# Crowsinc/LiveVisionKit

Hardware: AMD Instinct MI355X
Metric: stabilized frames/sec (one 4K YUV420 stream per GPU, steady state) (higher is better)
Workload: dtype f32

## Files before the change

### include/lvk_hip.h

```cpp
#ifndef LVK_HIP_H
#define LVK_HIP_H

#include <stdint.h>
#include <stddef.h>

#ifdef __cplusplus
extern "C" {
#endif

#define LVK_HIP_OK              0
#define LVK_HIP_ERR_ARG        -1
#define LVK_HIP_ERR_RUNTIME    -2
#define LVK_HIP_ERR_NO_DEVICE  -3

typedef struct lvk_hip_ctx lvk_hip_ctx;


int  lvk_hip_ctx_create(int device, lvk_hip_ctx** out);
int  lvk_hip_ctx_create_on_stream(int device, void* hip_stream, lvk_hip_ctx** out);
void lvk_hip_ctx_destroy(lvk_hip_ctx* ctx);
int  lvk_hip_sync(lvk_hip_ctx* ctx);
void* lvk_hip_stream(lvk_hip_ctx* ctx);
const char* lvk_hip_last_error(lvk_hip_ctx* ctx);
const char* lvk_hip_version(void);
// ... 247 lines not shown
#define LVK_SCHED_PUSH_FREE_RUNNING   0
#define LVK_SCHED_PUSH_SYNCHRONISED   1
#define LVK_SCHED_INGEST_ON_TRACKER   2
#define LVK_SCHED_INGEST_ON_BULK      3
#define LVK_SCHED_INGEST_INLINE       4
#define LVK_SCHED_REMAP_PERSISTENT    5
#define LVK_SCHED_REMAP_FULL          6
#define LVK_SCHED_WAIT_SIGNAL_WORD    7
#define LVK_SCHED_WAIT_EVENT          8
#define LVK_SCHED_WAIT_WORD_TIMEOUT   9
#define LVK_SCHED_COUNT              10
int  lvk_hip_stab_schedule_counters(lvk_hip_stab* stab, long long out[LVK_SCHED_COUNT], int reset);

int  lvk_hip_stab_get_stats(const lvk_hip_stab* stab, lvk_stab_stats* out);
int  lvk_hip_stab_detector_frames(const lvk_hip_stab* stab, long long* on_device, long long* on_host);
int  lvk_hip_stab_get_meshes(const lvk_hip_stab* stab, float* motion, float* correction, int cap_floats);
int  lvk_hip_stab_get_features(const lvk_hip_stab* stab, float* xy_resp_age, int cap);


#define LVK_STAGE_DOWNSCALE 0
#define LVK_STAGE_PYRAMID   1
#define LVK_STAGE_FAST      2
#define LVK_STAGE_PYRLK     3
#define LVK_STAGE_MOTION    4
#define LVK_STAGE_REMAP     5
#define LVK_STAGE_INGEST    6
#define LVK_STAGE_EGRESS    7
#define LVK_STAGE_COUNT     8
int  lvk_hip_stab_set_profiling(lvk_hip_stab* stab, int enable);
int  lvk_hip_stab_get_profile(lvk_hip_stab* stab, double total_ms[LVK_STAGE_COUNT], long long launches[LVK_STAGE_COUNT]);

int lvk_hip_native_rcp(lvk_hip_ctx* ctx, const float* d_in, float* d_out, size_t n);

typedef struct lvk_hip_mesh_solver lvk_hip_mesh_solver;
int  lvk_hip_mesh_solver_create(lvk_hip_ctx* ctx, int cols, int rows, float gen_region_w, float gen_region_h,
                                float temporal_smoothing, float local_smoothing, int max_points, lvk_hip_mesh_solver** out);
void lvk_hip_mesh_solver_destroy(lvk_hip_mesh_solver* solver);
int  lvk_hip_mesh_solver_reset(lvk_hip_mesh_solver* solver);
int  lvk_hip_mesh_solver_solve(lvk_hip_mesh_solver* solver, const float* tracked, const float* matched, int n, float region_w, float region_h,
                               float temporal_now, float threshold, uint8_t* inliers, float* offsets);

int lvk_hip_luma_area_resize(lvk_hip_ctx* ctx, const void* d_src, int src_step, int pix_stride, int channel,
                             int srows, int scols, void* d_dst, int dst_step, int drows, int dcols);

int lvk_hip_pyr_down(lvk_hip_ctx* ctx, const void* d_src, int src_step, int rows, int cols, void* d_dst, int dst_step);
int lvk_hip_scharr(lvk_hip_ctx* ctx, const void* d_src, int src_step, int rows, int cols, void* d_dst);

int lvk_hip_build_pyramid(lvk_hip_ctx* ctx, const void* d_img, int step, int rows, int cols, int max_level, int win_w, int win_h,
                          uint8_t* levels, int16_t* derivs, int* level_rows, int* level_cols);

int lvk_hip_fast_detect(lvk_hip_ctx* ctx, const void* d_img, int step, int rows, int cols,
                        const int* regions, int nregions, uint32_t* out, int cap, int* counts);

int lvk_hip_pyrlk(lvk_hip_ctx* ctx, const void* d_prev, int prev_step, const void* d_next, int next_step, int rows, int cols,
                  const float* prev_pts, int n, float* next_pts, uint8_t* status,
                  int win_w, int win_h, int max_level, int max_count, double epsilon, double min_eig_threshold);

int lvk_hip_estimate_global_motion(lvk_hip_ctx* ctx, const float* pts1, const float* pts2, int n, double threshold,
                                   double region_w, double region_h, int full_homography, double H[9], uint8_t* mask);

int lvk_hip_fast_filter(lvk_hip_ctx* ctx, const float* prev, const float* matched, const uint8_t* status, int n, float* out_prev, float* out_matched);

#define LVK_TRACK_CHAIN_GUARD 64
#define LVK_TRACK_CHAIN_FILL  0xA5
typedef struct lvk_track_chain_desc
{
    const float* prev; const float* matched; const uint8_t* status; const float* und;
    const void* d_prev_img; int prev_step; const void* d_next_img; int next_step; int rows, cols;
    int win_w, win_h, max_level, max_count; double epsilon, min_eig;
    const lvk_camera_params* lens; int lens_rows, lens_cols; double lens_sx, lens_sy;
    int n_bound, count_on_device, n_word;
    int full, model_on_device, full_word;
    int separate_compact, host_signal;
    double threshold; int region_w, region_h;
} lvk_track_chain_desc;
typedef struct lvk_track_chain_result
{
    double H[9]; int rc, signalled, count_dev, count_host;
    uint8_t* mask; float* pairs_dev; float* mirror_matched; uint8_t* mirror_status;
    float* next_pts; uint8_t* flow_status; float* flow_und;
} lvk_track_chain_result;
int lvk_hip_track_chain(lvk_hip_ctx* ctx, const lvk_track_chain_desc* desc, lvk_track_chain_result* result);

int lvk_hip_deblock_get_grid(lvk_hip_deblock* deb, uint8_t* mean, uint8_t* grid, float* keep_block, int capacity, int extent_xy[2]);

int lvk_hip_cas_const(float sharpness, float* peak);

int lvk_hip_cvt_code_target(int code, int src_format, int dcn);

int lvk_hip_fsr_easu_const(int rw, int rh, int W, int H, int ow, int oh, float con[16]);

int lvk_hip_fsr_easu_path(int rw, int rh, int out_rows, int out_cols);

enum
{
    LVK_AREA_PATH_FAST_DW_8x8_C3_BGR = 0, LVK_AREA_PATH_FAST_DW_8x8_C3_RGB = 1, LVK_AREA_PATH_FAST_DW_4x4_C3_BGR = 2, LVK_AREA_PATH_FAST_DW_4x4_C3_RGB = 3,
    LVK_AREA_PATH_FAST_DW_8x8_C3 = 4, LVK_AREA_PATH_FAST_DW_4x4_C3 = 5, LVK_AREA_PATH_FAST_DW_8x8_C1 = 6, LVK_AREA_PATH_FAST_DW_4x4_C1 = 7,
    LVK_AREA_PATH_FAST = 8, LVK_AREA_PATH_TILE_4 = 9, LVK_AREA_PATH_TILE_8 = 10, LVK_AREA_PATH_TAPS_4 = 11, LVK_AREA_PATH_TAPS_8 = 12,
    LVK_AREA_PATH_GENERAL = 13, LVK_AREA_PATH_ENLARGE = 14, LVK_AREA_PATH_COUNT = 15
};
int lvk_hip_area_resize_path(lvk_hip_ctx* ctx, const void* d_src, int src_step, int pix_stride, int channel,
                             int srows, int scols, int drows, int dcols);

#ifdef __cplusplus
}
#endif

#include "lvk_hip_deblock_px.h"
#endif
```

### livevisionkit_amd/_native.py

```python
import ctypes
import os

_HERE = os.path.dirname(os.path.abspath(__file__))
LIB_PATH = os.environ.get("LVK_HIP_LIB") or os.path.join(_HERE, "liblvk_hip.so")

_c = ctypes
_P = _c.c_void_p
_SIG = {
    "lvk_hip_ctx_create": (_c.c_int, [_c.c_int, _c.POINTER(_P)]),
    "lvk_hip_ctx_create_on_stream": (_c.c_int, [_c.c_int, _P, _c.POINTER(_P)]),
    "lvk_hip_ctx_destroy": (None, [_P]),
    "lvk_hip_sync": (_c.c_int, [_P]),
    "lvk_hip_stream": (_P, [_P]),
    "lvk_hip_last_error": (_c.c_char_p, [_P]),
    "lvk_hip_version": (_c.c_char_p, []),
    "lvk_hip_abi_version": (_c.c_int, []),
    "lvk_hip_device_count": (_c.c_int, []),
    "lvk_hip_device_usable": (_c.c_int, [_c.c_int]),
    "lvk_hip_malloc": (_c.c_int, [_P, _c.c_size_t, _c.POINTER(_P)]),
    "lvk_hip_free": (_c.c_int, [_P, _P]),
    "lvk_hip_trim": (_c.c_int, [_P]),
    "lvk_hip_ctx_wait": (_c.c_int, [_P, _P]),
    "lvk_hip_upload": (_c.c_int, [_P, _P, _P, _c.c_size_t]),
    "lvk_hip_download": (_c.c_int, [_P, _P, _P, _c.c_size_t]),
    "lvk_hip_remap_homography": (_c.c_int, [_P, _P, _c.c_int, _c.c_int, _c.c_int, _P, _c.c_int, _c.c_int, _c.c_int,
                                            _c.c_int, _c.c_int, _c.POINTER(_c.c_float), _c.POINTER(_c.c_uint8), _c.c_int]),
    "lvk_hip_remap_mesh": (_c.c_int, [_P, _P, _c.c_int, _c.c_int, _c.c_int, _P, _c.c_int,
                                      _c.POINTER(_c.c_float), _c.c_int, _c.c_int, _c.POINTER(_c.c_uint8), _c.c_int]),
    "lvk_hip_remap_map": (_c.c_int, [_P, _P, _c.c_int, _c.c_int, _c.c_int, _P, _c.c_int, _P, _c.c_int, _c.POINTER(_c.c_uint8), _c.c_int]),
    "lvk_hip_remap_homography_gray": (_c.c_int, [_P, _P, _c.c_int, _c.c_int, _c.c_int, _P, _c.c_int, _c.c_int, _c.c_int,
                                                 _c.c_int, _c.c_int, _c.POINTER(_c.c_float), _c.c_uint8]),
    "lvk_hip_remap_mesh_gray": (_c.c_int, [_P, _P, _c.c_int, _c.c_int, _c.c_int, _P, _c.c_int, _c.POINTER(_c.c_float), _c.c_int, _c.c_int, _c.c_uint8]),
    "lvk_hip_remap_map_gray": (_c.c_int, [_P, _P, _c.c_int, _c.c_int, _c.c_int, _P, _c.c_int, _P, _c.c_int, _c.c_uint8]),
    "lvk_hip_warpmesh_apply_gray": (_c.c_int, [_P, _P, _c.c_int, _c.c_int, _c.c_int, _P, _c.c_int, _c.POINTER(_c.c_float), _c.c_int, _c.c_int, _c.c_uint8]),
    "lvk_hip_warpmesh_apply_lens_gray": (_c.c_int, [_P, _P, _c.c_int, _c.c_int, _c.c_int, _P, _c.c_int, _c.POINTER(_c.c_float), _c.c_int, _c.c_int, _c.c_uint8, _P]),
    "lvk_hip_stab_push_gray": (_c.c_int, [_P, _P, _c.c_int, _c.c_int, _c.c_int, _c.c_uint64, _P, _c.c_int, _c.c_int,
                                          _c.POINTER(_c.c_int), _c.POINTER(_c.c_uint64), _c.POINTER(_P), _P]),
    "lvk_hip_stab_push_gray_host": (_c.c_int, [_P, _P, _c.c_int, _c.c_int, _c.c_int, _c.c_uint64, _P, _c.c_int, _c.c_int,
                                               _c.POINTER(_c.c_int), _c.POINTER(_c.c_uint64), _P]),
    "lvk_hip_set_remap_precision": (_c.c_int, [_P, _c.c_int]),
    "lvk_hip_get_remap_precision": (_c.c_int, [_P]),
    "lvk_hip_stab_set_remap_precision": (_c.c_int, [_P, _c.c_int]),
    "lvk_hip_stab_get_remap_precision": (_c.c_int, [_P]),
    "lvk_hip_remap_homography_c4": (_c.c_int, [_P, _P, _c.c_int, _c.c_int, _c.c_int, _P, _c.c_int, _c.c_int, _c.c_int,
                                               _c.c_int, _c.c_int, _c.POINTER(_c.c_float), _c.POINTER(_c.c_uint8)]),
    "lvk_hip_remap_mesh_c4": (_c.c_int, [_P, _P, _c.c_int, _c.c_int, _c.c_int, _P, _c.c_int, _c.POINTER(_c.c_float), _c.c_int, _c.c_int, _c.POINTER(_c.c_uint8)]),
    "lvk_hip_remap_map_c4": (_c.c_int, [_P, _P, _c.c_int, _c.c_int, _c.c_int, _P, _c.c_int, _P, _c.c_int, _c.POINTER(_c.c_uint8)]),
    "lvk_hip_warpmesh_apply_c4": (_c.c_int, [_P, _P, _c.c_int, _c.c_int, _c.c_int, _P, _c.c_int, _c.POINTER(_c.c_float), _c.c_int, _c.c_int, _c.POINTER(_c.c_uint8)]),
    "lvk_hip_warpmesh_apply_lens_c4": (_c.c_int, [_P, _P, _c.c_int, _c.c_int, _c.c_int, _P, _c.c_int, _c.POINTER(_c.c_float), _c.c_int, _c.c_int, _c.POINTER(_c.c_uint8), _P]),
    "lvk_hip_stab_set_background_alpha": (_c.c_int, [_P, _c.c_int]),
    "lvk_hip_stab_push_c4": (_c.c_int, [_P, _P, _c.c_int, _c.c_int, _c.c_int, _c.c_uint64, _c.c_int, _P, _c.c_int, _c.c_int,
                                        _c.POINTER(_c.c_int), _c.POINTER(_c.c_uint64), _c.POINTER(_P), _P]),
    "lvk_hip_stab_push_c4_host": (_c.c_int, [_P, _P, _c.c_int, _c.c_int, _c.c_int, _c.c_uint64, _c.c_int, _P, _c.c_int, _c.c_int,
                                             _c.POINTER(_c.c_int), _c.POINTER(_c.c_uint64), _P]),
    "lvk_hip_upscale": (_c.c_int, [_P, _P, _c.c_int, _c.c_int, _c.c_int, _P, _c.c_int, _c.c_int, _c.c_int, _c.c_int]),
    "lvk_hip_sharpen": (_c.c_int, [_P, _P, _c.c_int, _c.c_int, _c.c_int, _P, _c.c_int, _c.c_float]),
    "lvk_hip_upscale_gray": (_c.c_int, [_P, _P, _c.c_int, _c.c_int, _c.c_int, _P, _c.c_int, _c.c_int, _c.c_int]),
    "lvk_hip_upscale_c4": (_c.c_int, [_P, _P, _c.c_int, _c.c_int, _c.c_int, _P, _c.c_int, _c.c_int, _c.c_int]),
    "lvk_hip_sharpen_gray": (_c.c_int, [_P, _P, _c.c_int, _c.c_int, _c.c_int, _P, _c.c_int, _c.c_float]),
    "lvk_hip_sharpen_c4": (_c.c_int, [_P, _P, _c.c_int, _c.c_int, _c.c_int, _P, _c.c_int, _c.c_float]),
    "lvk_hip_native_rcp": (_c.c_int, [_P, _P, _P, _c.c_size_t]),
    "lvk_hip_mesh_solver_create": (_c.c_int, [_P, _c.c_int, _c.c_int, _c.c_float, _c.c_float, _c.c_float, _c.c_float, _c.c_int, _c.POINTER(_P)]),
    "lvk_hip_mesh_solver_destroy": (None, [_P]),
    "lvk_hip_mesh_solver_reset": (_c.c_int, [_P]),
    "lvk_hip_mesh_solver_solve": (_c.c_int, [_P, _c.POINTER(_c.c_float), _c.POINTER(_c.c_float), _c.c_int, _c.c_float, _c.c_float, _c.c_float, _c.c_float,
                                             _c.POINTER(_c.c_uint8), _c.POINTER(_c.c_float)]),
    "lvk_hip_lens_map_create": (_c.c_int, [_P, _P, _c.c_int, _c.c_int, _c.POINTER(_P), _c.POINTER(_c.c_int)]),
    "lvk_hip_lens_map_destroy": (_c.c_int, [_P, _P]),
    "lvk_hip_warpmesh_apply_lens": (_c.c_int, [_P, _P, _c.c_int, _c.c_int, _c.c_int, _P, _c.c_int, _c.POINTER(_c.c_float), _c.c_int, _c.c_int, _c.POINTER(_c.c_uint8), _c.c_int, _P]),
    "lvk_hip_lens_undistort_points": (_c.c_int, [_P, _P, _c.c_int, _c.c_int, _c.c_double, _c.c_double, _c.POINTER(_c.c_float), _c.c_int, _c.POINTER(_c.c_float)]),
    "lvk_hip_stab_set_lens": (_c.c_int, [_P, _P]),
    "lvk_hip_stab_output_stream": (_P, [_P]),
    "lvk_hip_fast_filter": (_c.c_int, [_P, _c.POINTER(_c.c_float), _c.POINTER(_c.c_float), _c.POINTER(_c.c_uint8), _c.c_int, _c.POINTER(_c.c_float), _c.POINTER(_c.c_float)]),
    "lvk_hip_stab_draw_trackers": (_c.c_int, [_P]),
    "lvk_hip_stab_draw_motion_mesh": (_c.c_int, [_P]),
    "lvk_hip_draw_grid": (_c.c_int, [_P, _P, _c.c_int, _c.c_int, _c.c_int, _c.c_int, _c.c_int, _c.POINTER(_c.c_uint8), _c.c_int]),
    "lvk_hip_draw_crosses": (_c.c_int, [_P, _P, _c.c_int, _c.c_int, _c.c_int, _c.POINTER(_c.c_float), _c.c_int, _c.c_float, _c.c_float,
                                        _c.POINTER(_c.c_uint8), _c.c_int, _c.c_int]),
    "lvk_hip_draw_points": (_c.c_int, [_P, _P, _c.c_int, _c.c_int, _c.c_int, _c.POINTER(_c.c_float), _c.c_int, _c.c_float, _c.c_float,
                                       _c.POINTER(_c.c_uint8), _c.c_int]),
    "lvk_hip_draw_rect": (_c.c_int, [_P, _P, _c.c_int, _c.c_int, _c.c_int, _c.POINTER(_c.c_int), _c.POINTER(_c.c_uint8), _c.c_int]),
    "lvk_hip_draw_text": (_c.c_int, [_P, _P, _c.c_int, _c.c_int, _c.c_int, _c.c_char_p, _c.c_int, _c.c_int, _c.POINTER(_c.c_uint8), _c.c_int, _c.c_int]),
    "lvk_hip_text_size": (_c.c_int, [_c.c_char_p, _c.c_int, _c.c_int, _c.POINTER(_c.c_int), _c.POINTER(_c.c_int)]),
    "lvk_hip_warpmesh_apply_yuv420": (_c.c_int, [_P, _P, _c.c_int, _c.c_int, _c.c_int, _P, _c.c_int, _P, _c.c_int, _P, _c.c_int, _c.c_int,
                                                 _c.POINTER(_c.c_float), _c.c_int, _c.c_int, _c.POINTER(_c.c_uint8)]),
    "lvk_hip_warpmesh_apply": (_c.c_int, [_P, _P, _c.c_int, _c.c_int, _c.c_int, _P, _c.c_int,
                                          _c.POINTER(_c.c_float), _c.c_int, _c.c_int, _c.POINTER(_c.c_uint8), _c.c_int]),
    "lvk_hip_luma_area_resize": (_c.c_int, [_P, _P, _c.c_int, _c.c_int, _c.c_int, _c.c_int, _c.c_int, _P, _c.c_int, _c.c_int, _c.c_int]),
    "lvk_hip_pyr_down": (_c.c_int, [_P, _P, _c.c_int, _c.c_int, _c.c_int, _P, _c.c_int]),
    "lvk_hip_scharr": (_c.c_int, [_P, _P, _c.c_int, _c.c_int, _c.c_int, _P]),
    "lvk_hip_build_pyramid": (_c.c_int, [_P, _P, _c.c_int, _c.c_int, _c.c_int, _c.c_int, _c.c_int, _c.c_int,
                                         _c.POINTER(_c.c_uint8), _c.POINTER(_c.c_int16), _c.POINTER(_c.c_int), _c.POINTER(_c.c_int)]),
    "lvk_hip_fast_detect": (_c.c_int, [_P, _P, _c.c_int, _c.c_int, _c.c_int, _c.POINTER(_c.c_int), _c.c_int,
                                       _c.POINTER(_c.c_uint32), _c.c_int, _c.POINTER(_c.c_int)]),
    "lvk_hip_pyrlk": (_c.c_int, [_P, _P, _c.c_int, _P, _c.c_int, _c.c_int, _c.c_int, _c.POINTER(_c.c_float), _c.c_int,
                                 _c.POINTER(_c.c_float), _c.POINTER(_c.c_uint8), _c.c_int, _c.c_int, _c.c_int, _c.c_int,
                                 _c.c_double, _c.c_double]),
    "lvk_hip_ingest_yuv420": (_c.c_int, [_P, _P, _c.c_int, _P, _c.c_int, _P, _c.c_int, _c.c_int, _c.c_int, _c.c_int, _P, _c.c_int]),
    "lvk_hip_egress_yuv420": (_c.c_int, [_P, _P, _c.c_int, _c.c_int, _c.c_int, _P, _c.c_int, _P, _c.c_int, _P, _c.c_int, _c.c_int]),
    "lvk_hip_ingest_obs": (_c.c_int, [_P, _c.c_int, _P * 3, _c.c_int * 3, _c.c_int, _c.c_int, _P, _c.c_int]),
    "lvk_hip_egress_obs": (_c.c_int, [_P, _c.c_int, _P, _c.c_int, _c.c_int, _c.c_int, _P * 3, _c.c_int * 3]),
    "lvk_hip_obs_frame_format": (_c.c_int, [_c.c_int]),
    "lvk_hip_estimate_global_motion": (_c.c_int, [_P, _c.POINTER(_c.c_float), _c.POINTER(_c.c_float), _c.c_int, _c.c_double,
                                                  _c.c_double, _c.c_double, _c.c_int, _c.POINTER(_c.c_double), _c.POINTER(_c.c_uint8)]),
    "lvk_hip_track_chain": (_c.c_int, [_P, _P, _P]),
    "lvk_stab_default_settings": (None, [_P]),
    "lvk_hip_stab_create": (_c.c_int, [_P, _P, _c.POINTER(_P)]),
    "lvk_hip_stab_destroy": (None, [_P]),
    "lvk_hip_stab_configure": (_c.c_int, [_P, _P]),
    "lvk_hip_stab_restart": (_c.c_int, [_P]),
    "lvk_hip_stab_reset_context": (_c.c_int, [_P]),
    "lvk_hip_stab_ready": (_c.c_int, [_P]),
    "lvk_hip_stab_frame_delay": (_c.c_int, [_P]),
    "lvk_hip_stab_stable_region": (_c.c_int, [_P, _c.c_int, _c.c_int, _c.POINTER(_c.c_int)]),
    "lvk_hip_stab_next_output": (_c.c_int, [_P, _c.c_int, _c.c_int, _c.c_int, _P]),
    "lvk_hip_stab_push": (_c.c_int, [_P, _P, _c.c_int, _c.c_int, _c.c_int, _c.c_uint64, _c.c_int, _P, _c.c_int, _c.c_int,
                                     _c.POINTER(_c.c_int), _c.POINTER(_c.c_uint64), _c.POINTER(_P), _P]),
    "lvk_hip_stab_push_yuv420": (_c.c_int, [_P, _P, _c.c_int, _P, _c.c_int, _P, _c.c_int, _c.c_int, _c.c_int, _c.c_int, _c.c_uint64,
                                            _P, _c.c_int, _P, _c.c_int, _P, _c.c_int, _c.c_int, _c.POINTER(_c.c_int), _c.POINTER(_c.c_uint64), _P]),
    "lvk_hip_stab_push_obs": (_c.c_int, [_P, _c.c_int, _P * 3, _c.c_int * 3, _c.c_int, _c.c_int, _c.c_uint64, _P * 3, _c.c_int * 3, _c.c_int,
                                         _c.POINTER(_c.c_int), _c.POINTER(_c.c_uint64), _P]),
    "lvk_hip_stab_push_yuv420_host": (_c.c_int, [_P, _P, _c.c_int, _P, _c.c_int, _P, _c.c_int, _c.c_int, _c.c_int, _c.c_int, _c.c_uint64,
                                            _P, _c.c_int, _P, _c.c_int, _P, _c.c_int, _c.c_int, _c.POINTER(_c.c_int), _c.POINTER(_c.c_uint64), _P]),
    "lvk_hip_stab_push_obs_host": (_c.c_int, [_P, _c.c_int, _P * 3, _c.c_int * 3, _c.c_int, _c.c_int, _c.c_uint64, _P * 3, _c.c_int * 3, _c.c_int,
                                              _c.POINTER(_c.c_int), _c.POINTER(_c.c_uint64), _P]),
    "lvk_hip_stab_prefetch_yuv420_host": (_c.c_int, [_P, _P, _c.c_int, _P, _c.c_int, _P, _c.c_int, _c.c_int, _c.c_int, _c.c_int]),
    "lvk_hip_stab_prefetch_cancel": (_c.c_int, [_P]),
    "lvk_hip_stab_prefetch": (_c.c_int, [_P, _P, _c.c_int, _c.c_int, _c.c_int, _c.c_int]),
    "lvk_hip_stab_prefetch_yuv420": (_c.c_int, [_P, _P, _c.c_int, _P, _c.c_int, _P, _c.c_int, _c.c_int, _c.c_int, _c.c_int]),
    "lvk_hip_stab_lookahead_frames": (_c.c_longlong, [_P]),
    "lvk_hip_stab_schedule_counters": (_c.c_int, [_P, _c.POINTER(_c.c_longlong), _c.c_int]),
    "lvk_hip_stab_detector_frames": (_c.c_int, [_P, _c.POINTER(_c.c_longlong), _c.POINTER(_c.c_longlong)]),
    "lvk_hip_host_malloc": (_c.c_int, [_P, _c.c_size_t, _c.POINTER(_P)]),
    "lvk_hip_host_free": (_c.c_int, [_P, _P]),
    "lvk_hip_stab_get_stats": (_c.c_int, [_P, _P]),
    "lvk_hip_stab_get_meshes": (_c.c_int, [_P, _c.POINTER(_c.c_float), _c.POINTER(_c.c_float), _c.c_int]),
    "lvk_hip_stab_get_features": (_c.c_int, [_P, _c.POINTER(_c.c_float), _c.c_int]),
    "lvk_hip_stab_set_overlap": (_c.c_int, [_P, _c.c_int]),
    "lvk_hip_stab_set_bulk_context": (_c.c_int, [_P, _P]),
    "lvk_hip_stab_set_profiling": (_c.c_int, [_P, _c.c_int]),
    "lvk_hip_stab_get_profile": (_c.c_int, [_P, _c.POINTER(_c.c_double), _c.POINTER(_c.c_longlong)]),
    "lvk_hip_deblock_default_settings": (None, [_P]),
    "lvk_hip_deblock_create": (_c.c_int, [_P, _P, _c.POINTER(_P)]),
    "lvk_hip_deblock_configure": (_c.c_int, [_P, _P]),
    "lvk_hip_deblock_destroy": (None, [_P]),
    "lvk_hip_deblock_apply": (_c.c_int, [_P, _P, _c.c_int, _c.c_int, _c.c_int, _c.c_int, _c.POINTER(_c.c_int)]),
    "lvk_hip_deblock_draw_influence": (_c.c_int, [_P, _P, _c.c_int, _c.c_int, _c.c_int, _c.c_int]),
    "lvk_hip_deblock_filter_region": (_c.c_int, [_P, _c.POINTER(_c.c_int)]),
    "lvk_hip_deblock_get_grid": (_c.c_int, [_P, _c.POINTER(_c.c_uint8), _c.POINTER(_c.c_uint8), _c.POINTER(_c.c_float), _c.c_int, _c.POINTER(_c.c_int)]),
    "lvk_hip_cas": (_c.c_int, [_P, _P, _c.c_int, _c.c_int, _c.c_int, _c.c_int, _P, _c.c_int, _c.c_float]),
    "lvk_hip_cas_const": (_c.c_int, [_c.c_float, _c.POINTER(_c.c_float)]),
    "lvk_hip_reformat": (_c.c_int, [_P, _P, _c.c_int, _c.c_int, _c.c_int, _c.c_int, _P, _c.c_int, _c.c_int]),
    "lvk_hip_cvt_code_target": (_c.c_int, [_c.c_int, _c.c_int, _c.c_int]),
    "lvk_hip_fsr_easu": (_c.c_int, [_P, _P, _c.c_int, _c.c_int, _c.c_int, _c.c_int, _c.POINTER(_c.c_int), _P, _c.c_int, _c.c_int, _c.c_int]),
    "lvk_hip_fsr_geometry": (_c.c_int, [_c.c_int, _c.c_int, _c.c_int, _c.c_int, _c.c_float, _c.c_int, _c.POINTER(_c.c_int), _c.POINTER(_c.c_int),
                                        _c.POINTER(_c.c_int), _c.POINTER(_c.c_int)]),
    "lvk_hip_fsr_easu_const": (_c.c_int, [_c.c_int, _c.c_int, _c.c_int, _c.c_int, _c.c_int, _c.c_int, _c.POINTER(_c.c_float)]),
    "lvk_hip_fsr_easu_path": (_c.c_int, [_c.c_int, _c.c_int, _c.c_int, _c.c_int]),
    "lvk_hip_area_resize_path": (_c.c_int, [_P, _P, _c.c_int, _c.c_int, _c.c_int, _c.c_int, _c.c_int, _c.c_int, _c.c_int]),
}

_SIG_DEBLOCK_PX = {
    "lvk_hip_deblock_apply_gray": (_c.c_int, [_P, _P, _c.c_int, _c.c_int, _c.c_int, _c.POINTER(_c.c_int)]),
    "lvk_hip_deblock_apply_c4": (_c.c_int, [_P, _P, _c.c_int, _c.c_int, _c.c_int, _c.c_int, _c.POINTER(_c.c_int)]),
}

_lib = None

# ... 26 lines not shown
```

### livevisionkit_amd/context.py

```python
import ctypes

import numpy as np

from . import _native


class LvkHipError(RuntimeError):
    pass


def _f32(a):
    a = np.ascontiguousarray(a, dtype=np.float32)
    return a, a.ctypes.data_as(ctypes.POINTER(ctypes.c_float))


def _u8x3(bg):
    a = np.ascontiguousarray(bg, dtype=np.uint8).reshape(3)
    return a, a.ctypes.data_as(ctypes.POINTER(ctypes.c_uint8))


def _u8x4(bg):
    a = np.ascontiguousarray(bg, dtype=np.uint8).reshape(4)
    return a, a.ctypes.data_as(ctypes.POINTER(ctypes.c_uint8))

# ... 408 lines not shown
        p = np.ascontiguousarray(points, np.float32).reshape(-1, 2)
        ca, cp = _u8x3(colour)
        self._check(self.lib.lvk_hip_draw_crosses(self.handle, frame.data_ptr(), frame.stride(0), frame.shape[0], frame.shape[1],
                                                  p.ctypes.data_as(ctypes.POINTER(ctypes.c_float)), len(p), float(scaling[0]), float(scaling[1]), cp,
                                                  int(cross_size), int(thickness)))
        return frame

    def fast_filter(self, prev, matched, status):
        a = np.ascontiguousarray(prev, np.float32).reshape(-1, 2); b = np.ascontiguousarray(matched, np.float32).reshape(-1, 2)
        st = np.ascontiguousarray(status, np.uint8).reshape(-1)
        oa = np.zeros_like(a); ob = np.zeros_like(b)
        fp = ctypes.POINTER(ctypes.c_float)
        m = self.lib.lvk_hip_fast_filter(self.handle, a.ctypes.data_as(fp), b.ctypes.data_as(fp), st.ctypes.data_as(ctypes.POINTER(ctypes.c_uint8)), len(a),
                                         oa.ctypes.data_as(fp), ob.ctypes.data_as(fp))
        if m < 0:
            self._check(m)
        return oa[:m], ob[:m]

    def track_chain(self, prev, matched=None, status=None, und=None, images=None, win=(11, 11), max_level=3, max_count=5, epsilon=0.01, min_eig=1e-4,
                    lens=None, threshold=3.0, region=(480, 270), full=True, full_word=None, n_word=None, separate_compact=False, host_signal=False):
        fp, bp = ctypes.POINTER(ctypes.c_float), ctypes.POINTER(ctypes.c_uint8)
        prev = np.ascontiguousarray(prev, np.float32).reshape(-1, 2)
        nb, G = len(prev), TRACK_CHAIN_GUARD
        d, r = TrackChainDesc(), TrackChainResult()
        keep = [prev]
        d.prev = prev.ctypes.data_as(fp)
        if images is None:
            matched = np.ascontiguousarray(matched, np.float32).reshape(nb, 2); status = np.ascontiguousarray(status, np.uint8).reshape(nb)
            keep += [matched, status]
            d.matched = matched.ctypes.data_as(fp); d.status = status.ctypes.data_as(bp)
            if und is not None:
                und = np.ascontiguousarray(und, np.float32).reshape(-1, 2)
                n_eff = nb if n_word is None else min(max(int(n_word), 0), nb)
                if len(und) != 2 * n_eff:
                    raise ValueError("und holds 2 x the effective count of positions (previous | matched)")
                keep.append(und)
                d.und = und.ctypes.data_as(fp)
        else:
            a, b = images
            keep += [a, b]
            d.d_prev_img = a.data_ptr(); d.prev_step = a.stride(0); d.d_next_img = b.data_ptr(); d.next_step = b.stride(0)
            d.rows, d.cols = a.shape[0], a.shape[1]
            d.win_w, d.win_h, d.max_level, d.max_count, d.epsilon, d.min_eig = win[0], win[1], max_level, max_count, float(epsilon), float(min_eig)
            if lens is not None:
                params, lrows, lcols, sx, sy = lens
                arr = (ctypes.c_double * 9)(*[float(v) for v in params])
                keep.append(arr)
                d.lens = ctypes.cast(arr, ctypes.c_void_p); d.lens_rows, d.lens_cols, d.lens_sx, d.lens_sy = int(lrows), int(lcols), float(sx), float(sy)
        d.n_bound = nb
        d.count_on_device, d.n_word = (0, 0) if n_word is None else (1, int(n_word))
        d.full = 1 if full else 0
        d.model_on_device, d.full_word = (0, 0) if full_word is None else (1, int(full_word))
        d.separate_compact = 1 if separate_compact else 0; d.host_signal = 1 if host_signal else 0
        d.threshold = float(threshold); d.region_w, d.region_h = int(region[0]), int(region[1])
        mask = np.zeros(nb, np.uint8); pairs = np.zeros((2, nb, 2), np.float32); mm = np.zeros((nb, 2), np.float32); ms = np.zeros(nb, np.uint8)
        r.mask = mask.ctypes.data_as(bp); r.pairs_dev = pairs.ctypes.data_as(fp); r.mirror_matched = mm.ctypes.data_as(fp); r.mirror_status = ms.ctypes.data_as(bp)
        out = {}
        if images is not None:
            nxt = np.zeros((nb + 2 * G, 2), np.float32); fst = np.zeros(nb + 2 * G, np.uint8); fund = np.zeros((2 * nb + 2 * G, 2), np.float32)
            r.next_pts = nxt.ctypes.data_as(fp); r.flow_status = fst.ctypes.data_as(bp); r.flow_und = fund.ctypes.data_as(fp)
            out.update(next_pts=nxt, flow_status=fst, flow_und=fund)
        self._check(self.lib.lvk_hip_track_chain(self.handle, ctypes.byref(d), ctypes.byref(r)))
        del keep
        out.update(H=np.array(r.H, np.float64).reshape(3, 3), rc=r.rc, signalled=r.signalled, count_dev=r.count_dev, count_host=r.count_host, mask=mask,
                   pairs_dev=pairs, mirror_matched=mm, mirror_status=ms)
        return out

    def warpmesh_apply_yuv420(self, src, mesh, bg=(255, 0, 255), nv12=False):
        import torch
        rows, cols = src.shape[0], src.shape[1]
        y = torch.empty((rows, cols), dtype=torch.uint8, device=src.device)
        if nv12:
            u = torch.empty((rows // 2, cols // 2, 2), dtype=torch.uint8, device=src.device); v = u
        else:
            u = torch.empty((rows // 2, cols // 2), dtype=torch.uint8, device=src.device); v = torch.empty_like(u)
        m = np.ascontiguousarray(mesh, dtype=np.float32)
        ma, mp = _f32(m)
        bga, bgp = _u8x3(bg)
        self._check(self.lib.lvk_hip_warpmesh_apply_yuv420(self.handle, src.data_ptr(), src.stride(0), rows, cols, y.data_ptr(), y.stride(0),
                                                           u.data_ptr(), u.stride(0), v.data_ptr(), v.stride(0), 1 if nv12 else 0,
                                                           mp, m.shape[0], m.shape[1], bgp))
        return (y, u) if nv12 else (y, u, v)


class MeshSolver:

    def __init__(self, ctx, cols, rows, gen_region, temporal, local, max_points):
        self.ctx, self.cols, self.rows = ctx, cols, rows
        h = ctypes.c_void_p()
        ctx._check(ctx.lib.lvk_hip_mesh_solver_create(ctx.handle, cols, rows, float(gen_region[0]), float(gen_region[1]), float(temporal), float(local),
                                                      int(max_points), ctypes.byref(h)))
        self.handle = h

    def solve(self, tracked, matched, region=(480, 270), temporal=1.0, threshold=10.0):
        t = np.ascontiguousarray(tracked, np.float32).reshape(-1, 2); m = np.ascontiguousarray(matched, np.float32).reshape(-1, 2)
        inl = np.zeros(len(t), np.uint8); off = np.zeros((self.rows, self.cols, 2), np.float32)
        fp = ctypes.POINTER(ctypes.c_float)
        rc = self.ctx.lib.lvk_hip_mesh_solver_solve(self.handle, t.ctypes.data_as(fp), m.ctypes.data_as(fp), len(t), float(region[0]), float(region[1]),
                                                    float(temporal), float(threshold), inl.ctypes.data_as(ctypes.POINTER(ctypes.c_uint8)), off.ctypes.data_as(fp))
        if rc < 0:
            self.ctx._check(rc)
        return rc, inl, off

    def reset(self):
        self.ctx._check(self.ctx.lib.lvk_hip_mesh_solver_reset(self.handle))

    def close(self):
        if getattr(self, "handle", None):
            if getattr(self.ctx, "handle", None):
                self.ctx.lib.lvk_hip_mesh_solver_destroy(self.handle)
            self.handle = None
```

### livevisionkit_amd/csrc/lvk_hip_internal.hpp

```cpp
#pragma once

#include <hip/hip_runtime.h>
#include <cstdint>
#include <cstdio>
#include <string>
#include <vector>
#include <functional>
#include <map>
#include <set>
#include <mutex>
#include <utility>

#include "lvk_hip.h"

struct LinTabEntry { int s0, s1; float a0, a1; };
struct Lin8Entry { int s0, s1, a0, a1; };
struct AreaTabEntry { int si; float alpha; };
struct FastRegion { int x, y, w, h, threshold, active; };
constexpr int LVK_FAST_INLINE_REGIONS = 8;

constexpr int LVK_MAX_PYR_LEVELS = 8;
struct PyrLevel { const uint8_t* img; const short2* deriv; int rows, cols, step; };
struct PyrArgs { PyrLevel lv[LVK_MAX_PYR_LEVELS]; int nlevels; };

// ... 154 lines not shown
int lvk_launch_fast(lvk_hip_ctx* ctx, const void* d_img, int step, int rows, int cols,
                    const FastRegion* d_regions, int nregions, int max_rw, int max_rh,
                    void* d_masks, void* d_scores, uint32_t* d_out, int cap, int* d_counts, const FastRegion* host_regions = nullptr);

struct FastInsertDesc
{
    const uint16_t* col_of; const uint32_t* row_base; const uint8_t* bucket;
    uint32_t* cell_first; void* cell_best ; int* region_count;
    const uint32_t* occ;
    const int* occ_bucket;
    int capacity; bool small_grid; int n_held, min_samples; float uniformity, homography_threshold;
    float2* pts; uint32_t* new_kp; int* result; int* d_n; int* d_full; int* counts;
};
int lvk_launch_fast_insert(lvk_hip_ctx* ctx, const void* d_img, int step, int rows, int cols, const FastRegion* host_regions, int nregions,
                           int max_rw, int max_rh, void* d_masks, void* d_scores, const FastInsertDesc& d);
bool lvk_fast_insert_fits(int cells, int nregions, int max_rw, int max_rh, int cols, int rows);
int lvk_fast_cells_reset(lvk_hip_ctx* ctx, uint32_t* d_first, void* d_best, int cells, int* d_region_count );

struct LensModel;
int lvk_pyramid_geometry(int rows, int cols, int max_level, int win_w, int win_h, int* lrows, int* lcols);
int lvk_launch_pyrlk(lvk_hip_ctx* ctx, const PyrArgs& prev, const PyrArgs& next, const float2* d_prev_pts, int n,
                     float2* d_next_pts, uint8_t* d_status, int win_w, int win_h, int max_count, double epsilon, double min_eig,
                     float2* d_prev_copy = nullptr,
                     const LensModel* lens = nullptr, double lens_sx = 0.0, double lens_sy = 0.0, float2* d_und = nullptr,
                     const int* d_n = nullptr);

struct DevicePyramid
{
    uint8_t* img_base = nullptr;
    uint8_t* deriv_base = nullptr;
    PyrArgs args{};
    int allocate(lvk_hip_ctx* ctx, int rows, int cols, int max_level, int win_w, int win_h);
    int build(lvk_hip_ctx* ctx, bool derivs = false);
    void release();
};

struct LvkHostSignal { unsigned* flag; unsigned seq; };

size_t lvk_ransac_workspace_bytes(int n);
int lvk_launch_ransac(lvk_hip_ctx* ctx, const float2* d_p1, const float2* d_p2, int n, double threshold, double region_w, double region_h,
                      bool full_homography, void* d_ws, double* d_H, int* d_ninl, uint8_t* d_mask, const int* d_n = nullptr,
                      const int* d_full = nullptr,
                      LvkHostSignal done = LvkHostSignal{nullptr, 0});
int lvk_launch_match_compact(lvk_hip_ctx* ctx, const float2* d_prev, const float2* d_matched, const uint8_t* d_status, int n,
                             float2* d_p1, float2* d_p2, int* d_count, int* h_count, float2* h_matched, uint8_t* h_status,
                             const float2* d_und = nullptr, float region_w = 0.0f, float region_h = 0.0f,
                             const int* d_n_raw = nullptr);
constexpr int LVK_COMPACT_RANSAC_MAX = 2048;
int lvk_launch_compact_ransac(lvk_hip_ctx* ctx, const float2* d_prev, const float2* d_matched, const uint8_t* d_status, int n,
                              float2* d_p1, float2* d_p2, int* d_count, int* h_count, float2* h_matched, uint8_t* h_status,
                              const float2* d_und, float region_wf, float region_hf,
                              double threshold, double region_w, double region_h, bool full_homography, void* d_ws, double* d_H, int* d_ninl, uint8_t* d_mask,
                              const int* d_n_raw = nullptr, const int* d_full = nullptr, LvkHostSignal done = LvkHostSignal{nullptr, 0});

struct LvkTrackChain
{
    const PyrArgs* prev_pyr = nullptr; const PyrArgs* next_pyr = nullptr;
    const float2* h_pts = nullptr;
    int win_w = 0, win_h = 0, max_count = 0; double epsilon = 0.0, min_eig = 0.0;
    const LensModel* lens = nullptr; double lens_sx = 0.0, lens_sy = 0.0;
    int n = 0; const int* d_n = nullptr;
    bool full = false; const int* d_full = nullptr;
    float2* d_pts = nullptr; float2* d_matched = nullptr; uint8_t* d_status = nullptr;
    float2* d_und = nullptr;
    float2* d_p1 = nullptr; float2* d_p2 = nullptr; int* d_count = nullptr;
    int* h_count = nullptr; float2* h_matched = nullptr; uint8_t* h_status = nullptr;
    int region_w = 0, region_h = 0; double threshold = 0.0;
    bool separate_compact = false;
    bool estimate = true;
    void* d_ws = nullptr; double* h_H = nullptr; int* h_ninl = nullptr; uint8_t* h_mask = nullptr;
    LvkHostSignal done{nullptr, 0};
    void (*stage_boundary)(void* user) = nullptr; void* user = nullptr;
};
int lvk_launch_track_chain(lvk_hip_ctx* ctx, const LvkTrackChain& c);

struct LensArgs;
struct RemapLaunch
{
    hipStream_t stream = nullptr;
    int precision = LVK_REMAP_EXACT;
    const LensArgs* lens = nullptr;
    bool co_scheduled = false;
    int co_blocks_per_cu = 0;
};
int lvk_launch_remap_homography(lvk_hip_ctx* ctx, const void* d_src, int src_step, int src_rows, int src_cols,
                                void* d_dst, int dst_step, int dst_rows, int dst_cols, int off_x, int off_y,
                                const float H[9], const uint8_t bg[3], int yuv, const RemapLaunch& o);
int lvk_launch_remap_mesh(lvk_hip_ctx* ctx, const void* d_src, int src_step, int src_rows, int src_cols,
                          void* d_dst, int dst_step, const float* mesh, int mesh_rows, int mesh_cols, const uint8_t bg[3], int yuv, const RemapLaunch& o);

int lvk_launch_ingest_yuv420(lvk_hip_ctx* ctx, hipStream_t stream, const void* d_y, int y_step, const void* d_u, int u_step,
                             const void* d_v, int v_step, int nv12, int rows, int cols, void* d_dst, int dst_step);
int lvk_launch_egress_yuv420(lvk_hip_ctx* ctx, hipStream_t stream, const void* d_src, int src_step, int rows, int cols,
                             void* d_y, int y_step, void* d_u, int u_step, void* d_v, int v_step, int nv12);
int lvk_ingest_obs_check(lvk_hip_ctx* ctx, int video_format, const void* const d_planes[3], const int steps[3], int rows, int cols);
int lvk_launch_ingest_obs(lvk_hip_ctx* ctx, hipStream_t stream, int video_format, const void* const d_planes[3], const int steps[3],
                          int rows, int cols, void* d_dst, int dst_step);
int lvk_launch_egress_obs(lvk_hip_ctx* ctx, hipStream_t stream, int video_format, const void* d_src, int src_step, int rows, int cols,
                          void* const d_planes[3], const int steps[3]);


int lvk_launch_remap_map(lvk_hip_ctx* ctx, const void* d_src, int src_step, int rows, int cols,
                         void* d_dst, int dst_step, const void* d_map, int map_step, const uint8_t bg[3], int yuv, const RemapLaunch& o);

struct LensModel { double d[17]; float f[17]; int view[4]; };
struct LensModelD { double d[17]; };
__device__ __forceinline__ float2 lvk_lens_undistort_point(const LensModelD& M, double sx, double sy, float2 p)
{
    const double nfx = M.d[0], nfy = M.d[1], ncx = M.d[2], ncy = M.d[3], fx = M.d[4], fy = M.d[5], cx = M.d[6], cy = M.d[7];
    const double k1 = M.d[8], k2 = M.d[9], p1 = M.d[10], p2 = M.d[11], k3 = M.d[12];
    const double kxc = M.d[13], vxc = M.d[14], kyc = M.d[15], vyc = M.d[16];
    const double s = (double)p.x * sx, t = (double)p.y * sy;
    double u = s, v = t;
    for (int pass = 0; pass < 2; pass++)
    {
        const double s1 = s - (u * kxc + vxc), t1 = t - (v * kyc + vyc);
        const double x0 = (s1 - cx) / fx, y0 = (t1 - cy) / fy;
        double x = x0, y = y0;
        for (int j = 0; j < 5; j++)
        {
            const double r2 = x * x + y * y;
            const double icdist = 1.0 / (1 + ((k3 * r2 + k2) * r2 + k1) * r2);
            if (icdist < 0) { x = x0; y = y0; break; }
            const double dX = 2 * p1 * x * y + p2 * (r2 + 2 * x * x);
            const double dY = p1 * (r2 + 2 * y * y) + 2 * p2 * x * y;
            x = (x0 - dX) * icdist;
            y = (y0 - dY) * icdist;
        }
        u = x * nfx + ncx; v = y * nfy + ncy;
    }
    return make_float2((float)(u / sx), (float)(v / sy));
}
struct LensArgs { float f[17]; };
int lvk_lens_model_build(const lvk_camera_params& params, int rows, int cols, LensModel& out);
int lvk_launch_lens_undistort(lvk_hip_ctx* ctx, hipStream_t stream, const LensModel& model, double sx, double sy,
                              const float2* a, int na, const float2* b, int nb, float2* out);
int lvk_launch_warpmesh_apply_lens(lvk_hip_ctx* ctx, const void* d_src, int src_step, int rows, int cols,
                                   void* d_dst, int dst_step, const float* mesh, int mesh_rows, int mesh_cols, const uint8_t bg[3], int yuv, const RemapLaunch& o);

int lvk_launch_remap_homography_gray(lvk_hip_ctx* ctx, const void* d_src, int src_step, int src_rows, int src_cols,
                                     void* d_dst, int dst_step, int dst_rows, int dst_cols, int off_x, int off_y, const float H[9], uint8_t bg, const RemapLaunch& o);
int lvk_launch_remap_mesh_gray(lvk_hip_ctx* ctx, const void* d_src, int src_step, int rows, int cols, void* d_dst, int dst_step,
                               const float* mesh, int mesh_rows, int mesh_cols, uint8_t bg, const RemapLaunch& o);
int lvk_launch_remap_map_gray(lvk_hip_ctx* ctx, const void* d_src, int src_step, int rows, int cols,
                              void* d_dst, int dst_step, const void* d_map, int map_step, uint8_t bg, const RemapLaunch& o);
int lvk_launch_warpmesh_apply_lens_gray(lvk_hip_ctx* ctx, const void* d_src, int src_step, int rows, int cols, void* d_dst, int dst_step,
                                        const float* mesh, int mesh_rows, int mesh_cols, uint8_t bg, const RemapLaunch& o);

int lvk_launch_remap_homography_c4(lvk_hip_ctx* ctx, const void* d_src, int src_step, int src_rows, int src_cols,
                                   void* d_dst, int dst_step, int dst_rows, int dst_cols, int off_x, int off_y, const float H[9], const uint8_t bg[4], const RemapLaunch& o);
int lvk_launch_remap_mesh_c4(lvk_hip_ctx* ctx, const void* d_src, int src_step, int rows, int cols, void* d_dst, int dst_step,
                             const float* mesh, int mesh_rows, int mesh_cols, const uint8_t bg[4], const RemapLaunch& o);
int lvk_launch_remap_map_c4(lvk_hip_ctx* ctx, const void* d_src, int src_step, int rows, int cols,
                            void* d_dst, int dst_step, const void* d_map, int map_step, const uint8_t bg[4], const RemapLaunch& o);
int lvk_launch_warpmesh_apply_lens_c4(lvk_hip_ctx* ctx, const void* d_src, int src_step, int rows, int cols, void* d_dst, int dst_step,
                                      const float* mesh, int mesh_rows, int mesh_cols, const uint8_t bg[4], const RemapLaunch& o);

int lvk_launch_draw_grid(lvk_hip_ctx* ctx, hipStream_t stream, void* d_dst, int dst_step, int rows, int cols, int grid_w, int grid_h,
                         const uint8_t colour[3], int thickness);
int lvk_launch_draw_crosses(lvk_hip_ctx* ctx, hipStream_t stream, void* d_dst, int dst_step, int rows, int cols, const float* pts, int n,
                            float scale_x, float scale_y, const uint8_t colour[3], int cross_size, int thickness);

int lvk_launch_upscale(lvk_hip_ctx* ctx, hipStream_t stream, const void* d_src, int src_step, int src_rows, int src_cols,
                       void* d_dst, int dst_step, int dst_rows, int dst_cols, int yuv);
int lvk_launch_sharpen(lvk_hip_ctx* ctx, hipStream_t stream, const void* d_src, int src_step, int rows, int cols,
                       void* d_dst, int dst_step, float sharpness);

struct lvk_mesh_solver_dev;
int lvk_mesh_solver_create(lvk_hip_ctx* ctx, int cols, int rows, float gen_w, float gen_h, float temporal, float local, lvk_mesh_solver_dev** out);
void lvk_mesh_solver_free(lvk_mesh_solver_dev* s);
int lvk_mesh_solver_reset(lvk_mesh_solver_dev* s, hipStream_t stream);
int lvk_mesh_solver_cols(const lvk_mesh_solver_dev* s);
int lvk_mesh_solver_rows(const lvk_mesh_solver_dev* s);
int lvk_launch_mesh_solve(lvk_mesh_solver_dev* s, hipStream_t stream, void* d_scratch , const float2* d_p1, const float2* d_p2, const int* d_count, int n_pts,
                          int min_samples, float region_w, float region_h, float temporal_now, float threshold,
                          float* h_offsets, uint8_t* h_mask, int* h_status);

int lvk_launch_warpmesh_apply_420(lvk_hip_ctx* ctx, const void* d_src, int src_step, int rows, int cols,
                                  void* o_y, int oy_step, void* o_u, int ou_step, void* o_v, int ov_step, int nv12,
                                  const float* mesh, int mesh_rows, int mesh_cols, const uint8_t bg[3], const RemapLaunch& o);
bool lvk_remap_obs_fusable(int video_format);
int lvk_launch_warpmesh_apply_obs(lvk_hip_ctx* ctx, int video_format, const void* d_src, int src_step, int rows, int cols,
                                  void* const planes[3], const int steps[3], const float* mesh, int mesh_rows, int mesh_cols, const uint8_t bg[3], const RemapLaunch& o);
```

### livevisionkit_amd/csrc/remap.hip

```cpp
#include "remap_core.hpp"
#ifndef LVK_CO_LDS_PAD
#define LVK_CO_LDS_PAD 0
#endif

namespace {


LVK_REMAP_KERNEL_CO(bool YUV, k_remap_homography,
                    (const uint8_t* __restrict__ src, int src_step, int src_rows, int src_cols,
                     uint8_t* __restrict__ dst, int dst_step, int dst_rows, int dst_cols,
                     int off_x, int off_y, HomographyArgs H, uint32_t bg),
{
    remap_homography<YUV, W, false>(src, src_step, src_rows, src_cols, PackedSink{dst, dst_step}, dst_rows, dst_cols, off_x, off_y, H, LensArgs{}, bg);
})

LVK_REMAP_KERNEL_CO(bool YUV, k_remap_homography_lens,
                    (const uint8_t* __restrict__ src, int src_step, int src_rows, int src_cols,
                     uint8_t* __restrict__ dst, int dst_step, int dst_rows, int dst_cols,
                     int off_x, int off_y, HomographyArgs H, LensArgs L, uint32_t bg),
{
    remap_homography<YUV, W, true>(src, src_step, src_rows, src_cols, PackedSink{dst, dst_step}, dst_rows, dst_cols, off_x, off_y, H, L, bg);
})

LVK_REMAP_KERNEL_CO(bool YUV, k_remap_mesh,
                    (const uint8_t* __restrict__ src, int src_step, int src_rows, int src_cols,
                     uint8_t* __restrict__ dst, int dst_step,
                     const float* __restrict__ mesh, int mesh_cols, int mesh_floats,
                     const LinTabEntry* __restrict__ xtab, const LinTabEntry* __restrict__ ytab, uint32_t bg),
{
    LVK_WITH_MESH_COORD(false, LensArgs{}, src_rows, src_cols, (remap_strip<YUV, W>(src, src_step, src_rows, src_cols, PackedSink{dst, dst_step}, src_rows, src_cols, coord, bg)))
})

LVK_REMAP_KERNEL_CO(bool YUV, k_remap_mesh_lens,
                    (const uint8_t* __restrict__ src, int src_step, int src_rows, int src_cols,
                     uint8_t* __restrict__ dst, int dst_step,
                     const float* __restrict__ mesh, int mesh_cols, int mesh_floats,
                     const LinTabEntry* __restrict__ xtab, const LinTabEntry* __restrict__ ytab, LensArgs L, uint32_t bg),
{
    LVK_WITH_MESH_COORD(true, L, src_rows, src_cols, (remap_strip<YUV, W>(src, src_step, src_rows, src_cols, PackedSink{dst, dst_step}, src_rows, src_cols, coord, bg)))
})

LVK_REMAP_KERNEL(bool YUV, , k_remap_map,
                 (const uint8_t* __restrict__ src, int src_step, int src_rows, int src_cols,
                  uint8_t* __restrict__ dst, int dst_step, const uint8_t* __restrict__ map, int map_step, uint32_t bg),
{
    const MapCoord coord{map, map_step};
    remap_strip<YUV, W>(src, src_step, src_rows, src_cols, PackedSink{dst, dst_step}, src_rows, src_cols, coord, bg);
})

template <bool YUV>
__global__ __launch_bounds__(256) LVK_REMAP_ATTR
void k_easu_scale(const uint8_t* __restrict__ src, int src_step, int src_rows, int src_cols,
                  uint8_t* __restrict__ dst, int dst_step, int dst_rows, int dst_cols, float rsx, float rsy)
{
    const ScaleCoord coord{rsx, rsy};
    remap_strip<YUV>(src, src_step, src_rows, src_cols, PackedSink{dst, dst_step}, dst_rows, dst_cols, coord, 0u);
}

struct Planes420 { uint8_t* y; int y_step; uint8_t* u; int u_step; uint8_t* v; int v_step; };
template <bool NV12> __device__ __forceinline__ Sink420<NV12> sink420(const Planes420& o) { return Sink420<NV12>{o.y, o.y_step, o.u, o.u_step, o.v, o.v_step}; }

LVK_REMAP_KERNEL(bool NV12, LVK_CO_SCHEDULED, k_remap_homography_420,
                 (const uint8_t* __restrict__ src, int src_step, int rows, int cols, Planes420 o, HomographyArgs H, uint32_t bg),
{
    LVK_TL(0);
    remap_homography<true, W, false>(src, src_step, rows, cols, sink420<NV12>(o), rows, cols, 0, 0, H, LensArgs{}, bg);
})

LVK_REMAP_KERNEL(bool NV12, LVK_CO_SCHEDULED, k_remap_homography_lens_420,
                 (const uint8_t* __restrict__ src, int src_step, int rows, int cols, Planes420 o, HomographyArgs H, LensArgs L, uint32_t bg),
{
    remap_homography<true, W, true>(src, src_step, rows, cols, sink420<NV12>(o), rows, cols, 0, 0, H, L, bg);
})

LVK_REMAP_KERNEL(bool NV12, LVK_CO_SCHEDULED, k_remap_mesh_420,
                 (const uint8_t* __restrict__ src, int src_step, int rows, int cols, Planes420 o,
                  const float* __restrict__ mesh, int mesh_cols, int mesh_floats, const LinTabEntry* __restrict__ xtab, const LinTabEntry* __restrict__ ytab, uint32_t bg),
{
    const Sink420<NV12> sink = sink420<NV12>(o);
    LVK_WITH_MESH_COORD(false, LensArgs{}, rows, cols, (remap_strip<true, W>(src, src_step, rows, cols, sink, rows, cols, coord, bg)))
})

LVK_REMAP_KERNEL(bool NV12, LVK_CO_SCHEDULED, k_remap_mesh_lens_420,
                 (const uint8_t* __restrict__ src, int src_step, int rows, int cols, Planes420 o,
                  const float* __restrict__ mesh, int mesh_cols, int mesh_floats, const LinTabEntry* __restrict__ xtab, const LinTabEntry* __restrict__ ytab,
                  LensArgs L, uint32_t bg),
{
    const Sink420<NV12> sink = sink420<NV12>(o);
    LVK_WITH_MESH_COORD(true, L, rows, cols, (remap_strip<true, W>(src, src_step, rows, cols, sink, rows, cols, coord, bg)))
})

}

int lvk_launch_remap_homography(lvk_hip_ctx* ctx, const void* d_src, int src_step, int src_rows, int src_cols,
                                void* d_dst, int dst_step, int dst_rows, int dst_cols,
                                int off_x, int off_y, const float H[9], const uint8_t bg[3], int yuv, const RemapLaunch& o)
{
    LVK_HIP_REQUIRE(ctx, remap_precision_known(o.precision));
    LVK_HIP_REQUIRE(ctx, H != nullptr && bg != nullptr);
    LVK_HIP_REQUIRE(ctx, remap_plane_ok(d_src, src_step, src_rows, src_cols, 3) && remap_plane_ok(d_dst, dst_step, dst_rows, dst_cols, 3));
    HomographyArgs args;
    std::memcpy(args.h, H, sizeof(args.h));
    if (o.lens)
        launch_remap(ctx, LVK_REMAP_FORMS_CO(k_remap_homography_lens, false, true), yuv != 0, dst_rows, dst_cols, o, 0, (const uint8_t*)d_src, src_step, src_rows, src_cols,
                     (uint8_t*)d_dst, dst_step, dst_rows, dst_cols, off_x, off_y, args, *o.lens, pack_bg(bg));
    else
        launch_remap(ctx, LVK_REMAP_FORMS_CO(k_remap_homography, false, true), yuv != 0, dst_rows, dst_cols, o, 0, (const uint8_t*)d_src, src_step, src_rows, src_cols,
                     (uint8_t*)d_dst, dst_step, dst_rows, dst_cols, off_x, off_y, args, pack_bg(bg));
    LVK_HIP_CHECK(ctx, hipGetLastError());
    return LVK_HIP_OK;
}

int lvk_launch_remap_mesh(lvk_hip_ctx* ctx, const void* d_src, int src_step, int src_rows, int src_cols,
                          void* d_dst, int dst_step,
                          const float* mesh, int mesh_rows, int mesh_cols, const uint8_t bg[3], int yuv, const RemapLaunch& o)
{
    LVK_HIP_REQUIRE(ctx, remap_precision_known(o.precision));
    LVK_HIP_REQUIRE(ctx, bg != nullptr && remap_mesh_ok(mesh, mesh_rows, mesh_cols));
    LVK_HIP_REQUIRE(ctx, remap_plane_ok(d_src, src_step, src_rows, src_cols, 3) && remap_plane_ok(d_dst, dst_step, src_rows, src_cols, 3));
    return with_staged_mesh(ctx, o.stream, mesh, mesh_rows, mesh_cols, src_rows, src_cols, [&](const StagedMesh& m) {
        if (o.lens)
            launch_remap(ctx, LVK_REMAP_FORMS_CO(k_remap_mesh_lens, false, true), yuv != 0, src_rows, src_cols, o, 0, (const uint8_t*)d_src, src_step, src_rows, src_cols,
                         (uint8_t*)d_dst, dst_step, m.d_mesh, m.mesh_cols, m.mesh_floats, m.xtab, m.ytab, *o.lens, pack_bg(bg));
        else
            launch_remap(ctx, LVK_REMAP_FORMS_CO(k_remap_mesh, false, true), yuv != 0, src_rows, src_cols, o, 0, (const uint8_t*)d_src, src_step, src_rows, src_cols,
                         (uint8_t*)d_dst, dst_step, m.d_mesh, m.mesh_cols, m.mesh_floats, m.xtab, m.ytab, pack_bg(bg));
    });
}

int lvk_launch_remap_map(lvk_hip_ctx* ctx, const void* d_src, int src_step, int rows, int cols,
                         void* d_dst, int dst_step, const void* d_map, int map_step, const uint8_t bg[3], int yuv, const RemapLaunch& o)
{
    LVK_HIP_REQUIRE(ctx, remap_precision_known(o.precision));
    LVK_HIP_REQUIRE(ctx, bg != nullptr);
    LVK_HIP_REQUIRE(ctx, remap_plane_ok(d_src, src_step, rows, cols, 3) && remap_plane_ok(d_dst, dst_step, rows, cols, 3) && remap_map_ok(d_map, map_step, rows, cols));
    launch_remap(ctx, LVK_REMAP_FORMS(k_remap_map, false, true), yuv != 0, rows, cols, RemapLaunch{o.stream, o.precision}, 0, (const uint8_t*)d_src, src_step, rows, cols, (uint8_t*)d_dst, dst_step,
                 (const uint8_t*)d_map, map_step, pack_bg(bg));
    LVK_HIP_CHECK(ctx, hipGetLastError());
    return LVK_HIP_OK;
}

int lvk_launch_upscale(lvk_hip_ctx* ctx, hipStream_t stream, const void* d_src, int src_step, int src_rows, int src_cols,
                       void* d_dst, int dst_step, int dst_rows, int dst_cols, int yuv)
{
    LVK_HIP_REQUIRE(ctx, d_src != d_dst);
    LVK_HIP_REQUIRE(ctx, dst_cols >= src_cols && dst_rows >= src_rows);
    LVK_HIP_REQUIRE(ctx, remap_plane_ok(d_src, src_step, src_rows, src_cols, 3) && remap_plane_ok(d_dst, dst_step, dst_rows, dst_cols, 3));
    if (dst_cols == src_cols && dst_rows == src_rows)
    {
        LVK_HIP_CHECK(ctx, hipMemcpy2DAsync(d_dst, (size_t)dst_step, d_src, (size_t)src_step, 3 * (size_t)src_cols, (size_t)src_rows,
                                            hipMemcpyDeviceToDevice, stream));
        return LVK_HIP_OK;
    }
    const float rsx = (float)src_cols / (float)dst_cols, rsy = (float)src_rows / (float)dst_rows;
    const dim3 block(256), grid = remap_grid(dst_rows, dst_cols);
    if (yuv) hipLaunchKernelGGL(k_easu_scale<true>, grid, block, 0, stream, (const uint8_t*)d_src, src_step, src_rows, src_cols, (uint8_t*)d_dst, dst_step, dst_rows, dst_cols, rsx, rsy);
    else hipLaunchKernelGGL(k_easu_scale<false>, grid, block, 0, stream, (const uint8_t*)d_src, src_step, src_rows, src_cols, (uint8_t*)d_dst, dst_step, dst_rows, dst_cols, rsx, rsy);
    LVK_HIP_CHECK(ctx, hipGetLastError());
    return LVK_HIP_OK;
}

int lvk_launch_warpmesh_apply_lens(lvk_hip_ctx* ctx, const void* d_src, int src_step, int rows, int cols,
                                   void* d_dst, int dst_step,
                                   const float* mesh, int mesh_rows, int mesh_cols, const uint8_t bg[3], int yuv, const RemapLaunch& o)
{
    return route_warpmesh(ctx, mesh, mesh_rows, mesh_cols, rows, cols,
                          [&](const float H[9]) { return lvk_launch_remap_homography(ctx, d_src, src_step, rows, cols, d_dst, dst_step, rows, cols, 0, 0, H, bg, yuv, o); },
                          [&] { return lvk_launch_remap_mesh(ctx, d_src, src_step, rows, cols, d_dst, dst_step, mesh, mesh_rows, mesh_cols, bg, yuv, o); });
}

int lvk_launch_warpmesh_apply_420(lvk_hip_ctx* ctx, const void* d_src, int src_step, int rows, int cols,
                                  void* o_y, int oy_step, void* o_u, int ou_step, void* o_v, int ov_step, int nv12,
                                  const float* mesh, int mesh_rows, int mesh_cols, const uint8_t bg[3], const RemapLaunch& o)
{
    LVK_HIP_REQUIRE(ctx, remap_precision_known(o.precision));
    LVK_HIP_REQUIRE(ctx, bg != nullptr && remap_mesh_ok(mesh, mesh_rows, mesh_cols));
    LVK_HIP_REQUIRE(ctx, (rows & 1) == 0 && (cols & 1) == 0 && remap_plane_ok(d_src, src_step, rows, cols, 3) && remap_plane_ok(o_y, oy_step, rows, cols, 1));
    LVK_HIP_REQUIRE(ctx, remap_plane_ok(o_u, ou_step, rows / 2, cols / 2, nv12 ? 2 : 1) && (nv12 || remap_plane_ok(o_v, ov_step, rows / 2, cols / 2, 1)));
    const Planes420 planes{(uint8_t*)o_y, oy_step, (uint8_t*)o_u, ou_step, (uint8_t*)(nv12 ? o_u : o_v), nv12 ? ou_step : ov_step};
    const size_t lds_pad = o.co_scheduled ? (size_t)LVK_CO_LDS_PAD : 0;
    if (mesh_rows == 2 && mesh_cols == 2)
    {
        HomographyArgs H;
        lvkh::mesh2x2_to_homography(mesh, rows, cols, H.h);
        if (o.lens) launch_remap(ctx, LVK_REMAP_FORMS(k_remap_homography_lens_420, false, true), nv12 != 0, rows, cols, o, lds_pad, (const uint8_t*)d_src, src_step, rows, cols, planes, H, *o.lens, pack_bg(bg));
        else launch_remap(ctx, LVK_REMAP_FORMS(k_remap_homography_420, false, true), nv12 != 0, rows, cols, o, lds_pad, (const uint8_t*)d_src, src_step, rows, cols, planes, H, pack_bg(bg));
        LVK_HIP_CHECK(ctx, hipGetLastError());
        return LVK_HIP_OK;
    }
    return with_staged_mesh(ctx, o.stream, mesh, mesh_rows, mesh_cols, rows, cols, [&](const StagedMesh& m) {
        if (o.lens) launch_remap(ctx, LVK_REMAP_FORMS(k_remap_mesh_lens_420, false, true), nv12 != 0, rows, cols, o, lds_pad, (const uint8_t*)d_src, src_step, rows, cols, planes,
                                 m.d_mesh, m.mesh_cols, m.mesh_floats, m.xtab, m.ytab, *o.lens, pack_bg(bg));
        else launch_remap(ctx, LVK_REMAP_FORMS(k_remap_mesh_420, false, true), nv12 != 0, rows, cols, o, lds_pad, (const uint8_t*)d_src, src_step, rows, cols, planes,
                          m.d_mesh, m.mesh_cols, m.mesh_floats, m.xtab, m.ytab, pack_bg(bg));
    });
}

extern "C" {

int lvk_hip_remap_homography(lvk_hip_ctx* ctx,
                             const void* d_src, int src_step, int src_rows, int src_cols,
                             void* d_dst, int dst_step, int dst_rows, int dst_cols,
                             int off_x, int off_y, const float H[9], const uint8_t bg[3], int yuv)
{
    LVK_HIP_ENTRY(ctx);
    return lvk_launch_remap_homography(ctx, d_src, src_step, src_rows, src_cols, d_dst, dst_step, dst_rows, dst_cols, off_x, off_y, H, bg, yuv, RemapLaunch{ctx->stream, ctx->remap_precision});
}

int lvk_hip_remap_mesh(lvk_hip_ctx* ctx,
                       const void* d_src, int src_step, int src_rows, int src_cols,
                       void* d_dst, int dst_step,
                       const float* mesh, int mesh_rows, int mesh_cols, const uint8_t bg[3], int yuv)
{
    LVK_HIP_ENTRY(ctx);
    return lvk_launch_remap_mesh(ctx, d_src, src_step, src_rows, src_cols, d_dst, dst_step, mesh, mesh_rows, mesh_cols, bg, yuv, RemapLaunch{ctx->stream, ctx->remap_precision});
}

int lvk_hip_remap_map(lvk_hip_ctx* ctx, const void* d_src, int src_step, int rows, int cols, void* d_dst, int dst_step,
                      const void* d_map, int map_step, const uint8_t bg[3], int yuv)
{
    LVK_HIP_ENTRY(ctx);
    return lvk_launch_remap_map(ctx, d_src, src_step, rows, cols, d_dst, dst_step, d_map, map_step, bg, yuv, RemapLaunch{ctx->stream, ctx->remap_precision});
}

int lvk_hip_warpmesh_apply_lens(lvk_hip_ctx* ctx, const void* d_src, int src_step, int rows, int cols, void* d_dst, int dst_step,
                                const float* mesh, int mesh_rows, int mesh_cols, const uint8_t bg[3], int yuv, const lvk_camera_params* lens)
{
    LVK_HIP_ENTRY(ctx);
    LVK_HIP_REQUIRE(ctx, lens != nullptr && rows > 1 && cols > 1);
    LensArgs a;
    const int rc = lens_args_of(ctx, lens, rows, cols, a);
    if (rc != LVK_HIP_OK) return rc;
    return lvk_launch_warpmesh_apply_lens(ctx, d_src, src_step, rows, cols, d_dst, dst_step, mesh, mesh_rows, mesh_cols, bg, yuv, RemapLaunch{ctx->stream, ctx->remap_precision, &a});
}

int lvk_hip_warpmesh_apply_yuv420(lvk_hip_ctx* ctx, const void* d_src, int src_step, int rows, int cols,
                                  void* o_y, int oy_step, void* o_u, int ou_step, void* o_v, int ov_step, int nv12,
                                  const float* mesh, int mesh_rows, int mesh_cols, const uint8_t bg[3])
{
    LVK_HIP_ENTRY(ctx);
    return lvk_launch_warpmesh_apply_420(ctx, d_src, src_step, rows, cols, o_y, oy_step, o_u, ou_step, o_v, ov_step, nv12, mesh, mesh_rows, mesh_cols, bg, RemapLaunch{ctx->stream, ctx->remap_precision});
}

int lvk_hip_upscale(lvk_hip_ctx* ctx, const void* d_src, int src_step, int src_rows, int src_cols,
                    void* d_dst, int dst_step, int dst_rows, int dst_cols, int yuv)
{
    LVK_HIP_ENTRY(ctx);
    return lvk_launch_upscale(ctx, ctx->stream, d_src, src_step, src_rows, src_cols, d_dst, dst_step, dst_rows, dst_cols, yuv);
}

int lvk_hip_warpmesh_apply(lvk_hip_ctx* ctx,
                           const void* d_src, int src_step, int rows, int cols,
                           void* d_dst, int dst_step,
                           const float* mesh, int mesh_rows, int mesh_cols, const uint8_t bg[3], int yuv)
{
    LVK_HIP_ENTRY(ctx);
    return lvk_launch_warpmesh_apply_lens(ctx, d_src, src_step, rows, cols, d_dst, dst_step, mesh, mesh_rows, mesh_cols, bg, yuv, RemapLaunch{ctx->stream, ctx->remap_precision});
}

}

LVK_TL_EXPORT(remap)
```

### livevisionkit_amd/csrc/remap_core.hpp

```cpp
#pragma once
#include "lvk_hip_internal.hpp"
#include "host_logic.hpp"

#include <climits>
#include <cstdlib>
#include <cstring>
#include <cmath>
#include <type_traits>

namespace {

struct HomographyArgs { float h[9]; };

__device__ __forceinline__ float fma_(float a, float b, float c) { return __builtin_fmaf(a, b, c); }
__device__ __forceinline__ float min_(float a, float b) { return __builtin_fminf(a, b); }
__device__ __forceinline__ float max_(float a, float b) { return __builtin_fmaxf(a, b); }
__device__ __forceinline__ float abs_(float a) { return __builtin_fabsf(a); }
__device__ __forceinline__ float rcp_lo(float a) { return __uint_as_float(0x7ef07ebbu - __float_as_uint(a)); }
__device__ __forceinline__ float rsq_lo(float a) { return __uint_as_float(0x5f347d74u - (__float_as_uint(a) >> 1)); }
__device__ __forceinline__ float sat_(float x) { return __builtin_amdgcn_fmed3f(x, 0.0f, 1.0f); }
__device__ __forceinline__ float clamp3_(float x, float lo, float hi) { return __builtin_amdgcn_fmed3f(x, lo, hi); }
__device__ __forceinline__ float rcp_native(float x) { return __builtin_amdgcn_rcpf(x); }
__device__ __forceinline__ float rcp_cl(float x)
{
// ... 284 lines not shown
struct LensCoord
{
    Inner inner; LensArgs L; int rows, cols;
    __device__ __forceinline__ void operator()(int px, int py, float& subx, float& suby) const
    {
        float u, v;
        inner(px, py, u, v);
        const int ux = (int)u, vy = (int)v;
        if (ux < 0 || ux >= cols || vy < 0 || vy >= rows) { subx = -16.0f; suby = -16.0f; return; }
        const float* f = L.f;
        const float x = (u - f[2]) * f[0], y = (v - f[3]) * f[1];
        const float r2 = __builtin_fmaf(x, x, y * y);
        const float kr = __builtin_fmaf(__builtin_fmaf(__builtin_fmaf(f[12], r2, f[9]), r2, f[8]), r2, 1.0f);
        const float xy2 = (x + x) * y;
        const float xd = __builtin_fmaf(x, kr, __builtin_fmaf(f[10], xy2, f[11] * __builtin_fmaf(x + x, x, r2)));
        const float yd = __builtin_fmaf(y, kr, __builtin_fmaf(f[10], __builtin_fmaf(y + y, y, r2), f[11] * xy2));
        subx = __builtin_fmaf(f[4], xd, f[6]) + __builtin_fmaf(u, f[13], f[14]);
        suby = __builtin_fmaf(f[5], yd, f[7]) + __builtin_fmaf(v, f[15], f[16]);
    }
};

template <bool LENS, class Coord>
__device__ __forceinline__ auto lens_coord(const Coord& coord, const LensArgs& L, int rows, int cols)
{
    if constexpr (LENS) return LensCoord<Coord>{coord, L, rows, cols};
    else return coord;
}

template <bool LENS, class F>
__device__ __forceinline__ void with_homography_coord(const HomographyArgs& H, int off_x, int off_y, const LensArgs& L, int rows, int cols, const F& f)
{
    f(lens_coord<LENS>(HomographyCoord{H, off_x, off_y}, L, rows, cols));
}

#define LVK_WITH_MESH_COORD(LENS, L, ROWS, COLS, RUN)                                                                                                        \
    if (mesh_to_lds(mesh, mesh_floats)) { const auto coord = lens_coord<LENS>(MeshCoordT<true>{mesh, mesh_cols, xtab, ytab, (float)(COLS), (float)(ROWS)}, L, ROWS, COLS); RUN; }  \
    else { const auto coord = lens_coord<LENS>(MeshCoordT<false>{mesh, mesh_cols, xtab, ytab, (float)(COLS), (float)(ROWS)}, L, ROWS, COLS); RUN; }

constexpr int PXT = 4, STRIP_W = 64 * PXT, STRIP_H = 4;
#ifndef LVK_CO_WAVES
#define LVK_CO_WAVES 4
#endif
#define LVK_CO_SCHEDULED
#ifdef LVK_REMAP_WAVES
#define LVK_REMAP_ATTR __attribute__((amdgpu_waves_per_eu(LVK_REMAP_WAVES, LVK_REMAP_WAVES)))
#else
#define LVK_REMAP_ATTR
#endif
constexpr int NUM_XCD = 8;

#define LVK_STREAM_STORE(ptr, v) __builtin_nontemporal_store((uint32_t)(v), (ptr))
__device__ __forceinline__ void store_pixels(uint8_t* __restrict__ drow, int x0, int npx, const uint32_t px[PXT], bool aligned)
{
    if (npx == PXT && aligned)
    {
        uint32_t* d = reinterpret_cast<uint32_t*>(drow + 3 * x0);
        LVK_STREAM_STORE(d + 0, px[0] | (px[1] << 24));
        LVK_STREAM_STORE(d + 1, (px[1] >> 8) | (px[2] << 16));
        LVK_STREAM_STORE(d + 2, (px[2] >> 16) | (px[3] << 8));
    }
    else
        for (int p = 0; p < npx; p++)
        {
            uint8_t* d = drow + 3 * (x0 + p);
            d[0] = (uint8_t)px[p]; d[1] = (uint8_t)(px[p] >> 8); d[2] = (uint8_t)(px[p] >> 16);
        }
}

struct PackedSink
{
    uint8_t* __restrict__ dst; int dst_step;
    __device__ __forceinline__ void store(int x0, int y, int npx, const uint32_t px[PXT], bool active, int ) const
    {
        if (!active) return;
        uint8_t* drow = dst + __umul24((uint32_t)y, (uint32_t)dst_step);
        store_pixels(drow, x0, npx, px, ((reinterpret_cast<uintptr_t>(drow) & 3u) == 0));
    }
};

template <bool NV12>
struct Sink420
{
    uint8_t* __restrict__ yp; int y_step; uint8_t* __restrict__ up; int u_step; uint8_t* __restrict__ vp; int v_step;
    __device__ __forceinline__ void store(int x0, int y, int npx, const uint32_t px[PXT], bool active, int parity) const
    {
        __shared__ uint2 s_uv2[2][256];
        uint2* s_uv = s_uv2[parity & 1];
        const int t = (int)threadIdx.x;
        const uint32_t u01 = ((px[0] >> 8) & 0xffu) + ((px[1] >> 8) & 0xffu), u23 = ((px[2] >> 8) & 0xffu) + ((px[3] >> 8) & 0xffu);
        const uint32_t v01 = ((px[0] >> 16) & 0xffu) + ((px[1] >> 16) & 0xffu), v23 = ((px[2] >> 16) & 0xffu) + ((px[3] >> 16) & 0xffu);
        s_uv[t] = make_uint2(u01 | (u23 << 16), v01 | (v23 << 16));
        if (active)
        {
            uint8_t* yr = yp + (__umul24((uint32_t)y, (uint32_t)y_step) + (uint32_t)x0);
            const uint32_t yy = (px[0] & 0xffu) | ((px[1] & 0xffu) << 8) | ((px[2] & 0xffu) << 16) | ((px[3] & 0xffu) << 24);
            if (npx == PXT && ((reinterpret_cast<uintptr_t>(yr) & 3u) == 0)) LVK_STREAM_STORE(reinterpret_cast<uint32_t*>(yr), yy);
            else for (int p = 0; p < npx; p++) yr[p] = (uint8_t)(yy >> (8 * p));
        }
        __syncthreads();
        if (active && ((t >> 6) & 1) == 0)
        {
            const uint2 a = s_uv[t], b = s_uv[t + 64];
            const uint32_t u0 = ((a.x & 0xffffu) + (b.x & 0xffffu) + 2u) >> 2, u1 = ((a.x >> 16) + (b.x >> 16) + 2u) >> 2;
            const uint32_t v0 = ((a.y & 0xffffu) + (b.y & 0xffffu) + 2u) >> 2, v1 = ((a.y >> 16) + (b.y >> 16) + 2u) >> 2;
            const int cx = x0 >> 1, cy = y >> 1, nc = npx >> 1;
            if (NV12)
            {
                uint8_t* d = up + (__umul24((uint32_t)cy, (uint32_t)u_step) + 2u * (uint32_t)cx);
                d[0] = (uint8_t)u0; d[1] = (uint8_t)v0;
                if (nc > 1) { d[2] = (uint8_t)u1; d[3] = (uint8_t)v1; }
            }
            else
            {
                uint8_t* du = up + (__umul24((uint32_t)cy, (uint32_t)u_step) + (uint32_t)cx); uint8_t* dv = vp + (__umul24((uint32_t)cy, (uint32_t)v_step) + (uint32_t)cx);
                du[0] = (uint8_t)u0; dv[0] = (uint8_t)v0;
                if (nc > 1) { du[1] = (uint8_t)u1; dv[1] = (uint8_t)v1; }
            }
        }
    }
};

template <bool YUV, class W = EasuExact, class Coord, class Sink>
__device__ __forceinline__ void remap_one_strip(const uint8_t* __restrict__ src, int src_step, int src_rows, int src_cols,
                                                const Sink& sink, int dst_rows, int dst_cols, const Coord& coord, uint32_t bg,
                                                int strip, int nstrips, int strips_x, int parity)
{
    const int sy_ = strip / strips_x, sx_ = strip - sy_ * strips_x;
    const int x0 = sx_ * STRIP_W + (int)(threadIdx.x & 63) * PXT;
    const int y = sy_ * STRIP_H + (int)(threadIdx.x >> 6);
    const bool active = strip < nstrips && x0 < dst_cols && y < dst_rows;
    const int npx = active ? min(PXT, dst_cols - x0) : 0;
    const TapBases tb = tap_bases(src, src_step);
    uint32_t px[PXT];
#pragma unroll
    for (int p = 0; p < PXT; p++)
    {
        px[p] = 0;
        if (p < npx)
        {
            float subx, suby;
            coord(x0 + p, y, subx, suby);
            const int sx = (int)subx;
            const int sy = (int)suby;
            const float ppx = __builtin_amdgcn_fractf(subx);
            const float ppy = __builtin_amdgcn_fractf(suby);
            if (sx < 1 || sy < 1 || sx >= src_cols - 4 || sy >= src_rows - 4)
            {
                if (sx >= 0 && sx < src_cols && sy >= 0 && sy < src_rows)
                {
                    const uint8_t* s = src + (__umul24((uint32_t)sy, (uint32_t)src_step) + 3u * (uint32_t)sx);
                    px[p] = (uint32_t)s[0] | ((uint32_t)s[1] << 8) | ((uint32_t)s[2] << 16);
                }
                else px[p] = bg;
            }
            else px[p] = easu_gather<YUV, W>(tb, src_step, sx, sy, ppx, ppy);
        }
    }
    sink.store(x0, y, npx, px, active, parity);
}

template <class F>
__device__ __forceinline__ void walk_strips(int dst_rows, int span_cols, const F& one_strip)
{
    const int strips_x = (span_cols + STRIP_W - 1) / STRIP_W, strips_y = (dst_rows + STRIP_H - 1) / STRIP_H;
    const int nstrips = strips_x * strips_y;
    const int band = (nstrips + NUM_XCD - 1) / NUM_XCD;
    const int xcd = (int)(blockIdx.x % NUM_XCD);
    const int kstride = (int)(gridDim.x / NUM_XCD);
    int parity = 0;
    for (int k = (int)(blockIdx.x / NUM_XCD); k < band; k += kstride, parity ^= 1)
    {
        const int strip = xcd * band + k;
        if (strip >= nstrips) break;
        one_strip(strip, nstrips, strips_x, parity);
    }
}

template <bool YUV, class W = EasuExact, class Coord, class Sink>
__device__ __forceinline__ void remap_strip(const uint8_t* __restrict__ src, int src_step, int src_rows, int src_cols,
                                            const Sink& sink, int dst_rows, int dst_cols,
                                            const Coord& coord, uint32_t bg)
{
    walk_strips(dst_rows, dst_cols, [&](int strip, int nstrips, int strips_x, int parity) __attribute__((always_inline)) {
        remap_one_strip<YUV, W>(src, src_step, src_rows, src_cols, sink, dst_rows, dst_cols, coord, bg, strip, nstrips, strips_x, parity);
    });
}

template <bool YUV, class W, bool LENS, class Sink>
__device__ __forceinline__ void remap_homography(const uint8_t* __restrict__ src, int src_step, int src_rows, int src_cols, const Sink& sink, int dst_rows, int dst_cols,
                                                 int off_x, int off_y, const HomographyArgs& H, const LensArgs& L, uint32_t bg)
{
    with_homography_coord<LENS>(H, off_x, off_y, L, src_rows, src_cols, [&](const auto& coord) __attribute__((always_inline)) {
        remap_strip<YUV, W>(src, src_step, src_rows, src_cols, sink, dst_rows, dst_cols, coord, bg);
    });
}

#define LVK_REMAP_KERNEL(TPARAM, ATTR, NAME, PARAMS, ...)                                                                          \
    template <TPARAM> __global__ __launch_bounds__(256) LVK_REMAP_ATTR ATTR void NAME PARAMS { using W = EasuExact; __VA_ARGS__ }  \
    template <TPARAM> __global__ __launch_bounds__(256) LVK_REMAP_ATTR ATTR void NAME##_r1 PARAMS { using W = EasuRegrouped; __VA_ARGS__ }
#define LVK_REMAP_KERNEL_CO(TPARAM, NAME, PARAMS, ...)                 \
    LVK_REMAP_KERNEL(TPARAM, , NAME, PARAMS, __VA_ARGS__)              \
    LVK_REMAP_KERNEL(TPARAM, LVK_CO_SCHEDULED, NAME##_co, PARAMS, __VA_ARGS__)
template <class K> struct RemapForms { K k[2][2][2]; };
#define LVK_REMAP_FORMS_(K, KCO, F0, F1) \
    RemapForms<decltype(&K<F0>)>{ { { { K<F0>, K<F1> }, { K##_r1<F0>, K##_r1<F1> } }, { { KCO<F0>, KCO<F1> }, { KCO##_r1<F0>, KCO##_r1<F1> } } } }
#define LVK_REMAP_FORMS(K, F0, F1) LVK_REMAP_FORMS_(K, K, F0, F1)
#define LVK_REMAP_FORMS_CO(K, F0, F1) LVK_REMAP_FORMS_(K, K##_co, F0, F1)

inline dim3 remap_grid(int dst_rows, int dst_cols)
{
    const int nstrips = ((dst_cols + STRIP_W - 1) / STRIP_W) * ((dst_rows + STRIP_H - 1) / STRIP_H);
    return dim3((unsigned)(((nstrips + NUM_XCD - 1) / NUM_XCD) * NUM_XCD));
}

inline dim3 lvk_co_grid(const lvk_hip_ctx* ctx, int blocks_per_cu, int dst_rows, int dst_cols)
{
    const int n = ctx->cu_count > 0 ? ctx->cu_count : 256;
    const unsigned full = remap_grid(dst_rows, dst_cols).x;
    const int per_cu = blocks_per_cu != 0 ? blocks_per_cu : LVK_CO_WAVES;
    const unsigned persistent = (unsigned)std::max(NUM_XCD, ((per_cu > 0 ? n * per_cu : n / -per_cu) / NUM_XCD) * NUM_XCD);
    return dim3(full < persistent ? full : persistent);
}

template <class K, class... Args>
inline void launch_remap(const lvk_hip_ctx* ctx, const RemapForms<K>& forms, bool flag, int dst_rows, int span_cols, const RemapLaunch& o, size_t lds_bytes,
                         const Args&... args)
{
    const dim3 grid = o.co_scheduled ? lvk_co_grid(ctx, o.co_blocks_per_cu, dst_rows, span_cols) : remap_grid(dst_rows, span_cols);
    hipLaunchKernelGGL(forms.k[o.co_scheduled ? 1 : 0][o.precision == LVK_REMAP_1LSB ? 1 : 0][flag ? 1 : 0], grid, dim3(256), lds_bytes, o.stream, args...);
}

inline bool remap_precision_known(int precision) { return precision == LVK_REMAP_EXACT || precision == LVK_REMAP_1LSB; }

inline bool fits_u32(int step, int rows) { return step > 0 && rows > 0 && step < (1 << 24) && rows < (1 << 24) && (uint64_t)step * (uint64_t)rows < (1ull << 32); }

inline bool remap_plane_ok(const void* p, int step, int rows, int cols, int bpp)
{
    return p != nullptr && cols > 0 && rows > 0 && step >= bpp * cols && fits_u32(step, rows);
}

inline bool remap_mesh_ok(const float* mesh, int mesh_rows, int mesh_cols) { return mesh != nullptr && mesh_rows >= 2 && mesh_cols >= 2; }

inline bool remap_map_ok(const void* d_map, int map_step, int rows, int cols)
{
    return remap_plane_ok(d_map, map_step, rows, cols, 8) && ((reinterpret_cast<uintptr_t>(d_map) | (uintptr_t)map_step) & 7u) == 0;
}

inline int lens_args_of(lvk_hip_ctx* ctx, const lvk_camera_params* lens, int rows, int cols, LensArgs& a)
{
    LensModel m;
    const int rc = lvk_lens_model_build(*lens, rows, cols, m);
    if (rc != LVK_HIP_OK) return ctx->fail(rc, "invalid camera profile");
    std::memcpy(a.f, m.f, sizeof(a.f));
    return LVK_HIP_OK;
}

template <class LaunchH, class LaunchM>
inline int route_warpmesh(lvk_hip_ctx* ctx, const float* mesh, int mesh_rows, int mesh_cols, int rows, int cols, const LaunchH& homography, const LaunchM& larger)
{
    LVK_HIP_REQUIRE(ctx, remap_mesh_ok(mesh, mesh_rows, mesh_cols));
    if (mesh_rows == 2 && mesh_cols == 2)
    {
        float H[9];
        lvkh::mesh2x2_to_homography(mesh, rows, cols, H);
        return homography(H);
    }
    return larger();
}

inline uint32_t pack_bg(const uint8_t bg[3]) { return (uint32_t)bg[0] | ((uint32_t)bg[1] << 8) | ((uint32_t)bg[2] << 16); }

struct StagedMesh { const float* d_mesh; int mesh_cols, mesh_floats; const LinTabEntry* xtab; const LinTabEntry* ytab; };

template <class Launch>
inline int with_staged_mesh(lvk_hip_ctx* ctx, hipStream_t stream, const float* mesh, int mesh_rows, int mesh_cols, int rows, int cols, const Launch& launch)
{
    const size_t mesh_bytes = (size_t)mesh_rows * mesh_cols * 2 * sizeof(float);
    LVK_HIP_REQUIRE(ctx, mesh_bytes <= lvk_hip_ctx::kStageBytes);
    StagedMesh m{nullptr, mesh_cols, mesh_rows * mesh_cols * 2, nullptr, nullptr};
    int rc;
    if ((rc = lvk_get_lintab(ctx, mesh_cols, cols, false, &m.xtab)) != LVK_HIP_OK) return rc;
    if ((rc = lvk_get_lintab(ctx, mesh_rows, rows, true, &m.ytab)) != LVK_HIP_OK) return rc;
    void* d_mesh = nullptr; int stage_slot = 0;
    if ((rc = lvk_stage_params(ctx, stream, mesh, mesh_bytes, &d_mesh, &stage_slot)) != LVK_HIP_OK) return rc;
    m.d_mesh = (const float*)d_mesh;
    static_assert(std::is_void_v<decltype(launch(m))>, "the launch cannot report a failure of its own: nothing returns between staging and lvk_stage_consumed");
    launch(m);
    const hipError_t le = hipGetLastError();
    rc = lvk_stage_consumed(ctx, stage_slot, stream);
    if (le != hipSuccess) return ctx->fail(LVK_HIP_ERR_RUNTIME, hipGetErrorString(le));
    return rc;
}

}
```

### livevisionkit_amd/csrc/remap_obs.hip

```cpp
#include "remap_core.hpp"

namespace {

__device__ __forceinline__ uint32_t half_even_u32(uint32_t s) { return (s + ((s >> 1) & 1u)) >> 1; }

template <int LAYOUT>
struct Sink422
{
    uint8_t* __restrict__ p0; int s0; uint8_t* __restrict__ p1; int s1; uint8_t* __restrict__ p2; int s2;
    __device__ __forceinline__ void store(int x0, int y, int npx, const uint32_t px[PXT], bool active, int ) const
    {
        if (!active) return;
        const uint32_t u0 = half_even_u32(((px[0] >> 8) & 0xffu) + ((px[1] >> 8) & 0xffu)), u1 = half_even_u32(((px[2] >> 8) & 0xffu) + ((px[3] >> 8) & 0xffu));
        const uint32_t v0 = half_even_u32(((px[0] >> 16) & 0xffu) + ((px[1] >> 16) & 0xffu)), v1 = half_even_u32(((px[2] >> 16) & 0xffu) + ((px[3] >> 16) & 0xffu));
        const uint32_t y0 = px[0] & 0xffu, y1 = px[1] & 0xffu, y2 = px[2] & 0xffu, y3 = px[3] & 0xffu;
        if (LAYOUT == 0)
        {
            uint8_t* yr = p0 + (__umul24((uint32_t)y, (uint32_t)s0) + (uint32_t)x0);
            uint8_t* ur = p1 + (__umul24((uint32_t)y, (uint32_t)s1) + (uint32_t)(x0 >> 1));
            uint8_t* vr = p2 + (__umul24((uint32_t)y, (uint32_t)s2) + (uint32_t)(x0 >> 1));
            const uint32_t yy = y0 | (y1 << 8) | (y2 << 16) | (y3 << 24);
            if (npx == PXT && ((reinterpret_cast<uintptr_t>(yr) & 3u) == 0)) LVK_STREAM_STORE(reinterpret_cast<uint32_t*>(yr), yy);
            else for (int p = 0; p < npx; p++) yr[p] = (uint8_t)(yy >> (8 * p));
            ur[0] = (uint8_t)u0; vr[0] = (uint8_t)v0;
// ... 4 lines not shown
            const uint32_t f0 = LAYOUT != 2 ? u0 : v0, g0 = LAYOUT != 2 ? v0 : u0, f1 = LAYOUT != 2 ? u1 : v1, g1 = LAYOUT != 2 ? v1 : u1;
            const uint32_t a = LAYOUT == 3 ? (f0 | (y0 << 8) | (g0 << 16) | (y1 << 24)) : (y0 | (f0 << 8) | (y1 << 16) | (g0 << 24));
            const uint32_t b = LAYOUT == 3 ? (f1 | (y2 << 8) | (g1 << 16) | (y3 << 24)) : (y2 | (f1 << 8) | (y3 << 16) | (g1 << 24));
            uint8_t* d = p0 + (__umul24((uint32_t)y, (uint32_t)s0) + 2u * (uint32_t)x0);
            if ((reinterpret_cast<uintptr_t>(d) & 3u) == 0)
            {
                LVK_STREAM_STORE(reinterpret_cast<uint32_t*>(d), a);
                if (npx > 2) LVK_STREAM_STORE(reinterpret_cast<uint32_t*>(d) + 1, b);
            }
            else
                for (int k = 0; k < 2 * npx; k++) d[k] = (uint8_t)((k < 4 ? a : b) >> (8 * (k & 3)));
        }
    }
};

template <int LAYOUT>
struct Sink444
{
    uint8_t* __restrict__ p0; int s0; uint8_t* __restrict__ p1; int s1; uint8_t* __restrict__ p2; int s2;
    __device__ __forceinline__ void store(int x0, int y, int npx, const uint32_t px[PXT], bool active, int ) const
    {
        if (!active) return;
        if (LAYOUT == 0)
        {
            uint8_t* r[3] = {p0 + (__umul24((uint32_t)y, (uint32_t)s0) + (uint32_t)x0), p1 + (__umul24((uint32_t)y, (uint32_t)s1) + (uint32_t)x0),
                             p2 + (__umul24((uint32_t)y, (uint32_t)s2) + (uint32_t)x0)};
#pragma unroll
            for (int ch = 0; ch < 3; ch++)
            {
                const uint32_t w = ((px[0] >> (8 * ch)) & 0xffu) | (((px[1] >> (8 * ch)) & 0xffu) << 8) | (((px[2] >> (8 * ch)) & 0xffu) << 16) | (((px[3] >> (8 * ch)) & 0xffu) << 24);
                if (npx == PXT && ((reinterpret_cast<uintptr_t>(r[ch]) & 3u) == 0)) LVK_STREAM_STORE(reinterpret_cast<uint32_t*>(r[ch]), w);
                else for (int p = 0; p < npx; p++) r[ch][p] = (uint8_t)(w >> (8 * p));
            }
        }
        else
        {
            uint8_t* d = p0 + (__umul24((uint32_t)y, (uint32_t)s0) + 4u * (uint32_t)x0);
            const bool al = (reinterpret_cast<uintptr_t>(d) & 3u) == 0;
            for (int p = 0; p < npx; p++)
            {
                const uint32_t w = 255u | (px[p] << 8);
                if (al) LVK_STREAM_STORE(reinterpret_cast<uint32_t*>(d) + p, w);
                else { d[4 * p] = 255; d[4 * p + 1] = (uint8_t)px[p]; d[4 * p + 2] = (uint8_t)(px[p] >> 8); d[4 * p + 3] = (uint8_t)(px[p] >> 16); }
            }
        }
    }
};

LVK_REMAP_KERNEL(class Sink, LVK_CO_SCHEDULED, k_remap_homography_planes,
                 (const uint8_t* __restrict__ src, int src_step, int rows, int cols, Sink sink, HomographyArgs H, uint32_t bg),
{
    remap_homography<true, W, false>(src, src_step, rows, cols, sink, rows, cols, 0, 0, H, LensArgs{}, bg);
})

LVK_REMAP_KERNEL(class Sink, LVK_CO_SCHEDULED, k_remap_homography_lens_planes,
                 (const uint8_t* __restrict__ src, int src_step, int rows, int cols, Sink sink, HomographyArgs H, LensArgs L, uint32_t bg),
{
    remap_homography<true, W, true>(src, src_step, rows, cols, sink, rows, cols, 0, 0, H, L, bg);
})

LVK_REMAP_KERNEL(class Sink, LVK_CO_SCHEDULED, k_remap_mesh_planes,
                 (const uint8_t* __restrict__ src, int src_step, int rows, int cols, Sink sink,
                  const float* __restrict__ mesh, int mesh_cols, int mesh_floats, const LinTabEntry* __restrict__ xtab, const LinTabEntry* __restrict__ ytab, uint32_t bg),
{
    LVK_WITH_MESH_COORD(false, LensArgs{}, rows, cols, (remap_strip<true, W>(src, src_step, rows, cols, sink, rows, cols, coord, bg)))
})

LVK_REMAP_KERNEL(class Sink, LVK_CO_SCHEDULED, k_remap_mesh_lens_planes,
                 (const uint8_t* __restrict__ src, int src_step, int rows, int cols, Sink sink,
                  const float* __restrict__ mesh, int mesh_cols, int mesh_floats, const LinTabEntry* __restrict__ xtab, const LinTabEntry* __restrict__ ytab,
                  LensArgs L, uint32_t bg),
{
    LVK_WITH_MESH_COORD(true, L, rows, cols, (remap_strip<true, W>(src, src_step, rows, cols, sink, rows, cols, coord, bg)))
})

template <class Sink>
int launch_planes(lvk_hip_ctx* ctx, const void* d_src, int src_step, int rows, int cols, const Sink& sink,
                  const float* mesh, int mesh_rows, int mesh_cols, const uint8_t bg[3], const RemapLaunch& o)
{
    if (mesh_rows == 2 && mesh_cols == 2)
    {
        HomographyArgs H;
        lvkh::mesh2x2_to_homography(mesh, rows, cols, H.h);
        if (o.lens) launch_remap(ctx, LVK_REMAP_FORMS(k_remap_homography_lens_planes, Sink, Sink), false, rows, cols, o, 0, (const uint8_t*)d_src, src_step, rows, cols, sink, H, *o.lens, pack_bg(bg));
        else launch_remap(ctx, LVK_REMAP_FORMS(k_remap_homography_planes, Sink, Sink), false, rows, cols, o, 0, (const uint8_t*)d_src, src_step, rows, cols, sink, H, pack_bg(bg));
        LVK_HIP_CHECK(ctx, hipGetLastError());
        return LVK_HIP_OK;
    }
    return with_staged_mesh(ctx, o.stream, mesh, mesh_rows, mesh_cols, rows, cols, [&](const StagedMesh& m) {
        if (o.lens) launch_remap(ctx, LVK_REMAP_FORMS(k_remap_mesh_lens_planes, Sink, Sink), false, rows, cols, o, 0, (const uint8_t*)d_src, src_step, rows, cols, sink,
                                 m.d_mesh, m.mesh_cols, m.mesh_floats, m.xtab, m.ytab, *o.lens, pack_bg(bg));
        else launch_remap(ctx, LVK_REMAP_FORMS(k_remap_mesh_planes, Sink, Sink), false, rows, cols, o, 0, (const uint8_t*)d_src, src_step, rows, cols, sink,
                          m.d_mesh, m.mesh_cols, m.mesh_floats, m.xtab, m.ytab, pack_bg(bg));
    });
}

}

bool lvk_remap_obs_fusable(int video_format)
{
    switch (video_format)
    {
    case LVK_VIDEO_FORMAT_I422: case LVK_VIDEO_FORMAT_I42A: case LVK_VIDEO_FORMAT_YUY2: case LVK_VIDEO_FORMAT_YVYU: case LVK_VIDEO_FORMAT_UYVY:
    case LVK_VIDEO_FORMAT_I444: case LVK_VIDEO_FORMAT_YUVA: case LVK_VIDEO_FORMAT_AYUV: return true;
    default: return false;
    }
}

int lvk_launch_warpmesh_apply_obs(lvk_hip_ctx* ctx, int video_format, const void* d_src, int src_step, int rows, int cols,
                                  void* const planes[3], const int steps[3], const float* mesh, int mesh_rows, int mesh_cols, const uint8_t bg[3], const RemapLaunch& o)
{
    LVK_HIP_REQUIRE(ctx, remap_precision_known(o.precision));
    LVK_HIP_REQUIRE(ctx, planes && steps && bg && remap_mesh_ok(mesh, mesh_rows, mesh_cols) && remap_plane_ok(d_src, src_step, rows, cols, 3));
    uint8_t* p0 = (uint8_t*)planes[0]; uint8_t* p1 = (uint8_t*)planes[1]; uint8_t* p2 = (uint8_t*)planes[2];
    auto plane_ok = [&](int i, int c, int bpp) { return remap_plane_ok(planes[i], steps[i], rows, c, bpp); };
    switch (video_format)
    {
    case LVK_VIDEO_FORMAT_I422: case LVK_VIDEO_FORMAT_I42A:
        LVK_HIP_REQUIRE(ctx, (cols & 1) == 0 && plane_ok(0, cols, 1) && plane_ok(1, cols / 2, 1) && plane_ok(2, cols / 2, 1));
        return launch_planes(ctx, d_src, src_step, rows, cols, Sink422<0>{p0, steps[0], p1, steps[1], p2, steps[2]}, mesh, mesh_rows, mesh_cols, bg, o);
    case LVK_VIDEO_FORMAT_YUY2:
        LVK_HIP_REQUIRE(ctx, (cols & 1) == 0 && plane_ok(0, cols, 2));
        return launch_planes(ctx, d_src, src_step, rows, cols, Sink422<1>{p0, steps[0], p0, 0, p0, 0}, mesh, mesh_rows, mesh_cols, bg, o);
    case LVK_VIDEO_FORMAT_YVYU:
        LVK_HIP_REQUIRE(ctx, (cols & 1) == 0 && plane_ok(0, cols, 2));
        return launch_planes(ctx, d_src, src_step, rows, cols, Sink422<2>{p0, steps[0], p0, 0, p0, 0}, mesh, mesh_rows, mesh_cols, bg, o);
    case LVK_VIDEO_FORMAT_UYVY:
        LVK_HIP_REQUIRE(ctx, (cols & 1) == 0 && plane_ok(0, cols, 2));
        return launch_planes(ctx, d_src, src_step, rows, cols, Sink422<3>{p0, steps[0], p0, 0, p0, 0}, mesh, mesh_rows, mesh_cols, bg, o);
    case LVK_VIDEO_FORMAT_I444: case LVK_VIDEO_FORMAT_YUVA:
        LVK_HIP_REQUIRE(ctx, plane_ok(0, cols, 1) && plane_ok(1, cols, 1) && plane_ok(2, cols, 1));
        return launch_planes(ctx, d_src, src_step, rows, cols, Sink444<0>{p0, steps[0], p1, steps[1], p2, steps[2]}, mesh, mesh_rows, mesh_cols, bg, o);
    case LVK_VIDEO_FORMAT_AYUV:
        LVK_HIP_REQUIRE(ctx, plane_ok(0, cols, 4));
        return launch_planes(ctx, d_src, src_step, rows, cols, Sink444<1>{p0, steps[0], p0, 0, p0, 0}, mesh, mesh_rows, mesh_cols, bg, o);
    }
    return ctx->fail(LVK_HIP_ERR_ARG, "lvk_launch_warpmesh_apply_obs: no fused sink for video format " + std::to_string(video_format));
}
```

### livevisionkit_amd/csrc/remap_px.hip

```cpp
#include "remap_core.hpp"

namespace {

typedef uint32_t u32x4 __attribute__((ext_vector_type(4)));

struct GrayPix
{
    static constexpr int BPP = 1;
    using Bg = uint8_t;
    static bool bg_ok(Bg) { return true; }
    static uint32_t pack_bg(Bg bg) { return bg; }
    static bool plane_ok(const void* p, int step, int rows, int cols) { return remap_plane_ok(p, step, rows, cols, 1); }

    static __device__ __forceinline__ TapBases bases(const uint8_t* __restrict__ src, int step)
    {
        return TapBases{src - 1, src + step - 1, src + 2 * (long)step - 1, src + 3 * (long)step - 1};
    }
    static __device__ __forceinline__ float4 make_tap(float byte_as_float)
    {
        const float v = byte_as_float * 0.00392156862f;
        return make_float4(v, 0.0f, 0.0f, v);
    }
#define LVK_GRAY_BYTE(w, k) make_tap((float)(((w) >> (8 * (k))) & 0xffu))
    static __device__ __forceinline__ uint32_t gather(const TapBases& gb, int step, int sx, int sy, float ppx, float ppy)
// ... 109 lines not shown
        if (x >= 0 && x < dst_cols)
        {
            float subx, suby;
            coord(x, y, subx, suby);
            const int sx = (int)subx;
            const int sy = (int)suby;
            const float ppx = __builtin_amdgcn_fractf(subx);
            const float ppy = __builtin_amdgcn_fractf(suby);
            if (sx < 1 || sy < 1 || sx >= src_cols - 4 || sy >= src_rows - 4)
            {
                if (sx >= 0 && sx < src_cols && sy >= 0 && sy < src_rows) px[p] = Pix::border(src, src_step, sx, sy);
                else px[p] = bg;
            }
            else px[p] = Pix::gather(tb, src_step, sx, sy, ppx, ppy);
        }
    }
    const auto g = Pix::group(drow, x0);
    if (x0 >= 0 && x0 + PXT <= dst_cols) Pix::store_group(g, px);
    else Pix::store_ragged(g, dst_cols, px);
}

template <class Pix, class Coord>
__device__ __forceinline__ void remap_strip_px(const uint8_t* __restrict__ src, int src_step, int src_rows, int src_cols,
                                               uint8_t* __restrict__ dst, int dst_step, int dst_rows, int dst_cols, const Coord& coord, uint32_t bg)
{
    walk_strips(dst_rows, px_span(dst_cols), [&](int strip, int , int strips_x, int ) __attribute__((always_inline)) {
        remap_one_strip_px<Pix>(src, src_step, src_rows, src_cols, dst, dst_step, dst_rows, dst_cols, coord, bg, strip, strips_x);
    });
}

template <class Pix, bool LENS, bool CO>
__global__ __launch_bounds__(256) LVK_REMAP_ATTR LVK_CO_SCHEDULED
void k_remap_homography_px(const uint8_t* __restrict__ src, int src_step, int src_rows, int src_cols,
                           uint8_t* __restrict__ dst, int dst_step, int dst_rows, int dst_cols,
                           int off_x, int off_y, HomographyArgs H, LensArgs L, uint32_t bg)
{
    with_homography_coord<LENS>(H, off_x, off_y, L, src_rows, src_cols, [&](const auto& coord) __attribute__((always_inline)) {
        remap_strip_px<Pix>(src, src_step, src_rows, src_cols, dst, dst_step, dst_rows, dst_cols, coord, bg);
    });
}

template <class Pix, bool LENS, bool CO>
__global__ __launch_bounds__(256) LVK_REMAP_ATTR LVK_CO_SCHEDULED
void k_remap_mesh_px(const uint8_t* __restrict__ src, int src_step, int rows, int cols, uint8_t* __restrict__ dst, int dst_step,
                     const float* __restrict__ mesh, int mesh_cols, int mesh_floats,
                     const LinTabEntry* __restrict__ xtab, const LinTabEntry* __restrict__ ytab, LensArgs L, uint32_t bg)
{
    LVK_WITH_MESH_COORD(LENS, L, rows, cols, remap_strip_px<Pix>(src, src_step, rows, cols, dst, dst_step, rows, cols, coord, bg))
}

template <class Pix>
__global__ __launch_bounds__(256) LVK_REMAP_ATTR
void k_remap_map_px(const uint8_t* __restrict__ src, int src_step, int rows, int cols, uint8_t* __restrict__ dst, int dst_step,
                    const uint8_t* __restrict__ map, int map_step, uint32_t bg)
{
    remap_strip_px<Pix>(src, src_step, rows, cols, dst, dst_step, rows, cols, MapCoord{map, map_step}, bg);
}

template <class Pix>
__global__ __launch_bounds__(256) LVK_REMAP_ATTR
void k_easu_scale_px(const uint8_t* __restrict__ src, int src_step, int src_rows, int src_cols,
                     uint8_t* __restrict__ dst, int dst_step, int dst_rows, int dst_cols, float rsx, float rsy)
{
    remap_strip_px<Pix>(src, src_step, src_rows, src_cols, dst, dst_step, dst_rows, dst_cols, ScaleCoord{rsx, rsy}, 0u);
}

#define LVK_PX_FORMS(K, PIX) RemapForms<decltype(&K<PIX, false, false>)>{ { { { K<PIX, false, false>, K<PIX, true, false> }, { K<PIX, false, false>, K<PIX, true, false> } }, \
                                                                            { { K<PIX, false, true>, K<PIX, true, true> }, { K<PIX, false, true>, K<PIX, true, true> } } } }

template <class Pix>
bool planes_ok(const void* src, int src_step, int src_rows, int src_cols, const void* dst, int dst_step, int dst_rows, int dst_cols)
{
    return Pix::plane_ok(src, src_step, src_rows, src_cols) && Pix::plane_ok(dst, dst_step, dst_rows, dst_cols) &&
           !lvk_pitched_overlap(src, src_step, src_rows, (long long)Pix::BPP * src_cols, dst, dst_step, dst_rows, (long long)Pix::BPP * dst_cols);
}

template <class Pix>
int launch_homography(lvk_hip_ctx* ctx, const void* d_src, int src_step, int src_rows, int src_cols,
                      void* d_dst, int dst_step, int dst_rows, int dst_cols, int off_x, int off_y, const float H[9], typename Pix::Bg bg, const RemapLaunch& o)
{
    LVK_HIP_REQUIRE(ctx, H != nullptr && Pix::bg_ok(bg) && planes_ok<Pix>(d_src, src_step, src_rows, src_cols, d_dst, dst_step, dst_rows, dst_cols));
    HomographyArgs args;
    std::memcpy(args.h, H, sizeof(args.h));
    launch_remap(ctx, LVK_PX_FORMS(k_remap_homography_px, Pix), o.lens != nullptr, dst_rows, px_span(dst_cols), o, 0, (const uint8_t*)d_src, src_step, src_rows, src_cols,
                 (uint8_t*)d_dst, dst_step, dst_rows, dst_cols, off_x, off_y, args, o.lens ? *o.lens : LensArgs{}, Pix::pack_bg(bg));
    LVK_HIP_CHECK(ctx, hipGetLastError());
    return LVK_HIP_OK;
}

template <class Pix>
int launch_mesh(lvk_hip_ctx* ctx, const void* d_src, int src_step, int rows, int cols, void* d_dst, int dst_step,
                const float* mesh, int mesh_rows, int mesh_cols, typename Pix::Bg bg, const RemapLaunch& o)
{
    LVK_HIP_REQUIRE(ctx, Pix::bg_ok(bg) && remap_mesh_ok(mesh, mesh_rows, mesh_cols) && planes_ok<Pix>(d_src, src_step, rows, cols, d_dst, dst_step, rows, cols));
    return with_staged_mesh(ctx, o.stream, mesh, mesh_rows, mesh_cols, rows, cols, [&](const StagedMesh& m) {
        launch_remap(ctx, LVK_PX_FORMS(k_remap_mesh_px, Pix), o.lens != nullptr, rows, px_span(cols), o, 0, (const uint8_t*)d_src, src_step, rows, cols, (uint8_t*)d_dst, dst_step,
                     m.d_mesh, m.mesh_cols, m.mesh_floats, m.xtab, m.ytab, o.lens ? *o.lens : LensArgs{}, Pix::pack_bg(bg));
    });
}

template <class Pix>
int launch_map(lvk_hip_ctx* ctx, const void* d_src, int src_step, int rows, int cols,
               void* d_dst, int dst_step, const void* d_map, int map_step, typename Pix::Bg bg, const RemapLaunch& o)
{
    LVK_HIP_REQUIRE(ctx, Pix::bg_ok(bg) && remap_map_ok(d_map, map_step, rows, cols) && planes_ok<Pix>(d_src, src_step, rows, cols, d_dst, dst_step, rows, cols));
    hipLaunchKernelGGL(k_remap_map_px<Pix>, remap_grid(rows, px_span(cols)), dim3(256), 0, o.stream, (const uint8_t*)d_src, src_step, rows, cols, (uint8_t*)d_dst, dst_step,
                       (const uint8_t*)d_map, map_step, Pix::pack_bg(bg));
    LVK_HIP_CHECK(ctx, hipGetLastError());
    return LVK_HIP_OK;
}

template <class Pix>
int launch_warpmesh_apply_lens(lvk_hip_ctx* ctx, const void* d_src, int src_step, int rows, int cols, void* d_dst, int dst_step,
                               const float* mesh, int mesh_rows, int mesh_cols, typename Pix::Bg bg, const RemapLaunch& o)
{
    return route_warpmesh(ctx, mesh, mesh_rows, mesh_cols, rows, cols,
                          [&](const float H[9]) { return launch_homography<Pix>(ctx, d_src, src_step, rows, cols, d_dst, dst_step, rows, cols, 0, 0, H, bg, o); },
                          [&] { return launch_mesh<Pix>(ctx, d_src, src_step, rows, cols, d_dst, dst_step, mesh, mesh_rows, mesh_cols, bg, o); });
}

template <class Pix>
int launch_upscale(lvk_hip_ctx* ctx, const void* d_src, int src_step, int src_rows, int src_cols, void* d_dst, int dst_step, int dst_rows, int dst_cols)
{
    LVK_HIP_REQUIRE(ctx, planes_ok<Pix>(d_src, src_step, src_rows, src_cols, d_dst, dst_step, dst_rows, dst_cols));
    LVK_HIP_REQUIRE(ctx, dst_cols >= src_cols && dst_rows >= src_rows);
    if (dst_cols == src_cols && dst_rows == src_rows)
    {
        LVK_HIP_CHECK(ctx, hipMemcpy2DAsync(d_dst, (size_t)dst_step, d_src, (size_t)src_step, Pix::BPP * (size_t)src_cols, (size_t)src_rows,
                                            hipMemcpyDeviceToDevice, ctx->stream));
        return LVK_HIP_OK;
    }
    const float rsx = (float)src_cols / (float)dst_cols, rsy = (float)src_rows / (float)dst_rows;
    hipLaunchKernelGGL(k_easu_scale_px<Pix>, remap_grid(dst_rows, px_span(dst_cols)), dim3(256), 0, ctx->stream, (const uint8_t*)d_src, src_step, src_rows, src_cols,
                       (uint8_t*)d_dst, dst_step, dst_rows, dst_cols, rsx, rsy);
    LVK_HIP_CHECK(ctx, hipGetLastError());
    return LVK_HIP_OK;
}

}

int lvk_launch_remap_homography_gray(lvk_hip_ctx* ctx, const void* d_src, int src_step, int src_rows, int src_cols,
                                     void* d_dst, int dst_step, int dst_rows, int dst_cols, int off_x, int off_y, const float H[9], uint8_t bg, const RemapLaunch& o)
{
    return launch_homography<GrayPix>(ctx, d_src, src_step, src_rows, src_cols, d_dst, dst_step, dst_rows, dst_cols, off_x, off_y, H, bg, o);
}

int lvk_launch_remap_mesh_gray(lvk_hip_ctx* ctx, const void* d_src, int src_step, int rows, int cols, void* d_dst, int dst_step,
                               const float* mesh, int mesh_rows, int mesh_cols, uint8_t bg, const RemapLaunch& o)
{
    return launch_mesh<GrayPix>(ctx, d_src, src_step, rows, cols, d_dst, dst_step, mesh, mesh_rows, mesh_cols, bg, o);
}

int lvk_launch_remap_map_gray(lvk_hip_ctx* ctx, const void* d_src, int src_step, int rows, int cols,
                              void* d_dst, int dst_step, const void* d_map, int map_step, uint8_t bg, const RemapLaunch& o)
{
    return launch_map<GrayPix>(ctx, d_src, src_step, rows, cols, d_dst, dst_step, d_map, map_step, bg, o);
}

int lvk_launch_warpmesh_apply_lens_gray(lvk_hip_ctx* ctx, const void* d_src, int src_step, int rows, int cols, void* d_dst, int dst_step,
                                        const float* mesh, int mesh_rows, int mesh_cols, uint8_t bg, const RemapLaunch& o)
{
    return launch_warpmesh_apply_lens<GrayPix>(ctx, d_src, src_step, rows, cols, d_dst, dst_step, mesh, mesh_rows, mesh_cols, bg, o);
}

int lvk_launch_remap_homography_c4(lvk_hip_ctx* ctx, const void* d_src, int src_step, int src_rows, int src_cols,
                                   void* d_dst, int dst_step, int dst_rows, int dst_cols, int off_x, int off_y, const float H[9], const uint8_t bg[4], const RemapLaunch& o)
{
    return launch_homography<C4Pix>(ctx, d_src, src_step, src_rows, src_cols, d_dst, dst_step, dst_rows, dst_cols, off_x, off_y, H, bg, o);
}

int lvk_launch_remap_mesh_c4(lvk_hip_ctx* ctx, const void* d_src, int src_step, int rows, int cols, void* d_dst, int dst_step,
                             const float* mesh, int mesh_rows, int mesh_cols, const uint8_t bg[4], const RemapLaunch& o)
{
    return launch_mesh<C4Pix>(ctx, d_src, src_step, rows, cols, d_dst, dst_step, mesh, mesh_rows, mesh_cols, bg, o);
}

int lvk_launch_remap_map_c4(lvk_hip_ctx* ctx, const void* d_src, int src_step, int rows, int cols,
                            void* d_dst, int dst_step, const void* d_map, int map_step, const uint8_t bg[4], const RemapLaunch& o)
{
// ... 104 lines not shown
```

### livevisionkit_amd/csrc/stab_configure.hip

```cpp
#include "stab_state.hpp"

using namespace lvkstab;

int lvk_hip_stab::prof_begin(int kind, hipStream_t stream)
{
    if (!stream) stream = ctx->stream;
    if (!profiling || !((prof_mask >> kind) & 1u) || (prof_tick % prof_every) != 0) return -1;
    if (ev_used >= 1024 && prof_collect() != LVK_HIP_OK) return -1;
    if (ev_used == ev_pool.size())
    {
        EvPair p{nullptr, nullptr, kind};
        if (hipEventCreate(&p.a) != hipSuccess || hipEventCreate(&p.b) != hipSuccess) return -1;
        ev_pool.push_back(p);
    }
    ev_pool[ev_used].kind = kind;
    (void)hipEventRecord(ev_pool[ev_used].a, stream);
    return (int)ev_used++;
}

void lvk_hip_stab::prof_end(int idx, hipStream_t stream) { if (idx >= 0) (void)hipEventRecord(ev_pool[(size_t)idx].b, stream ? stream : ctx->stream); }

int lvk_hip_stab::prof_collect()
{
    LVK_HIP_CHECK(ctx, hipStreamSynchronize(ctx->stream));
// ... 172 lines not shown
    if (configured && s.stabilize_output && !st.stabilize_output) reset_context();
    const bool res_changed = !configured || st.detection_width != s.detection_width || st.detection_height != s.detection_height;
    const bool layout_changed = res_changed || st.detection_regions_x != s.detection_regions_x || st.detection_regions_y != s.detection_regions_y
                                || st.max_feature_density != s.max_feature_density;
    mesh_gen = gen;
    if (regenerate || new_solver)
    {
        if (mesh_dev) { (void)hipStreamSynchronize(ctx->stream); lvk_mesh_solver_free(mesh_dev); }
        mesh_dev = new_solver;
    }
    if (new_offsets)
    {
        (void)hipStreamSynchronize(ctx->stream);
        if (h_offsets) (void)hipHostFree(h_offsets);
        h_offsets = new_offsets; h_offsets_floats = want_offsets;
    }
    tracker_s = st;
    smoother.configure(st);
    queue_capacity = (size_t)st.predictive_samples + 1;
    while (queue.size() > queue_capacity)
    {
        if (queue_kind == 1) orphaned.push_back(queue.front().d_ptr);
        queue.pop_front();
    }
    grid.configure(st);
    if (configured && res_changed && initialized) grid.reset();
    s = st;
    configured = true;
    if (layout_changed || !buffers_ok)
    {
        buffers_ok = false;
        int rc = alloc_tracker_buffers();
        if (rc != LVK_HIP_OK) return rc;
        if (res_changed || pyr_w != s.detection_width || pyr_h != s.detection_height)
        {
            if ((rc = alloc_pyramids()) != LVK_HIP_OK) return rc;
            prev_w = prev_h = cur_w = cur_h = 0;
        }
        buffers_ok = true;
    }
    return LVK_HIP_OK;
}

extern "C" {

void lvk_stab_default_settings(lvk_stab_settings* s)
{
    if (!s) return;
    s->detection_width = 256; s->detection_height = 256; s->detection_regions_x = 2; s->detection_regions_y = 2; s->force_detection = 0;
    s->max_feature_density = 0.20f; s->min_feature_density = 0.05f; s->accumulation_rate = 2.0f;
    s->track_local_motions = 1; s->temporal_smoothing = 1.0f; s->local_smoothing = 20.0f;
    s->min_motion_samples = 75; s->acceptance_threshold = 8.0f; s->uniformity_threshold = 0.20f;
    s->predictive_samples = 10; s->corrective_limit_x = 0.1f; s->corrective_limit_y = 0.1f; s->smoothing_steps = 20.0f; s->response_rate = 0.04f;
    s->motion_width = 2; s->motion_height = 2;
    s->background[0] = 255; s->background[1] = 0; s->background[2] = 255;
    s->crop_to_stable_region = 0; s->stabilize_output = 1; s->min_scene_quality = 0.8f; s->min_tracking_quality = 0.3f;
}

int lvk_hip_stab_create(lvk_hip_ctx* ctx, const lvk_stab_settings* settings, lvk_hip_stab** out)
{
    if (!ctx) return LVK_HIP_ERR_ARG;
    LVK_HIP_REQUIRE(ctx, settings && out);
    lvk_device_guard device_guard(ctx);
    *out = nullptr;
    auto* st = new lvk_hip_stab();
    st->ctx = ctx;
    const int rc = st->configure(*settings);
    if (rc != LVK_HIP_OK)
    {
        st->free_tracker_buffers(); lvk_mesh_solver_free(st->mesh_dev); st->pyr[0].release(); st->pyr[1].release();
        if (st->h_offsets) (void)hipHostFree(st->h_offsets);
        if (st->h_mesh_status) (void)hipHostFree(st->h_mesh_status);
        delete st; return rc;
    }
    *out = st;
    return LVK_HIP_OK;
}

static void rehome_stage_events(lvk_hip_ctx* ctx);

void lvk_hip_stab_destroy(lvk_hip_stab* st)
{
    if (!st) return;
    lvk_device_guard device_guard(st->ctx);
    (void)hipStreamSynchronize(st->ctx->stream);
    st->trace.dump();
    if (st->trace.on && st->host_trace_n)
        std::fprintf(stderr, "[lvk host trace] push_yuv420_host, us/frame: uploads enqueued %.1f, stream wait + sink choice %.1f, inner push %.1f, chroma wait %.1f, download enqueued %.1f\n",
                     st->host_trace_acc[0] / st->host_trace_n, st->host_trace_acc[1] / st->host_trace_n, st->host_trace_acc[2] / st->host_trace_n,
                     st->host_trace_acc[3] / st->host_trace_n, st->host_trace_acc[4] / st->host_trace_n);
    st->free_tracker_buffers();
    lvk_mesh_solver_free(st->mesh_dev);
    if (st->h_offsets) (void)hipHostFree(st->h_offsets);
    if (st->h_mesh_status) (void)hipHostFree(st->h_mesh_status);
    st->pyr[0].release(); st->pyr[1].release();
    st->free_pool();
    st->free_hostio();
    if (st->remap_stream) (void)hipStreamSynchronize(st->remap_stream);
    st->free_gray_host();
    if (st->remap_stream)
    {
        (void)hipStreamSynchronize(st->remap_stream);
        rehome_stage_events(st->ctx);
        auto& aux = st->ctx->aux_streams;
        { std::lock_guard<std::mutex> alock(st->ctx->aux_mutex); aux.erase(std::remove(aux.begin(), aux.end(), st->remap_stream), aux.end()); }
        if (st->remap_stream_owned) (void)hipStreamDestroy(st->remap_stream);
    }
    for (int i = 0; i < 2; i++) if (st->remap_done[i]) (void)hipEventDestroy(st->remap_done[i]);
    if (st->ingest_done) (void)hipEventDestroy(st->ingest_done);
    if (st->chain_done) (void)hipEventDestroy(st->chain_done);
    if (st->caller_ready) (void)hipEventDestroy(st->caller_ready);
    if (st->ahead_read_done) (void)hipEventDestroy(st->ahead_read_done);
    if (st->h_chain_flag) (void)hipHostFree(st->h_chain_flag);
    for (auto& p : st->ev_pool) { (void)hipEventDestroy(p.a); (void)hipEventDestroy(p.b); }
    delete st;
}

void* lvk_hip_stab_output_stream(lvk_hip_stab* st)
{
    if (!st) return nullptr;
    return (void*)((st->overlap && st->s.stabilize_output && st->remap_stream) ? st->remap_stream : st->ctx->stream);
}

static void rehome_stage_events(lvk_hip_ctx* ctx)
{
    for (int i = 0; i < lvk_hip_ctx::kStageSlots; i++) if (ctx->stage_done[i]) (void)hipEventRecord(ctx->stage_done[i], ctx->stream);
}

static int stab_detach_bulk_stream(lvk_hip_stab* st)
{
    lvk_hip_ctx* ctx = st->ctx;
    if (!st->remap_stream) return LVK_HIP_OK;
    (void)hipStreamSynchronize(st->remap_stream);
    rehome_stage_events(ctx);
    std::fill(st->slot_read_armed.begin(), st->slot_read_armed.end(), (char)0);
    for (int i = 0; i < 2; i++) if (st->remap_done[i]) (void)hipEventRecord(st->remap_done[i], ctx->stream);
    if (st->ingest_done) (void)hipEventRecord(st->ingest_done, ctx->stream);
    st->remap_wait = nullptr;
    auto& aux = ctx->aux_streams;
    { std::lock_guard<std::mutex> alock(ctx->aux_mutex); aux.erase(std::remove(aux.begin(), aux.end(), st->remap_stream), aux.end()); }
    if (st->remap_stream_owned) LVK_HIP_CHECK(ctx, hipStreamDestroy(st->remap_stream));
    st->remap_stream = nullptr; st->remap_stream_owned = false;
    return LVK_HIP_OK;
}

static int stab_set_overlap(lvk_hip_stab* st, bool enable, lvk_hip_ctx* bulk)
{
    lvk_hip_ctx* ctx = st->ctx;
    LVK_HIP_CHECK(ctx, hipStreamSynchronize(ctx->stream));
    if (st->remap_stream) LVK_HIP_CHECK(ctx, hipStreamSynchronize(st->remap_stream));
    if (st->pending_release) { if (st->queue_kind == 1) st->orphaned.push_back(st->pending_release); st->pending_release = nullptr; st->pending_slot = -1; }
    st->caller_wait_pending = false;
    if (enable)
    {
        hipStream_t want = bulk ? bulk->stream : nullptr;
        if (bulk) LVK_HIP_REQUIRE(ctx, bulk != ctx && bulk->device == ctx->device && bulk->stream != ctx->stream);
        if (st->remap_stream && (bulk ? st->remap_stream != want : !st->remap_stream_owned))
        { const int rc = stab_detach_bulk_stream(st); if (rc != LVK_HIP_OK) return rc; }
        if (!st->remap_stream)
        {
            if (bulk) { st->remap_stream = want; st->remap_stream_owned = false; }
            else
            {
                int prio_least = 0, prio_greatest = 0;
                LVK_HIP_CHECK(ctx, hipDeviceGetStreamPriorityRange(&prio_least, &prio_greatest));
                LVK_HIP_CHECK(ctx, hipStreamCreateWithPriority(&st->remap_stream, hipStreamNonBlocking, prio_least));
// ... 219 lines not shown
```

### livevisionkit_amd/csrc/stab_state.hpp

```cpp
#pragma once
#include "lvk_hip_internal.hpp"
#include "host_logic.hpp"

#include <chrono>
#include <cstdio>
#include <cstdlib>
#include <cstring>
#include <deque>
#include <functional>
#include <thread>

namespace lvkstab {

using lvkh::Feature;
using lvkh::WarpMeshF;

constexpr int LK_WIN = 11, LK_LEVELS = 3, LK_ITERS = 5;
constexpr double LK_EPS = 0.01, LK_MIN_EIG = 1e-4;
constexpr float HOMOGRAPHY_DISTRIBUTION_THRESHOLD = 0.6f;
constexpr float QA_UPDATE_RATE = 0.1f, QA_BLEND_STEP = 0.05f;

inline void lvk_cpu_relax()
{
#if defined(__x86_64__) || defined(__i386__)
    __builtin_ia32_pause();
#elif defined(__aarch64__)
    asm volatile("yield" ::: "memory");
#else
    std::this_thread::yield();
#endif
}

inline float step_toward(float current, float target, float amount)
{
    return current > target ? std::max(current - amount, target) : std::min(current + amount, target);
}

struct HostTrace
{
    enum { ENTER, DOWN_PYR_LAUNCH, FAST_SYNC, GRID, LK_LAUNCH, LK_SYNC, FILTER, RANSAC_LAUNCH, RANSAC_SYNC, POST, SMOOTH, REMAP_LAUNCH, EXIT, EMIT_WAITS, EMIT_KERNEL, EMIT_EVENT, EXIT_PRE, EXIT_WAIT, N };
    bool on = std::getenv("LVK_HIP_HOST_TRACE") != nullptr;
    double acc[N] = {0}; long cnt[N] = {0};
    std::chrono::steady_clock::time_point last;
    void begin() { if (on) last = std::chrono::steady_clock::now(); }
    void mark(int k)
    {
        if (!on) return;
        const auto now = std::chrono::steady_clock::now();
        acc[k] += std::chrono::duration<double, std::micro>(now - last).count(); cnt[k]++; last = now;
    }
    void dump() const
    {
        if (!on) return;
        static const char* names[N] = {"enter", "downscale+pyramid launch", "fast launch+sync", "grid (host)", "lk upload+launch", "lk sync", "filter (host)",
                                       "ransac upload+launch", "ransac sync", "post (host)", "qa+smoother (host)", "remap launch", "exit",
                                       "  emit: stream waits", "  emit: remap kernel launch", "  emit: slot event record", "  exit: up to the conversion wait", "  exit: conversion wait"};
        double total = 0; long frames = cnt[DOWN_PYR_LAUNCH] ? cnt[DOWN_PYR_LAUNCH] : 1;
        for (int i = 0; i < N; i++) total += acc[i];
        std::fprintf(stderr, "[lvk host trace] %ld frames, %.1f us/frame inside push\n", frames, total / frames);
        for (int i = 0; i < N; i++) if (cnt[i]) std::fprintf(stderr, "  %-28s %8.1f us/frame (%ld marks)\n", names[i], acc[i] / frames, cnt[i]);
    }
};

struct QueuedFrame { const void* d_ptr; int step, rows, cols; uint64_t ts; int format; };


struct OutPlanes420 { void* y; int y_step; void* u; int u_step; void* v; int v_step; int nv12; bool used; int rows_cap = 0; int vf = 0; void* p[3] = {nullptr, nullptr, nullptr}; int s[3] = {0, 0, 0}; };

struct HostPlane { const void* p; int step, width, rows; };

inline int host_planes_of(int vf, const void* const planes[3], const int steps[3], int rows, int cols, HostPlane out[3])
{
    auto set = [&](int i, int w, int r, bool tight = false) { out[i] = HostPlane{planes[i], tight ? w : steps[i], w, r}; };
    switch (vf)
    {
    case LVK_VIDEO_FORMAT_I420: case LVK_VIDEO_FORMAT_I40A: set(0, cols, rows); set(1, cols / 2, rows / 2); set(2, cols / 2, rows / 2); return 3;
    case LVK_VIDEO_FORMAT_NV12: set(0, cols, rows); set(1, cols, rows / 2); return 2;
    case LVK_VIDEO_FORMAT_I422: case LVK_VIDEO_FORMAT_I42A: set(0, cols, rows); set(1, cols / 2, rows); set(2, cols / 2, rows); return 3;
    case LVK_VIDEO_FORMAT_I444: case LVK_VIDEO_FORMAT_YUVA: set(0, cols, rows); set(1, cols, rows); set(2, cols, rows); return 3;
    case LVK_VIDEO_FORMAT_YUY2: case LVK_VIDEO_FORMAT_YVYU: case LVK_VIDEO_FORMAT_UYVY: set(0, 2 * cols, rows); return 1;
    case LVK_VIDEO_FORMAT_AYUV: set(0, 4 * cols, rows); return 1;
    case LVK_VIDEO_FORMAT_BGR3: set(0, 3 * cols, rows); return 1;
    case LVK_VIDEO_FORMAT_RGBA: case LVK_VIDEO_FORMAT_BGRA: case LVK_VIDEO_FORMAT_BGRX: set(0, 3 * cols, rows, true); return 1;
// ... 15 lines not shown
    DevicePyramid pyr[2];
    int cur = 0;
    int pyr_w = 0, pyr_h = 0;
    int prev_w = 0, prev_h = 0, cur_w = 0, cur_h = 0;
    bool initialized = false;
    size_t cap_features = 0;
    int fast_cap = 0, fast_max_rw = 0, fast_max_rh = 0, fast_regions = 0;
    void* d_fast_masks = nullptr; void* d_fast_scores = nullptr;
    float2 *d_pts = nullptr, *d_matched = nullptr, *d_p1 = nullptr; uint8_t* d_status = nullptr;
    void* d_ransac_ws = nullptr;
    int* d_count = nullptr;
    uint16_t* d_grid_col = nullptr; uint32_t* d_grid_row = nullptr; uint8_t* d_grid_bucket = nullptr;
    uint32_t* d_cell_first = nullptr; void* d_cell_best = nullptr; int* d_region_count = nullptr;
    int* d_n_points = nullptr; int* d_full = nullptr;
    uint32_t* h_occ = nullptr; uint32_t* h_new_kp = nullptr; int* h_insert = nullptr;
    bool device_grid = [] { const char* e = std::getenv("LVK_HIP_HOST_GRID"); return !(e && e[0] == '1'); }();
    long device_grid_frames = 0, host_grid_frames = 0;
    float2* d_und = nullptr;
    uint32_t* h_fast_out = nullptr; int* h_fast_counts = nullptr; FastRegion* h_regions = nullptr;
    float2 *h_pts = nullptr, *h_matched = nullptr, *h_p1 = nullptr; uint8_t* h_status = nullptr;
    double* h_H = nullptr; int* h_ninl = nullptr; uint8_t* h_mask = nullptr;
    int* h_count = nullptr;
    float2* h_und = nullptr;

    bool lens = false;
    lvk_camera_params lens_params{};
    LensModel lens_model{}; LensArgs lens_args{};
    int lens_rows = 0, lens_cols = 0;
    int ensure_lens(int rows, int cols)
    {
        if (!lens || (rows == lens_rows && cols == lens_cols)) return LVK_HIP_OK;
        if (lvk_lens_model_build(lens_params, rows, cols, lens_model) != LVK_HIP_OK) return fail(LVK_HIP_ERR_ARG, "invalid camera profile for this frame size");
        std::memcpy(lens_args.f, lens_model.f, sizeof(lens_args.f));
        lens_rows = rows; lens_cols = cols;
        return LVK_HIP_OK;
    }

    HostTrace trace;

    lvkh::FeatureGridH grid;
    lvkh::PathSmootherH smoother;
    struct MeshGen { int cols = 0, rows = 0; float w = 0, h = 0, temporal = 0, local = 0; } mesh_gen;
    lvk_mesh_solver_dev* mesh_dev = nullptr;
    void* d_mesh_scratch = nullptr; float* h_offsets = nullptr; int* h_mesh_status = nullptr; size_t h_offsets_floats = 0;
    lvk_stab_settings tracker_s{};
    std::vector<Feature> tracked;
    std::vector<FastRegion> plan;
    std::deque<QueuedFrame> queue;
    size_t queue_capacity = 1;
    bool next_output(const QueuedFrame& in, QueuedFrame* f) const
    {
        const size_t n = queue.size(), drop = n == queue_capacity ? 1 : 0;
        if (n - drop + 1 != queue_capacity) return false;
        if (f) *f = n > drop ? queue[drop] : in;
        return true;
    }
    float tracking_stability = 0.0f, scene_quality = 0.0f, trust = 0.0f;
    float last_distribution = 0.0f; int last_detected = 0, last_matched = 0;
    double last_H[9] = {1, 0, 0, 0, 1, 0, 0, 0, 1};
    WarpMeshF last_motion, last_correction;

    int remap_precision = LVK_REMAP_EXACT;
    uint8_t background_alpha = 0;

    bool overlap = false;
    hipStream_t remap_stream = nullptr;
    bool remap_stream_owned = false;
    hipEvent_t remap_done[2] = {nullptr, nullptr};
    int remap_slot = 0;
    const void* pending_release = nullptr;
    bool pool_frames = false;
    int queue_kind = 0;
    std::function<int()> deferred_ingest;
    int run_deferred_ingest() { auto f = std::move(deferred_ingest); deferred_ingest = nullptr; return f ? f() : LVK_HIP_OK; }
    hipEvent_t ingest_done = nullptr;
    unsigned long long ingest_recorded_for = 0;
    hipEvent_t chain_done = nullptr;
    unsigned* h_chain_flag = nullptr; unsigned chain_seq = 0;
    long signal_spin_us = [] { const char* e = std::getenv("LVK_HIP_SIGNAL_SPIN_US"); return e ? std::max(0L, std::atol(e)) : 400L; }();
    bool signal_test_lose = [] { const char* e = std::getenv("LVK_HIP_SIGNAL_TEST_LOSE"); return e && e[0] == '1'; }();
    bool ingest_on_tracker = false, tracker_ingest_capable = false;
    bool bulk_busy_at_push = false;
    bool caller_runs_free = false;
    int assume_caller = [] { const char* e = std::getenv("LVK_HIP_ASSUME_CALLER"); return !e ? 0 : (e[0] == 'f' ? 1 : (e[0] == 's' ? 2 : 0)); }();
    int free_streak = 0, sync_streak = 0;
    std::chrono::steady_clock::time_point last_push_end{};
    long long sched[LVK_SCHED_COUNT] = {0};
    int ingest_placement = [] { const char* e = std::getenv("LVK_HIP_INGEST_PLACEMENT"); return !e ? 0 : (e[0] == 't' ? 1 : (e[0] == 'b' ? 2 : 0)); }();
    std::vector<hipEvent_t> slot_read_done;
    std::vector<char> slot_read_armed;
    int slot_index(const void* p) const { for (size_t i = 0; i < pool_all.size(); i++) if (pool_all[i] == p) return (int)i; return -1; }
    int pending_slot = -1;
    hipEvent_t caller_ready = nullptr;
    bool caller_wait_pending = false;
    int mark_caller_work()
    {
        if (!(overlap && s.stabilize_output && remap_stream)) return LVK_HIP_OK;
        if (hipStreamQuery(ctx->stream) == hipSuccess) { caller_wait_pending = false; return LVK_HIP_OK; }
        (void)hipGetLastError();
        if (!caller_ready) LVK_HIP_CHECK(ctx, hipEventCreateWithFlags(&caller_ready, hipEventDisableTiming));
        LVK_HIP_CHECK(ctx, hipEventRecord(caller_ready, ctx->stream));
        caller_wait_pending = true;
        return LVK_HIP_OK;
    }
    int bulk_stream_sees_caller_work()
    {
        if (!caller_wait_pending) return LVK_HIP_OK;
        caller_wait_pending = false;
        LVK_HIP_CHECK(ctx, hipStreamWaitEvent(remap_stream, caller_ready, 0));
        return LVK_HIP_OK;
    }
    std::deque<const void*> orphaned;

    bool profiling = false;
    unsigned prof_mask = ~0u;
    unsigned prof_every = 1, prof_tick = 0;
    struct EvPair { hipEvent_t a, b; int kind; };
    std::vector<EvPair> ev_pool; size_t ev_used = 0;
    double prof_ms[LVK_STAGE_COUNT] = {0}; long prof_n[LVK_STAGE_COUNT] = {0};
    int prof_begin(int kind, hipStream_t stream = nullptr);
    void prof_end(int idx, hipStream_t stream = nullptr);
    int prof_collect();

    int fail(int code, const std::string& msg) { return ctx->fail(code, msg); }
    void free_tracker_buffers();
    int alloc_tracker_buffers();
    int alloc_pyramids();
    int configure(const lvk_stab_settings& st);
    void tracker_restart();
    void reset_context() { tracker_restart(); smoother.restart(); }
    int post_n = -1, post_m = 0;
    bool post_error = false;
    void finish_post();
    int track(const QueuedFrame& f, const void* luma, int luma_step, int luma_pix, int luma_channel, WarpMeshF& motion, bool& have_motion);

    struct HostIO
    {
        static constexpr int K_IN = 2, K_OUT = 3;
        hipStream_t up = nullptr, down = nullptr, down2 = nullptr;
        struct Pending { bool valid = false; int slot = 0; void* y; void* u; void* v; int ys, us, vs, nv12; } pending;
        int rows = 0, cols = 0;
        size_t in_bytes = 0;
        void* d_in[K_IN] = {nullptr, nullptr}; void* d_out[K_OUT] = {nullptr, nullptr, nullptr};
        hipEvent_t y_done[K_IN] = {}, c_done[K_IN] = {}, out_ready[K_OUT] = {}, down_done[K_OUT] = {};
        bool down_armed[K_OUT] = {false, false, false};
        bool y_is_c[K_IN] = {false, false};
        struct Ahead { int slot; const void* key[3]; int rows, cols, nv12; };
        std::deque<Ahead> ahead;
        const uint8_t* last_dst_lo = nullptr; const uint8_t* last_dst_hi = nullptr;
        int in_next = 0, out_next = 0, last_down = -1;
        std::chrono::steady_clock::time_point last_end{};
    } hostio;
    bool host_free_running_hint = false;
    std::vector<void*> gray_host_live;
    hipEvent_t gray_up_done = nullptr, gray_fence = nullptr;
    bool gray_host_owns(const void* p) const { return std::find(gray_host_live.begin(), gray_host_live.end(), p) != gray_host_live.end(); }
    bool gray_host_entry_now = false;
    void free_gray_host();
    bool host_direct_now = false;
    hipEvent_t ingest_wait[2] = {nullptr, nullptr};
    hipEvent_t remap_wait = nullptr;
    int ensure_hostio(int rows, int cols, size_t in_bytes = 0);
    int require_pinned(const void* p, size_t bytes, const char* what)
    {
        if (!p || bytes == 0) return LVK_HIP_OK;
        for (const uint8_t* q : {(const uint8_t*)p, (const uint8_t*)p + (bytes - 1)})
// ... 88 lines not shown
```

### livevisionkit_amd/csrc/stabilizer.hip

```cpp
#include "stab_state.hpp"

using namespace lvkstab;

int lvk_hip_stab::track(const QueuedFrame& f, const void* luma, int luma_step, int luma_pix, int luma_channel, WarpMeshF& motion, bool& have_motion)
{
    have_motion = false;
    tracking_stability = 0.0f;
    last_detected = last_matched = 0; last_distribution = 0.0f;
    hipStream_t st = ctx->stream;
    int rc;

    cur ^= 1;
    std::swap(prev_w, cur_w); std::swap(prev_h, cur_h);
    cur_w = s.detection_width; cur_h = s.detection_height;
    DevicePyramid& C = pyr[cur];
    DevicePyramid& P = pyr[cur ^ 1];
    int pe = 0;
    const bool built_ahead = ahead_built_for == push_seq && ahead_built.same(luma, luma_step, luma_pix, luma_channel, f.rows, f.cols) && pyr_w == cur_w && pyr_h == cur_h;
    ahead_built = LumaAhead(); ahead_built_for = 0;
    if (built_ahead) lookahead_frames++;
    else
    {
        pe = prof_begin(LVK_STAGE_DOWNSCALE);
        if ((rc = lvk_launch_luma_area_resize(ctx, luma, luma_step, luma_pix, luma_channel, f.rows, f.cols, const_cast<uint8_t*>(C.args.lv[0].img), C.args.lv[0].step, cur_h, cur_w)) != LVK_HIP_OK) return rc;
// ... 19 lines not shown
    if (dev_insert)
    {
        for (size_t i = 0; i < n_held; i++) h_pts[i] = make_float2(grid.held[i].x, grid.held[i].y);
        int occ_bucket[16];
        grid.occupancy(h_occ, occ_bucket);
        const FastInsertDesc d{d_grid_col, d_grid_row, d_grid_bucket, d_cell_first, d_cell_best, d_region_count, h_occ, occ_bucket, (int)grid.capacity(), grid.grid_cols() <= 4 || grid.grid_rows() <= 4, (int)n_held,
                               s.min_motion_samples, s.uniformity_threshold, HOMOGRAPHY_DISTRIBUTION_THRESHOLD, h_pts, h_new_kp, h_insert, d_n_points, d_full, h_fast_counts};
        pe = prof_begin(LVK_STAGE_FAST);
        if ((rc = lvk_launch_fast_insert(ctx, C.args.lv[0].img, C.args.lv[0].step, cur_h, cur_w, h_regions, (int)plan.size(), fast_max_rw, fast_max_rh,
                                         d_fast_masks, d_fast_scores, d)) != LVK_HIP_OK) return rc;
        prof_end(pe);
        device_grid_frames++;
    }
    else
    {
    if (any)
    {
        pe = prof_begin(LVK_STAGE_FAST);
        if ((rc = lvk_launch_fast(ctx, C.args.lv[0].img, C.args.lv[0].step, cur_h, cur_w, h_regions, (int)plan.size(), fast_max_rw, fast_max_rh,
                                  d_fast_masks, d_fast_scores, h_fast_out, fast_cap, h_fast_counts, h_regions)) != LVK_HIP_OK) return rc;
        prof_end(pe);
        LVK_HIP_CHECK(ctx, hipStreamSynchronize(st));
        trace.mark(HostTrace::FAST_SYNC);
        host_grid_frames++;
    }
    for (size_t i = 0; i < plan.size(); i++)
        if (plan[i].active) grid.absorb(i, h_fast_out + i * (size_t)fast_cap, std::min(h_fast_counts[i], fast_cap));
    distribution = grid.finish(tracked);
    last_distribution = distribution; last_detected = (int)tracked.size();
    if (tracked.size() < (size_t)s.min_motion_samples || distribution < s.uniformity_threshold) { tracked.clear(); return leave_early(); }
    if (tracked.size() > cap_features) return fail(LVK_HIP_ERR_RUNTIME, "feature count exceeds the suppression grid capacity");
    }

    trace.mark(HostTrace::GRID);
    int n = dev_insert ? (int)n_bound : (int)tracked.size();
    if (!dev_insert) for (int i = 0; i < n; i++) h_pts[i] = make_float2(tracked[i].x, tracked[i].y);
    const int* dn = dev_insert ? d_n_points : nullptr;
    const int* dfull = dev_insert ? d_full : nullptr;
    const bool full = distribution > HOMOGRAPHY_DISTRIBUTION_THRESHOLD;
    const bool chained = n <= 4096;
    const bool field = s.track_local_motions != 0;
    LvkHostSignal done{nullptr, 0};
    if (chained && !field && !caller_runs_free)
    {
        if (!h_chain_flag) { LVK_HIP_CHECK(ctx, hipHostMalloc((void**)&h_chain_flag, 64, hipHostMallocCoherent)); *h_chain_flag = 0; }
        done = LvkHostSignal{h_chain_flag, ++chain_seq};
    }
    pe = prof_begin(LVK_STAGE_PYRLK);
    if (chained)
    {
        struct Stage { lvk_hip_stab* self; int* pe; } stage{this, &pe};
        LvkTrackChain c;
        c.prev_pyr = &P.args; c.next_pyr = &C.args; c.h_pts = h_pts;
        c.win_w = LK_WIN; c.win_h = LK_WIN; c.max_count = LK_ITERS; c.epsilon = LK_EPS; c.min_eig = LK_MIN_EIG;
        c.lens = lens ? &lens_model : nullptr; c.lens_sx = (double)f.cols / (double)cur_w; c.lens_sy = (double)f.rows / (double)cur_h;
        c.n = n; c.d_n = dn; c.full = full; c.d_full = dfull;
        c.d_pts = d_pts; c.d_matched = d_matched; c.d_status = d_status; c.d_und = lens ? d_und : nullptr;
        c.d_p1 = d_p1; c.d_p2 = d_p1 + cap_features; c.d_count = d_count; c.h_count = h_count; c.h_matched = h_matched; c.h_status = h_status;
        c.region_w = cur_w; c.region_h = cur_h; c.threshold = s.acceptance_threshold;
        c.separate_compact = field; c.estimate = !field;
        c.d_ws = d_ransac_ws; c.h_H = h_H; c.h_ninl = h_ninl; c.h_mask = h_mask; c.done = done;
        c.stage_boundary = [](void* u) { Stage* g = (Stage*)u; g->self->prof_end(*g->pe); *g->pe = g->self->prof_begin(LVK_STAGE_MOTION); };
        c.user = &stage;
        if ((rc = lvk_launch_track_chain(ctx, c)) != LVK_HIP_OK) return rc;
        if (field)
        {
            if ((rc = lvk_launch_mesh_solve(mesh_dev, st, d_mesh_scratch, d_p1, d_p1 + cap_features, d_count, n, s.min_motion_samples, (float)cur_w, (float)cur_h,
                                            s.temporal_smoothing, s.acceptance_threshold, h_offsets, h_mask, h_mesh_status)) != LVK_HIP_OK) return rc;
        }
        prof_end(pe);
    }
    else
    {
        LVK_HIP_CHECK(ctx, hipMemcpyAsync(d_pts, h_pts, n * sizeof(float2), hipMemcpyHostToDevice, st));
        if ((rc = lvk_launch_pyrlk(ctx, P.args, C.args, d_pts, n, h_matched, h_status, LK_WIN, LK_WIN, LK_ITERS, LK_EPS, LK_MIN_EIG)) != LVK_HIP_OK) return rc;
        prof_end(pe);
    }
    trace.mark(HostTrace::LK_LAUNCH);
    bool chain_event_armed = false;
    if (deferred_ingest && tracker_ingest_capable)
    {
        const hipError_t q = hipStreamQuery(remap_stream);
        if (q != hipSuccess) (void)hipGetLastError();
        ingest_on_tracker = ingest_placement == 1 || (ingest_placement == 0 && ((q == hipErrorNotReady && !host_direct_now) || ingest_wait[0] != nullptr));
    }
    const bool build_ahead = chained && ahead_announced.luma != nullptr && pyr_w == cur_w && pyr_h == cur_h;
    if (chained && ((deferred_ingest && tracker_ingest_capable && ingest_on_tracker) || build_ahead))
    {
        if (!chain_done) LVK_HIP_CHECK(ctx, hipEventCreateWithFlags(&chain_done, hipEventDisableTiming));
        LVK_HIP_CHECK(ctx, hipEventRecord(chain_done, st)); chain_event_armed = true;
    }
    if (deferred_ingest && (rc = run_deferred_ingest()) != LVK_HIP_OK) return rc;
    if (build_ahead && (rc = launch_build_ahead(P, cur_w, cur_h)) != LVK_HIP_OK) return rc;
    if (lens && !chained)
    {
        if ((rc = lvk_launch_lens_undistort(ctx, st, lens_model, (double)f.cols / (double)cur_w, (double)f.rows / (double)cur_h,
                                            d_pts, n, h_matched, n, h_und)) != LVK_HIP_OK) return rc;
    }
    bool have_results = false;
    if (done.flag)
    {
        const unsigned expect = signal_test_lose ? done.seq + 0x40000000u : done.seq;
        const auto t0 = std::chrono::steady_clock::now();
        const auto budget = std::chrono::microseconds(signal_spin_us);
        for (unsigned spins = 0;; spins++)
        {
            if (__atomic_load_n(done.flag, __ATOMIC_ACQUIRE) == expect) { have_results = true; break; }
            if ((spins & 63u) == 63u && std::chrono::steady_clock::now() - t0 > budget) break;
            lvk_cpu_relax();
        }
        sched[have_results ? LVK_SCHED_WAIT_SIGNAL_WORD : LVK_SCHED_WAIT_WORD_TIMEOUT]++;
    }
    if (!have_results)
    {
        if (chain_event_armed) LVK_HIP_CHECK(ctx, hipEventSynchronize(chain_done));
        else LVK_HIP_CHECK(ctx, hipStreamSynchronize(st));
        sched[LVK_SCHED_WAIT_EVENT]++;
    }
    trace.mark(HostTrace::LK_SYNC);

    if (dev_insert)
    {
        const int n_new = h_insert[0];
        float q_dev; std::memcpy(&q_dev, &h_insert[2], sizeof(float));
        if (n_new < 0 || (size_t)n_new > grid.capacity()) return fail(LVK_HIP_ERR_RUNTIME, "device suppression grid returned an impossible count");
        distribution = grid.finish_device(tracked, h_new_kp, n_new, h_fast_counts, fast_cap);
        last_distribution = distribution; last_detected = (int)tracked.size();
        if (distribution != q_dev || tracked.size() != n_held + (size_t)n_new)
            return fail(LVK_HIP_ERR_RUNTIME, "device suppression grid disagrees with the host's bookkeeping");
        if (tracked.size() < (size_t)s.min_motion_samples || distribution < s.uniformity_threshold) { tracked.clear(); return LVK_HIP_OK; }
        if (tracked.size() > cap_features) return fail(LVK_HIP_ERR_RUNTIME, "feature count exceeds the suppression grid capacity");
        n = (int)tracked.size();
    }
    if (chained)
    {
        const int m = *h_count;
        last_matched = m;
        if (m < 0 || m > n) return fail(LVK_HIP_ERR_RUNTIME, "GPU-side fast_filter returned an impossible count");
        if ((size_t)m < (size_t)s.min_motion_samples) { tracked.clear(); return LVK_HIP_OK; }
        motion = WarpMeshF(s.motion_height, s.motion_width);
        if (field)
        {
            if (*h_mesh_status != 0) { tracked.clear(); return LVK_HIP_OK; }
            std::memcpy(motion.off.data(), h_offsets, motion.off.size() * sizeof(float));
        }
        else
        {
            std::memcpy(last_H, h_H, sizeof(last_H));
            motion.from_homography(last_H, (float)cur_w, (float)cur_h);
        }
        size_t inliers = 0;
        for (int i = 0; i < m; i++) inliers += h_mask[i] ? 1 : 0;
        tracking_stability = (float)inliers / (float)m;
        have_motion = true;
        post_n = n; post_m = m;
        trace.mark(HostTrace::POST);
        return LVK_HIP_OK;
    }

    if (lens && !chained)
    {
        const float w = (float)cur_w, h = (float)cur_h;
        auto inside = [&](const float2& p) { return p.x >= 0.0f && p.x < w && p.y >= 0.0f && p.y < h; };
        for (int k = 0; k < n; k++)
            if (!(inside(h_und[k]) && inside(h_und[n + k]))) h_status[k] = 0;
    }
    int m = n;
// ... 37 lines not shown
            if (h_mask[i]) { tracked[i].age++; tracked[i].x = h_matched[i].x; tracked[i].y = h_matched[i].y; }
            else { std::swap(tracked[i], tracked.back()); tracked.pop_back(); }
        }
        grid.propagate(tracked);
        have_motion = true;
        return LVK_HIP_OK;
    }
    if (!chained)
    {
        std::memcpy(h_p1, e1, m * sizeof(float2));
        std::memcpy(h_p1 + m, e2, m * sizeof(float2));
        LVK_HIP_CHECK(ctx, hipMemcpyAsync(d_p1, h_p1, 2 * (size_t)m * sizeof(float2), hipMemcpyHostToDevice, st));
        pe = prof_begin(LVK_STAGE_MOTION);
        if ((rc = lvk_launch_ransac(ctx, d_p1, d_p1 + m, m, s.acceptance_threshold, (double)cur_w, (double)cur_h, full, d_ransac_ws, h_H, h_ninl, h_mask)) != LVK_HIP_OK) return rc;
        prof_end(pe);
        trace.mark(HostTrace::RANSAC_LAUNCH);
        LVK_HIP_CHECK(ctx, hipStreamSynchronize(st));
        trace.mark(HostTrace::RANSAC_SYNC);
    }
    std::memcpy(last_H, h_H, sizeof(last_H));
    motion.from_homography(last_H, (float)cur_w, (float)cur_h);

    size_t inliers = 0;
    for (int i = 0; i < m; i++) inliers += h_mask[i] ? 1 : 0;
    tracking_stability = (float)inliers / (float)m;

    for (int i = m - 1; i >= 0; i--)
    {
        if (h_mask[i]) { tracked[i].age++; tracked[i].x = h_matched[i].x; tracked[i].y = h_matched[i].y; }
        else { std::swap(tracked[i], tracked.back()); tracked.pop_back(); }
    }
    grid.propagate(tracked);
    have_motion = true;
    trace.mark(HostTrace::POST);
    return LVK_HIP_OK;
}

static const char* lvk_frame_format_name(int f);
static std::string lvk_stab_pixel_class_clash(const lvk_hip_stab* st, int bpp, int format);


int lvk_stab_push_impl(lvk_hip_stab* st, const void* d_frame, int step, int rows, int cols, uint64_t timestamp, int format,
                     const void* luma, int luma_step, int luma_pix,
                     void* d_out, int out_step, int out_rows, int* produced, uint64_t* out_timestamp, const void** released, OutPlanes420* o420,
                     lvk_frame_info* emitted, int bpp)
{
    lvk_hip_ctx* ctx = st->ctx;
    if (produced) *produced = 0;
    if (released) *released = nullptr;
    LVK_HIP_REQUIRE(ctx, bpp == 1 || bpp == 3 || bpp == 4);
    const bool gray_entry = bpp == 1, c4_entry = bpp == 4;
    if (gray_entry) LVK_HIP_REQUIRE(ctx, d_frame && rows > 0 && cols > 0 && step >= cols && format == LVK_FORMAT_GRAY && luma_pix == 1);
    else if (c4_entry) LVK_HIP_REQUIRE(ctx, d_frame && rows > 0 && cols > 0 && step >= 4 * cols && (format == LVK_FORMAT_BGRA || format == LVK_FORMAT_RGBA) && luma_pix == 4);
    else LVK_HIP_REQUIRE(ctx, d_frame && rows > 0 && cols > 0 && step >= 3 * cols);
    if (!st->buffers_ok) return ctx->fail(LVK_HIP_ERR_RUNTIME, "the last configure() failed while allocating the tracker's buffers: configure again");
    if (bpp == 3) LVK_HIP_REQUIRE(ctx, format == LVK_FORMAT_YUV || format == LVK_FORMAT_BGR || format == LVK_FORMAT_RGB);
    const int luma_channel = (gray_entry || format == LVK_FORMAT_YUV) ? 0 : ((format == LVK_FORMAT_BGR || format == LVK_FORMAT_BGRA) ? -1 : -2);
    if (bpp == 3) LVK_HIP_REQUIRE(ctx, luma_pix == 3 || format == LVK_FORMAT_YUV);
    { const std::string why = lvk_stab_pixel_class_clash(st, bpp, format); if (!why.empty()) return ctx->fail(LVK_HIP_ERR_ARG, why); }
    const QueuedFrame in{d_frame, step, rows, cols, timestamp, format};
    {
        QueuedFrame due;
        if (st->next_output(in, &due))
        {
            const bool to_planes = o420 && o420->y && (st->s.stabilize_output || st->s.crop_to_stable_region || st->lens);
            const bool planes_fit = !o420 || o420->vf != 0 ||
                                    (o420->y && o420->y_step >= due.cols && o420->u_step >= (o420->nv12 ? due.cols : due.cols / 2) &&
                                     (o420->nv12 || o420->v_step >= due.cols / 2) && o420->rows_cap >= due.rows);
            const bool fits = planes_fit && (to_planes || (d_out != nullptr && out_step >= bpp * due.cols && out_rows >= due.rows));
            if (!fits)
                return ctx->fail(LVK_HIP_ERR_ARG, "the output buffer does not hold the frame this push emits: " + std::to_string(due.cols) + " x " + std::to_string(due.rows) +
                                                      " (the DELAYED frame's own size -- lvk_hip_stab_next_output); nothing was queued");
        }
    }
    st->caller_runs_free = st->caller_free_running_now() || st->host_free_running_hint;
    if (st->caller_runs_free) { st->free_streak++; st->sync_streak = 0; }
    else
    {
        const bool grace = st->free_streak >= 8 && st->sync_streak == 0;
        st->sync_streak++;
        if (grace) st->caller_runs_free = true; else st->free_streak = 0;
    }
    st->sched[st->caller_runs_free ? LVK_SCHED_PUSH_FREE_RUNNING : LVK_SCHED_PUSH_SYNCHRONISED]++;
    { const int lrc = st->ensure_lens(rows, cols); if (lrc != LVK_HIP_OK) return lrc; }
    static const WarpMeshF identity_mesh(2, 2);
    const uint8_t bg[4] = {(uint8_t)st->s.background[0], (uint8_t)st->s.background[1], (uint8_t)st->s.background[2], st->background_alpha};

    auto enqueue = [&]() {
        if (st->queue.size() == st->queue_capacity) { if (released) *released = st->queue.front().d_ptr; st->queue.pop_front(); }
        st->queue.push_back(in);
    };
    auto emit = [&](const WarpMeshF* mesh) -> int {
        const QueuedFrame f = st->queue.front();
        st->queue.pop_front();
        int rc = LVK_HIP_OK;
        const bool side = st->overlap && mesh && st->s.stabilize_output;
        hipStream_t rs = side ? st->remap_stream : ctx->stream;
        const bool persistent = side && st->caller_runs_free;
        if (mesh) st->sched[persistent ? LVK_SCHED_REMAP_PERSISTENT : LVK_SCHED_REMAP_FULL]++;
        const int co_blocks_per_cu = (persistent && st->host_direct_now) ? 1 : 0;
        if (side && (rc = st->bulk_stream_sees_caller_work()) != LVK_HIP_OK) return rc;
        if (st->remap_wait) { const hipEvent_t e = st->remap_wait; st->remap_wait = nullptr; LVK_HIP_CHECK(ctx, hipStreamWaitEvent(rs, e, 0)); }
        st->trace.mark(HostTrace::EMIT_WAITS);
        const int pe = st->prof_begin(LVK_STAGE_REMAP, rs);
        LensArgs lens_other; const LensArgs* lens_args = nullptr;
        if (st->lens)
        {
            lens_args = &st->lens_args;
            if (f.rows != st->lens_rows || f.cols != st->lens_cols)
            {
                LensModel m;
                if (lvk_lens_model_build(st->lens_params, f.rows, f.cols, m) != LVK_HIP_OK) return ctx->fail(LVK_HIP_ERR_ARG, "invalid camera profile for the delayed frame's size");
                std::memcpy(lens_other.f, m.f, sizeof(lens_other.f)); lens_args = &lens_other;
            }
        }
        const RemapLaunch how{rs, st->remap_precision, lens_args, persistent, co_blocks_per_cu};
        if (mesh && o420 && o420->y && o420->vf != 0)
        {
            rc = lvk_launch_warpmesh_apply_obs(ctx, o420->vf, f.d_ptr, f.step, f.rows, f.cols, o420->p, o420->s, mesh->off.data(), mesh->rows, mesh->cols, bg, how);
            o420->used = true;
        }
        else if (mesh && o420 && o420->y)
        {
            rc = lvk_launch_warpmesh_apply_420(ctx, f.d_ptr, f.step, f.rows, f.cols, o420->y, o420->y_step, o420->u, o420->u_step, o420->v, o420->v_step,
                                               o420->nv12, mesh->off.data(), mesh->rows, mesh->cols, bg, how);
            o420->used = true;
        }
        else if (mesh && gray_entry) rc = lvk_launch_warpmesh_apply_lens_gray(ctx, f.d_ptr, f.step, f.rows, f.cols, d_out, out_step, mesh->off.data(), mesh->rows, mesh->cols, bg[0], how);
        else if (mesh && c4_entry) rc = lvk_launch_warpmesh_apply_lens_c4(ctx, f.d_ptr, f.step, f.rows, f.cols, d_out, out_step, mesh->off.data(), mesh->rows, mesh->cols, bg, how);
        else if (mesh) rc = lvk_launch_warpmesh_apply_lens(ctx, f.d_ptr, f.step, f.rows, f.cols, d_out, out_step, mesh->off.data(), mesh->rows, mesh->cols, bg,
                                                      f.format == LVK_FORMAT_YUV ? 1 : 0, how);
        else
        {
            hipError_t e = hipMemcpy2DAsync(d_out, out_step, f.d_ptr, f.step, (size_t)f.cols * bpp, f.rows, hipMemcpyDeviceToDevice, ctx->stream);
            if (e != hipSuccess) rc = ctx->fail(LVK_HIP_ERR_RUNTIME, hipGetErrorString(e));
        }
        st->prof_end(pe, rs);
        st->trace.mark(HostTrace::EMIT_KERNEL);
        if (rc != LVK_HIP_OK) return rc;
        if (produced) *produced = 1;
        if (out_timestamp) *out_timestamp = f.ts;
        if (emitted) *emitted = lvk_frame_info{f.rows, f.cols, f.format};
        if (side && st->pool_frames)
        {
            if (st->tracker_ingest_capable)
            {
                const int si = st->slot_index(f.d_ptr);
                if (si >= 0)
                {
                    if (!st->slot_read_done[(size_t)si]) { hipError_t e = hipEventCreateWithFlags(&st->slot_read_done[(size_t)si], hipEventDisableTiming); if (e != hipSuccess) return ctx->fail(LVK_HIP_ERR_RUNTIME, hipGetErrorString(e)); }
                    hipError_t e = hipEventRecord(st->slot_read_done[(size_t)si], rs);
                    if (e != hipSuccess) return ctx->fail(LVK_HIP_ERR_RUNTIME, hipGetErrorString(e));
                    st->slot_read_armed[(size_t)si] = 1;
                }
            }
            if (released) *released = f.d_ptr;
        }
        else if (side)
        {
            const int slot = st->remap_slot; st->remap_slot ^= 1;
            hipError_t e = hipEventRecord(st->remap_done[slot], rs);
            if (e != hipSuccess) return ctx->fail(LVK_HIP_ERR_RUNTIME, hipGetErrorString(e));
            if (st->pending_release)
            {
                if ((e = hipEventSynchronize(st->remap_done[st->pending_slot])) != hipSuccess) return ctx->fail(LVK_HIP_ERR_RUNTIME, hipGetErrorString(e));
                if (released) *released = st->pending_release;
            }
            st->pending_release = f.d_ptr; st->pending_slot = slot;
        }
        else if (released) *released = f.d_ptr;
        return LVK_HIP_OK;
    };

    if (!st->s.stabilize_output)
    {
        enqueue();
        if (st->queue.size() != st->queue_capacity) return LVK_HIP_OK;
        return emit(st->s.crop_to_stable_region ? &st->smoother.scene_crop() : st->lens ? &identity_mesh : nullptr);
    }

    st->trace.mark(HostTrace::ENTER);
    WarpMeshF motion(st->s.motion_height, st->s.motion_width);
    WarpMeshF est; bool have = false;
    if (st->post_error) { st->post_error = false; return st->fail(LVK_HIP_ERR_RUNTIME, "GPU-side fast_filter disagrees with the host's"); }
    int rc = st->track(in, luma, luma_step, luma_pix, luma_channel, est, have);
    if (rc != LVK_HIP_OK) { st->finish_post(); return rc; }
    if (have) motion = est;

    const float tq = st->tracking_stability;
    st->scene_quality = st->scene_quality + QA_UPDATE_RATE * (tq - st->scene_quality);
    if (tq < st->s.min_tracking_quality) st->trust = 0.0f;
    else if (st->scene_quality < st->s.min_scene_quality) st->trust = step_toward(st->trust, 0.0f, QA_BLEND_STEP);
    else st->trust = step_toward(st->trust, 1.0f, QA_BLEND_STEP);
    motion.scale(st->trust);
    st->last_motion = motion;

    enqueue();
    WarpMeshF correction = st->smoother.next(motion);
    if (st->queue.size() != st->queue_capacity) return LVK_HIP_OK;
    if (st->s.crop_to_stable_region) correction += st->smoother.scene_crop();
    st->last_correction = correction;
    st->trace.mark(HostTrace::SMOOTH);
    const int erc = emit(&correction);
    st->trace.mark(HostTrace::REMAP_LAUNCH);
    return erc;
}

bool lvk_hip_stab::caller_free_running_now()
{
    bulk_busy_at_push = false;
    if (overlap && remap_stream)
    {
        const hipError_t q = hipStreamQuery(remap_stream);
        if (q != hipSuccess) (void)hipGetLastError();
        bulk_busy_at_push = q == hipErrorNotReady;
    }
    if (assume_caller) return assume_caller == 1;
    return bulk_busy_at_push || (last_push_end.time_since_epoch().count() != 0 && std::chrono::steady_clock::now() - last_push_end < std::chrono::microseconds(15));
}
// ... 388 lines not shown
```

Measured before the change: 9495.

## Add persistent unit-grid remap for YUV420 and adapt ingest placement to it

Converts the YUV420 remap kernels to a units-capable form in which a persistent grid processes work units, using a wave-level 420 sink and an LDS-staged mesh when the mesh fits. It drops the LDS padding knob and reports which grid form was launched back to the stabilizer. When the last remap used units and only one free-running stream is active on the device, the stabilizer stops moving ingest onto the tracker stream, on the assumption that the bulk stream has spare room. A per-device atomic counter tracks free-running stabilizers, and a test entry point exposes explicit grid selection.

Result: slower. 9378 (-1.2%).

```diff
diff --git a/include/lvk_hip.h b/include/lvk_hip.h
--- a/include/lvk_hip.h
+++ b/include/lvk_hip.h
@@ -353,6 +353,12 @@
 } lvk_track_chain_result;
 int lvk_hip_track_chain(lvk_hip_ctx* ctx, const lvk_track_chain_desc* desc, lvk_track_chain_result* result);
 
+enum { LVK_REMAP_GRID_FULL = 0, LVK_REMAP_GRID_PERSISTENT = 1, LVK_REMAP_GRID_PERSISTENT_UNITS = 2 };
+int lvk_hip_warpmesh_apply_yuv420_grid(lvk_hip_ctx* ctx, const void* d_src, int src_step, int rows, int cols,
+                                       void* o_y, int oy_step, void* o_u, int ou_step, void* o_v, int ov_step, int nv12,
+                                       const float* mesh, int mesh_rows, int mesh_cols, const uint8_t bg[3], const lvk_camera_params* lens,
+                                       int precision, int grid, int unit_blocks);
+
 int lvk_hip_deblock_get_grid(lvk_hip_deblock* deb, uint8_t* mean, uint8_t* grid, float* keep_block, int capacity, int extent_xy[2]);
 
 int lvk_hip_cas_const(float sharpness, float* peak);
diff --git a/livevisionkit_amd/_native.py b/livevisionkit_amd/_native.py
--- a/livevisionkit_amd/_native.py
+++ b/livevisionkit_amd/_native.py
@@ -84,6 +84,8 @@
     "lvk_hip_text_size": (_c.c_int, [_c.c_char_p, _c.c_int, _c.c_int, _c.POINTER(_c.c_int), _c.POINTER(_c.c_int)]),
     "lvk_hip_warpmesh_apply_yuv420": (_c.c_int, [_P, _P, _c.c_int, _c.c_int, _c.c_int, _P, _c.c_int, _P, _c.c_int, _P, _c.c_int, _c.c_int,
                                                  _c.POINTER(_c.c_float), _c.c_int, _c.c_int, _c.POINTER(_c.c_uint8)]),
+    "lvk_hip_warpmesh_apply_yuv420_grid": (_c.c_int, [_P, _P, _c.c_int, _c.c_int, _c.c_int, _P, _c.c_int, _P, _c.c_int, _P, _c.c_int, _c.c_int,
+                                                      _c.POINTER(_c.c_float), _c.c_int, _c.c_int, _c.POINTER(_c.c_uint8), _P, _c.c_int, _c.c_int, _c.c_int]),
     "lvk_hip_warpmesh_apply": (_c.c_int, [_P, _P, _c.c_int, _c.c_int, _c.c_int, _P, _c.c_int,
                                           _c.POINTER(_c.c_float), _c.c_int, _c.c_int, _c.POINTER(_c.c_uint8), _c.c_int]),
     "lvk_hip_luma_area_resize": (_c.c_int, [_P, _P, _c.c_int, _c.c_int, _c.c_int, _c.c_int, _c.c_int, _P, _c.c_int, _c.c_int, _c.c_int]),
diff --git a/livevisionkit_amd/context.py b/livevisionkit_amd/context.py
--- a/livevisionkit_amd/context.py
+++ b/livevisionkit_amd/context.py
@@ -514,6 +514,21 @@
                                                            mp, m.shape[0], m.shape[1], bgp))
         return (y, u) if nv12 else (y, u, v)
 
+    def warpmesh_apply_yuv420_grid(self, src, mesh, planes, bg=(255, 0, 255), nv12=False, lens=None, precision=0, persistent=False, unit_blocks=0):
+        rows, cols = src.shape[0], src.shape[1]
+        y, u = planes[0], planes[1]
+        v = u if nv12 else planes[2]
+        m = np.ascontiguousarray(mesh, dtype=np.float32)
+        ma, mp = _f32(m)
+        bga, bgp = _u8x3(bg)
+        arr = (ctypes.c_double * 9)(*[float(x) for x in lens]) if lens is not None else None
+        rc = self.lib.lvk_hip_warpmesh_apply_yuv420_grid(self.handle, src.data_ptr(), src.stride(0), rows, cols, y.data_ptr(), y.stride(0),
+                                                         u.data_ptr(), u.stride(0), v.data_ptr(), v.stride(0), 1 if nv12 else 0,
+                                                         mp, m.shape[0], m.shape[1], bgp, arr, int(precision), 1 if persistent else 0, int(unit_blocks))
+        if rc < 0:
+            self._check(rc)
+        return rc
+
 
 class MeshSolver:
 
diff --git a/livevisionkit_amd/csrc/lvk_hip_internal.hpp b/livevisionkit_amd/csrc/lvk_hip_internal.hpp
--- a/livevisionkit_amd/csrc/lvk_hip_internal.hpp
+++ b/livevisionkit_amd/csrc/lvk_hip_internal.hpp
@@ -260,6 +260,7 @@
     const LensArgs* lens = nullptr;
     bool co_scheduled = false;
     int co_blocks_per_cu = 0;
+    int co_unit_blocks = 0;
 };
 int lvk_launch_remap_homography(lvk_hip_ctx* ctx, const void* d_src, int src_step, int src_rows, int src_cols,
                                 void* d_dst, int dst_step, int dst_rows, int dst_cols, int off_x, int off_y,
@@ -356,7 +357,7 @@
 
 int lvk_launch_warpmesh_apply_420(lvk_hip_ctx* ctx, const void* d_src, int src_step, int rows, int cols,
                                   void* o_y, int oy_step, void* o_u, int ou_step, void* o_v, int ov_step, int nv12,
-                                  const float* mesh, int mesh_rows, int mesh_cols, const uint8_t bg[3], const RemapLaunch& o);
+                                  const float* mesh, int mesh_rows, int mesh_cols, const uint8_t bg[3], const RemapLaunch& o, int* grid_taken = nullptr);
 bool lvk_remap_obs_fusable(int video_format);
 int lvk_launch_warpmesh_apply_obs(lvk_hip_ctx* ctx, int video_format, const void* d_src, int src_step, int rows, int cols,
                                   void* const planes[3], const int steps[3], const float* mesh, int mesh_rows, int mesh_cols, const uint8_t bg[3], const RemapLaunch& o);
diff --git a/livevisionkit_amd/csrc/remap.hip b/livevisionkit_amd/csrc/remap.hip
--- a/livevisionkit_amd/csrc/remap.hip
+++ b/livevisionkit_amd/csrc/remap.hip
@@ -1,7 +1,4 @@
 #include "remap_core.hpp"
-#ifndef LVK_CO_LDS_PAD
-#define LVK_CO_LDS_PAD 0
-#endif
 
 namespace {
 
@@ -58,36 +55,45 @@
 }
 
 struct Planes420 { uint8_t* y; int y_step; uint8_t* u; int u_step; uint8_t* v; int v_step; };
-template <bool NV12> __device__ __forceinline__ Sink420<NV12> sink420(const Planes420& o) { return Sink420<NV12>{o.y, o.y_step, o.u, o.u_step, o.v, o.v_step}; }
-
-LVK_REMAP_KERNEL(bool NV12, LVK_CO_SCHEDULED, k_remap_homography_420,
-                 (const uint8_t* __restrict__ src, int src_step, int rows, int cols, Planes420 o, HomographyArgs H, uint32_t bg),
+template <bool NV12, class G> __device__ __forceinline__ auto sink420(const Planes420& o)
+{
+    const Sink420<NV12> strips{o.y, o.y_step, o.u, o.u_step, o.v, o.v_step};
+    if constexpr (std::is_same_v<G, UnitGrid>) return Sink420Wave<NV12>{strips};
+    else return strips;
+}
+
+LVK_REMAP_KERNEL_UNITS(bool NV12, k_remap_homography_420,
+                       (const uint8_t* __restrict__ src, int src_step, int rows, int cols, Planes420 o, HomographyArgs H, uint32_t bg),
 {
     LVK_TL(0);
-    remap_homography<true, W, false>(src, src_step, rows, cols, sink420<NV12>(o), rows, cols, 0, 0, H, LensArgs{}, bg);
-})
-
-LVK_REMAP_KERNEL(bool NV12, LVK_CO_SCHEDULED, k_remap_homography_lens_420,
-                 (const uint8_t* __restrict__ src, int src_step, int rows, int cols, Planes420 o, HomographyArgs H, LensArgs L, uint32_t bg),
-{
-    remap_homography<true, W, true>(src, src_step, rows, cols, sink420<NV12>(o), rows, cols, 0, 0, H, L, bg);
-})
-
-LVK_REMAP_KERNEL(bool NV12, LVK_CO_SCHEDULED, k_remap_mesh_420,
-                 (const uint8_t* __restrict__ src, int src_step, int rows, int cols, Planes420 o,
-                  const float* __restrict__ mesh, int mesh_cols, int mesh_floats, const LinTabEntry* __restrict__ xtab, const LinTabEntry* __restrict__ ytab, uint32_t bg),
-{
-    const Sink420<NV12> sink = sink420<NV12>(o);
-    LVK_WITH_MESH_COORD(false, LensArgs{}, rows, cols, (remap_strip<true, W>(src, src_step, rows, cols, sink, rows, cols, coord, bg)))
-})
-
-LVK_REMAP_KERNEL(bool NV12, LVK_CO_SCHEDULED, k_remap_mesh_lens_420,
-                 (const uint8_t* __restrict__ src, int src_step, int rows, int cols, Planes420 o,
-                  const float* __restrict__ mesh, int mesh_cols, int mesh_floats, const LinTabEntry* __restrict__ xtab, const LinTabEntry* __restrict__ ytab,
-                  LensArgs L, uint32_t bg),
-{
-    const Sink420<NV12> sink = sink420<NV12>(o);
-    LVK_WITH_MESH_COORD(true, L, rows, cols, (remap_strip<true, W>(src, src_step, rows, cols, sink, rows, cols, coord, bg)))
+    G::open(false);
+    remap_homography<true, W, false, G>(src, src_step, rows, cols, sink420<NV12, G>(o), rows, cols, 0, 0, H, LensArgs{}, bg);
+})
+
+LVK_REMAP_KERNEL_UNITS(bool NV12, k_remap_homography_lens_420,
+                       (const uint8_t* __restrict__ src, int src_step, int rows, int cols, Planes420 o, HomographyArgs H, LensArgs L, uint32_t bg),
+{
+    G::open(false);
+    remap_homography<true, W, true, G>(src, src_step, rows, cols, sink420<NV12, G>(o), rows, cols, 0, 0, H, L, bg);
+})
+
+LVK_REMAP_KERNEL_UNITS(bool NV12, k_remap_mesh_420,
+                       (const uint8_t* __restrict__ src, int src_step, int rows, int cols, Planes420 o,
+                        const float* __restrict__ mesh, int mesh_cols, int mesh_floats, const LinTabEntry* __restrict__ xtab, const LinTabEntry* __restrict__ ytab, uint32_t bg),
+{
+    const auto sink = sink420<NV12, G>(o);
+    G::open(mesh_floats <= MESH_LDS_FLOATS);
+    LVK_WITH_MESH_COORD(false, LensArgs{}, rows, cols, (remap_strip<true, W, G>(src, src_step, rows, cols, sink, rows, cols, coord, bg)))
+})
+
+LVK_REMAP_KERNEL_UNITS(bool NV12, k_remap_mesh_lens_420,
+                       (const uint8_t* __restrict__ src, int src_step, int rows, int cols, Planes420 o,
+                        const float* __restrict__ mesh, int mesh_cols, int mesh_floats, const LinTabEntry* __restrict__ xtab, const LinTabEntry* __restrict__ ytab,
+                        LensArgs L, uint32_t bg),
+{
+    const auto sink = sink420<NV12, G>(o);
+    G::open(mesh_floats <= MESH_LDS_FLOATS);
+    LVK_WITH_MESH_COORD(true, L, rows, cols, (remap_strip<true, W, G>(src, src_step, rows, cols, sink, rows, cols, coord, bg)))
 })
 
 }
@@ -102,10 +108,10 @@
     HomographyArgs args;
     std::memcpy(args.h, H, sizeof(args.h));
     if (o.lens)
-        launch_remap(ctx, LVK_REMAP_FORMS_CO(k_remap_homography_lens, false, true), yuv != 0, dst_rows, dst_cols, o, 0, (const uint8_t*)d_src, src_step, src_rows, src_cols,
+        launch_remap(ctx, LVK_REMAP_FORMS_CO(k_remap_homography_lens, false, true), yuv != 0, dst_rows, dst_cols, o, (const uint8_t*)d_src, src_step, src_rows, src_cols,
                      (uint8_t*)d_dst, dst_step, dst_rows, dst_cols, off_x, off_y, args, *o.lens, pack_bg(bg));
     else
-        launch_remap(ctx, LVK_REMAP_FORMS_CO(k_remap_homography, false, true), yuv != 0, dst_rows, dst_cols, o, 0, (const uint8_t*)d_src, src_step, src_rows, src_cols,
+        launch_remap(ctx, LVK_REMAP_FORMS_CO(k_remap_homography, false, true), yuv != 0, dst_rows, dst_cols, o, (const uint8_t*)d_src, src_step, src_rows, src_cols,
                      (uint8_t*)d_dst, dst_step, dst_rows, dst_cols, off_x, off_y, args, pack_bg(bg));
     LVK_HIP_CHECK(ctx, hipGetLastError());
     return LVK_HIP_OK;
@@ -120,10 +126,10 @@
     LVK_HIP_REQUIRE(ctx, remap_plane_ok(d_src, src_step, src_rows, src_cols, 3) && remap_plane_ok(d_dst, dst_step, src_rows, src_cols, 3));
     return with_staged_mesh(ctx, o.stream, mesh, mesh_rows, mesh_cols, src_rows, src_cols, [&](const StagedMesh& m) {
         if (o.lens)
-            launch_remap(ctx, LVK_REMAP_FORMS_CO(k_remap_mesh_lens, false, true), yuv != 0, src_rows, src_cols, o, 0, (const uint8_t*)d_src, src_step, src_rows, src_cols,
+            launch_remap(ctx, LVK_REMAP_FORMS_CO(k_remap_mesh_lens, false, true), yuv != 0, src_rows, src_cols, o, (const uint8_t*)d_src, src_step, src_rows, src_cols,
                          (uint8_t*)d_dst, dst_step, m.d_mesh, m.mesh_cols, m.mesh_floats, m.xtab, m.ytab, *o.lens, pack_bg(bg));
         else
-            launch_remap(ctx, LVK_REMAP_FORMS_CO(k_remap_mesh, false, true), yuv != 0, src_rows, src_cols, o, 0, (const uint8_t*)d_src, src_step, src_rows, src_cols,
+            launch_remap(ctx, LVK_REMAP_FORMS_CO(k_remap_mesh, false, true), yuv != 0, src_rows, src_cols, o, (const uint8_t*)d_src, src_step, src_rows, src_cols,
                          (uint8_t*)d_dst, dst_step, m.d_mesh, m.mesh_cols, m.mesh_floats, m.xtab, m.ytab, pack_bg(bg));
     });
 }
@@ -134,7 +140,7 @@
     LVK_HIP_REQUIRE(ctx, remap_precision_known(o.precision));
     LVK_HIP_REQUIRE(ctx, bg != nullptr);
     LVK_HIP_REQUIRE(ctx, remap_plane_ok(d_src, src_step, rows, cols, 3) && remap_plane_ok(d_dst, dst_step, rows, cols, 3) && remap_map_ok(d_map, map_step, rows, cols));
-    launch_remap(ctx, LVK_REMAP_FORMS(k_remap_map, false, true), yuv != 0, rows, cols, RemapLaunch{o.stream, o.precision}, 0, (const uint8_t*)d_src, src_step, rows, cols, (uint8_t*)d_dst, dst_step,
+    launch_remap(ctx, LVK_REMAP_FORMS(k_remap_map, false, true), yuv != 0, rows, cols, RemapLaunch{o.stream, o.precision}, (const uint8_t*)d_src, src_step, rows, cols, (uint8_t*)d_dst, dst_step,
                  (const uint8_t*)d_map, map_step, pack_bg(bg));
     LVK_HIP_CHECK(ctx, hipGetLastError());
     return LVK_HIP_OK;
@@ -171,29 +177,32 @@
 
 int lvk_launch_warpmesh_apply_420(lvk_hip_ctx* ctx, const void* d_src, int src_step, int rows, int cols,
                                   void* o_y, int oy_step, void* o_u, int ou_step, void* o_v, int ov_step, int nv12,
-                                  const float* mesh, int mesh_rows, int mesh_cols, const uint8_t bg[3], const RemapLaunch& o)
+                                  const float* mesh, int mesh_rows, int mesh_cols, const uint8_t bg[3], const RemapLaunch& o, int* grid_taken)
 {
     LVK_HIP_REQUIRE(ctx, remap_precision_known(o.precision));
     LVK_HIP_REQUIRE(ctx, bg != nullptr && remap_mesh_ok(mesh, mesh_rows, mesh_cols));
     LVK_HIP_REQUIRE(ctx, (rows & 1) == 0 && (cols & 1) == 0 && remap_plane_ok(d_src, src_step, rows, cols, 3) && remap_plane_ok(o_y, oy_step, rows, cols, 1));
     LVK_HIP_REQUIRE(ctx, remap_plane_ok(o_u, ou_step, rows / 2, cols / 2, nv12 ? 2 : 1) && (nv12 || remap_plane_ok(o_v, ov_step, rows / 2, cols / 2, 1)));
     const Planes420 planes{(uint8_t*)o_y, oy_step, (uint8_t*)o_u, ou_step, (uint8_t*)(nv12 ? o_u : o_v), nv12 ? ou_step : ov_step};
-    const size_t lds_pad = o.co_scheduled ? (size_t)LVK_CO_LDS_PAD : 0;
+    int taken = LVK_REMAP_GRID_FULL;
     if (mesh_rows == 2 && mesh_cols == 2)
     {
         HomographyArgs H;
         lvkh::mesh2x2_to_homography(mesh, rows, cols, H.h);
-        if (o.lens) launch_remap(ctx, LVK_REMAP_FORMS(k_remap_homography_lens_420, false, true), nv12 != 0, rows, cols, o, lds_pad, (const uint8_t*)d_src, src_step, rows, cols, planes, H, *o.lens, pack_bg(bg));
-        else launch_remap(ctx, LVK_REMAP_FORMS(k_remap_homography_420, false, true), nv12 != 0, rows, cols, o, lds_pad, (const uint8_t*)d_src, src_step, rows, cols, planes, H, pack_bg(bg));
+        if (o.lens) taken = launch_remap(ctx, LVK_REMAP_FORMS_UNITS(k_remap_homography_lens_420, false, true), nv12 != 0, rows, cols, o, (const uint8_t*)d_src, src_step, rows, cols, planes, H, *o.lens, pack_bg(bg));
+        else taken = launch_remap(ctx, LVK_REMAP_FORMS_UNITS(k_remap_homography_420, false, true), nv12 != 0, rows, cols, o, (const uint8_t*)d_src, src_step, rows, cols, planes, H, pack_bg(bg));
         LVK_HIP_CHECK(ctx, hipGetLastError());
+        if (grid_taken) *grid_taken = taken;
         return LVK_HIP_OK;
     }
-    return with_staged_mesh(ctx, o.stream, mesh, mesh_rows, mesh_cols, rows, cols, [&](const StagedMesh& m) {
-        if (o.lens) launch_remap(ctx, LVK_REMAP_FORMS(k_remap_mesh_lens_420, false, true), nv12 != 0, rows, cols, o, lds_pad, (const uint8_t*)d_src, src_step, rows, cols, planes,
-                                 m.d_mesh, m.mesh_cols, m.mesh_floats, m.xtab, m.ytab, *o.lens, pack_bg(bg));
-        else launch_remap(ctx, LVK_REMAP_FORMS(k_remap_mesh_420, false, true), nv12 != 0, rows, cols, o, lds_pad, (const uint8_t*)d_src, src_step, rows, cols, planes,
-                          m.d_mesh, m.mesh_cols, m.mesh_floats, m.xtab, m.ytab, pack_bg(bg));
+    const int rc = with_staged_mesh(ctx, o.stream, mesh, mesh_rows, mesh_cols, rows, cols, [&](const StagedMesh& m) {
+        if (o.lens) taken = launch_remap(ctx, LVK_REMAP_FORMS_UNITS(k_remap_mesh_lens_420, false, true), nv12 != 0, rows, cols, o, (const uint8_t*)d_src, src_step, rows, cols, planes,
+                                         m.d_mesh, m.mesh_cols, m.mesh_floats, m.xtab, m.ytab, *o.lens, pack_bg(bg));
+        else taken = launch_remap(ctx, LVK_REMAP_FORMS_UNITS(k_remap_mesh_420, false, true), nv12 != 0, rows, cols, o, (const uint8_t*)d_src, src_step, rows, cols, planes,
+                                  m.d_mesh, m.mesh_cols, m.mesh_floats, m.xtab, m.ytab, pack_bg(bg));
     });
+    if (grid_taken) *grid_taken = taken;
+    return rc;
 }
 
 extern "C" {
@@ -242,6 +251,28 @@
     return lvk_launch_warpmesh_apply_420(ctx, d_src, src_step, rows, cols, o_y, oy_step, o_u, ou_step, o_v, ov_step, nv12, mesh, mesh_rows, mesh_cols, bg, RemapLaunch{ctx->stream, ctx->remap_precision});
 }
 
+int lvk_hip_warpmesh_apply_yuv420_grid(lvk_hip_ctx* ctx, const void* d_src, int src_step, int rows, int cols,
+                                       void* o_y, int oy_step, void* o_u, int ou_step, void* o_v, int ov_step, int nv12,
+                                       const float* mesh, int mesh_rows, int mesh_cols, const uint8_t bg[3], const lvk_camera_params* lens,
+                                       int precision, int grid, int unit_blocks)
+{
+    LVK_HIP_ENTRY(ctx);
+    LVK_HIP_REQUIRE(ctx, (grid == LVK_REMAP_GRID_FULL || grid == LVK_REMAP_GRID_PERSISTENT) && unit_blocks >= 0 && unit_blocks <= 4096);
+    LVK_HIP_REQUIRE(ctx, grid == LVK_REMAP_GRID_PERSISTENT || unit_blocks == 0);
+    LensArgs a;
+    if (lens)
+    {
+        LVK_HIP_REQUIRE(ctx, rows > 1 && cols > 1);
+        const int rc = lens_args_of(ctx, lens, rows, cols, a);
+        if (rc != LVK_HIP_OK) return rc;
+    }
+    RemapLaunch how{ctx->stream, precision, lens ? &a : nullptr, grid == LVK_REMAP_GRID_PERSISTENT};
+    how.co_unit_blocks = unit_blocks;
+    int taken = 0;
+    const int rc = lvk_launch_warpmesh_apply_420(ctx, d_src, src_step, rows, cols, o_y, oy_step, o_u, ou_step, o_v, ov_step, nv12, mesh, mesh_rows, mesh_cols, bg, how, &taken);
+    return rc != LVK_HIP_OK ? rc : taken;
+}
+
 int lvk_hip_upscale(lvk_hip_ctx* ctx, const void* d_src, int src_step, int src_rows, int src_cols,
                     void* d_dst, int dst_step, int dst_rows, int dst_cols, int yuv)
 {
diff --git a/livevisionkit_amd/csrc/remap_core.hpp b/livevisionkit_amd/csrc/remap_core.hpp
--- a/livevisionkit_amd/csrc/remap_core.hpp
+++ b/livevisionkit_amd/csrc/remap_core.hpp
@@ -390,56 +390,67 @@
 struct Sink420
 {
     uint8_t* __restrict__ yp; int y_step; uint8_t* __restrict__ up; int u_step; uint8_t* __restrict__ vp; int v_step;
+    static __device__ __forceinline__ uint2 pair_sums(const uint32_t px[PXT])
+    {
+        const uint32_t u01 = ((px[0] >> 8) & 0xffu) + ((px[1] >> 8) & 0xffu), u23 = ((px[2] >> 8) & 0xffu) + ((px[3] >> 8) & 0xffu);
+        const uint32_t v01 = ((px[0] >> 16) & 0xffu) + ((px[1] >> 16) & 0xffu), v23 = ((px[2] >> 16) & 0xffu) + ((px[3] >> 16) & 0xffu);
+        return make_uint2(u01 | (u23 << 16), v01 | (v23 << 16));
+    }
+    __device__ __forceinline__ void store_luma(int x0, int y, int npx, const uint32_t px[PXT]) const
+    {
+        uint8_t* yr = yp + (__umul24((uint32_t)y, (uint32_t)y_step) + (uint32_t)x0);
+        const uint32_t yy = (px[0] & 0xffu) | ((px[1] & 0xffu) << 8) | ((px[2] & 0xffu) << 16) | ((px[3] & 0xffu) << 24);
+        if (npx == PXT && ((reinterpret_cast<uintptr_t>(yr) & 3u) == 0)) LVK_STREAM_STORE(reinterpret_cast<uint32_t*>(yr), yy);
+        else for (int p = 0; p < npx; p++) yr[p] = (uint8_t)(yy >> (8 * p));
+    }
+    __device__ __forceinline__ void store_chroma(int x0, int y, int npx, const uint2 a, const uint2 b) const
+    {
+        const uint32_t u0 = ((a.x & 0xffffu) + (b.x & 0xffffu) + 2u) >> 2, u1 = ((a.x >> 16) + (b.x >> 16) + 2u) >> 2;
+        const uint32_t v0 = ((a.y & 0xffffu) + (b.y & 0xffffu) + 2u) >> 2, v1 = ((a.y >> 16) + (b.y >> 16) + 2u) >> 2;
+        const int cx = x0 >> 1, cy = y >> 1, nc = npx >> 1;
+        if (NV12)
+        {
+            uint8_t* d = up + (__umul24((uint32_t)cy, (uint32_t)u_step) + 2u * (uint32_t)cx);
+            d[0] = (uint8_t)u0; d[1] = (uint8_t)v0;
+            if (nc > 1) { d[2] = (uint8_t)u1; d[3] = (uint8_t)v1; }
+        }
+        else
+        {
+            uint8_t* du = up + (__umul24((uint32_t)cy, (uint32_t)u_step) + (uint32_t)cx); uint8_t* dv = vp + (__umul24((uint32_t)cy, (uint32_t)v_step) + (uint32_t)cx);
+            du[0] = (uint8_t)u0; dv[0] = (uint8_t)v0;
+            if (nc > 1) { du[1] = (uint8_t)u1; dv[1] = (uint8_t)v1; }
+        }
+    }
     __device__ __forceinline__ void store(int x0, int y, int npx, const uint32_t px[PXT], bool active, int parity) const
     {
         __shared__ uint2 s_uv2[2][256];
         uint2* s_uv = s_uv2[parity & 1];
         const int t = (int)threadIdx.x;
-        const uint32_t u01 = ((px[0] >> 8) & 0xffu) + ((px[1] >> 8) & 0xffu), u23 = ((px[2] >> 8) & 0xffu) + ((px[3] >> 8) & 0xffu);
-        const uint32_t v01 = ((px[0] >> 16) & 0xffu) + ((px[1] >> 16) & 0xffu), v23 = ((px[2] >> 16) & 0xffu) + ((px[3] >> 16) & 0xffu);
-        s_uv[t] = make_uint2(u01 | (u23 << 16), v01 | (v23 << 16));
-        if (active)
-        {
-            uint8_t* yr = yp + (__umul24((uint32_t)y, (uint32_t)y_step) + (uint32_t)x0);
-            const uint32_t yy = (px[0] & 0xffu) | ((px[1] & 0xffu) << 8) | ((px[2] & 0xffu) << 16) | ((px[3] & 0xffu) << 24);
-            if (npx == PXT && ((reinterpret_cast<uintptr_t>(yr) & 3u) == 0)) LVK_STREAM_STORE(reinterpret_cast<uint32_t*>(yr), yy);
-            else for (int p = 0; p < npx; p++) yr[p] = (uint8_t)(yy >> (8 * p));
-        }
+        s_uv[t] = pair_sums(px);
+        if (active) store_luma(x0, y, npx, px);
         __syncthreads();
-        if (active && ((t >> 6) & 1) == 0)
-        {
-            const uint2 a = s_uv[t], b = s_uv[t + 64];
-            const uint32_t u0 = ((a.x & 0xffffu) + (b.x & 0xffffu) + 2u) >> 2, u1 = ((a.x >> 16) + (b.x >> 16) + 2u) >> 2;
-            const uint32_t v0 = ((a.y & 0xffffu) + (b.y & 0xffffu) + 2u) >> 2, v1 = ((a.y >> 16) + (b.y >> 16) + 2u) >> 2;
-            const int cx = x0 >> 1, cy = y >> 1, nc = npx >> 1;
-            if (NV12)
-            {
-                uint8_t* d = up + (__umul24((uint32_t)cy, (uint32_t)u_step) + 2u * (uint32_t)cx);
-                d[0] = (uint8_t)u0; d[1] = (uint8_t)v0;
-                if (nc > 1) { d[2] = (uint8_t)u1; d[3] = (uint8_t)v1; }
-            }
-            else
-            {
-                uint8_t* du = up + (__umul24((uint32_t)cy, (uint32_t)u_step) + (uint32_t)cx); uint8_t* dv = vp + (__umul24((uint32_t)cy, (uint32_t)v_step) + (uint32_t)cx);
-                du[0] = (uint8_t)u0; dv[0] = (uint8_t)v0;
-                if (nc > 1) { du[1] = (uint8_t)u1; dv[1] = (uint8_t)v1; }
-            }
-        }
-    }
-};
-
-template <bool YUV, class W = EasuExact, class Coord, class Sink>
-__device__ __forceinline__ void remap_one_strip(const uint8_t* __restrict__ src, int src_step, int src_rows, int src_cols,
-                                                const Sink& sink, int dst_rows, int dst_cols, const Coord& coord, uint32_t bg,
-                                                int strip, int nstrips, int strips_x, int parity)
-{
-    const int sy_ = strip / strips_x, sx_ = strip - sy_ * strips_x;
-    const int x0 = sx_ * STRIP_W + (int)(threadIdx.x & 63) * PXT;
-    const int y = sy_ * STRIP_H + (int)(threadIdx.x >> 6);
-    const bool active = strip < nstrips && x0 < dst_cols && y < dst_rows;
-    const int npx = active ? min(PXT, dst_cols - x0) : 0;
+        if (active && ((t >> 6) & 1) == 0) store_chroma(x0, y, npx, s_uv[t], s_uv[t + 64]);
+    }
+};
+
+template <bool NV12>
+struct Sink420Wave : Sink420<NV12>
+{
+    __device__ __forceinline__ void store(int x0, int y, int npx, const uint32_t px[PXT], bool active) const
+    {
+        const uint2 a = this->pair_sums(px);
+        const uint2 b = make_uint2((uint32_t)__shfl_xor((int)a.x, 32), (uint32_t)__shfl_xor((int)a.y, 32));
+        if (!active) return;
+        this->store_luma(x0, y, npx, px);
+        if ((threadIdx.x & 32u) == 0) this->store_chroma(x0, y, npx, a, b);
+    }
+};
+
+template <bool YUV, class W, class Coord>
+__device__ __forceinline__ void remap_pixels(const uint8_t* __restrict__ src, int src_step, int src_rows, int src_cols, const Coord& coord, uint32_t bg,
+                                             int x0, int y, int npx, uint32_t px[PXT])
+{
     const TapBases tb = tap_bases(src, src_step);
-    uint32_t px[PXT];
 #pragma unroll
     for (int p = 0; p < PXT; p++)
     {
@@ -464,6 +475,20 @@
             else px[p] = easu_gather<YUV, W>(tb, src_step, sx, sy, ppx, ppy);
         }
     }
+}
+
+template <bool YUV, class W = EasuExact, class Coord, class Sink>
+__device__ __forceinline__ void remap_one_strip(const uint8_t* __restrict__ src, int src_step, int src_rows, int src_cols,
+                                                const Sink& sink, int dst_rows, int dst_cols, const Coord& coord, uint32_t bg,
+                                                int strip, int nstrips, int strips_x, int parity)
+{
+    const int sy_ = strip / strips_x, sx_ = strip - sy_ * strips_x;
+    const int x0 = sx_ * STRIP_W + (int)(threadIdx.x & 63) * PXT;
+    const int y = sy_ * STRIP_H + (int)(threadIdx.x >> 6);
+    const bool active = strip < nstrips && x0 < dst_cols && y < dst_rows;
+    const int npx = active ? min(PXT, dst_cols - x0) : 0;
+    uint32_t px[PXT];
+    remap_pixels<YUV, W>(src, src_step, src_rows, src_cols, coord, bg, x0, y, npx, px);
     sink.store(x0, y, npx, px, active, parity);
 }
 
@@ -484,36 +509,98 @@
     }
 }
 
-template <bool YUV, class W = EasuExact, class Coord, class Sink>
+constexpr int UNIT_W = 32 * PXT, UNIT_H = 2, CO_UNIT_THREADS = 1024;
+#define LVK_CO_UNIT_VGPRS __attribute__((amdgpu_waves_per_eu(6)))
+__shared__ unsigned s_unit_next;
+
+struct StripGrid
+{
+    static __device__ __forceinline__ void open(bool ) {}
+};
+struct UnitGrid
+{
+    static __device__ __forceinline__ void open(bool barrier_follows)
+    {
+        if (threadIdx.x == 0) s_unit_next = 0;
+        if (!barrier_follows) __syncthreads();
+    }
+};
+
+template <class F>
+__device__ __forceinline__ void walk_units(int dst_rows, int dst_cols, const F& one_unit)
+{
+    const int units_x = (dst_cols + UNIT_W - 1) / UNIT_W, nunits = units_x * ((dst_rows + UNIT_H - 1) / UNIT_H);
+    const int band = (nunits + NUM_XCD - 1) / NUM_XCD;
+    const int per_xcd = (int)(gridDim.x / NUM_XCD), run = (band + per_xcd - 1) / per_xcd;
+    const int xcd = (int)(blockIdx.x % NUM_XCD);
+    const int first = xcd * band + (int)(blockIdx.x / NUM_XCD) * run;
+    const int end = min(min(first + run, (xcd + 1) * band), nunits);
+    for (;;)
+    {
+        unsigned drawn = 0;
+        if ((threadIdx.x & 63u) == 0) drawn = atomicAdd(&s_unit_next, 1u);
+        const int unit = first + (int)__builtin_amdgcn_readfirstlane(drawn);
+        if (unit >= end) break;
+        one_unit(unit, units_x);
+    }
+}
+
+template <bool YUV, class W, class Coord, class Sink>
+__device__ __forceinline__ void remap_one_unit(const uint8_t* __restrict__ src, int src_step, int src_rows, int src_cols,
+                                               const Sink& sink, int dst_rows, int dst_cols, const Coord& coord, uint32_t bg, int unit, int units_x)
+{
+    const int uy = unit / units_x, ux = unit - uy * units_x;
+    const int x0 = ux * UNIT_W + (int)(threadIdx.x & 31) * PXT;
+    const int y = uy * UNIT_H + (int)((threadIdx.x >> 5) & 1);
+    const bool active = x0 < dst_cols && y < dst_rows;
+    const int npx = active ? min(PXT, dst_cols - x0) : 0;
+    uint32_t px[PXT];
+    remap_pixels<YUV, W>(src, src_step, src_rows, src_cols, coord, bg, x0, y, npx, px);
+    sink.store(x0, y, npx, px, active);
+}
+
+template <bool YUV, class W = EasuExact, class G = StripGrid, class Coord, class Sink>
 __device__ __forceinline__ void remap_strip(const uint8_t* __restrict__ src, int src_step, int src_rows, int src_cols,
                                             const Sink& sink, int dst_rows, int dst_cols,
                                             const Coord& coord, uint32_t bg)
 {
-    walk_strips(dst_rows, dst_cols, [&](int strip, int nstrips, int strips_x, int parity) __attribute__((always_inline)) {
-        remap_one_strip<YUV, W>(src, src_step, src_rows, src_cols, sink, dst_rows, dst_cols, coord, bg, strip, nstrips, strips_x, parity);
-    });
-}
-
-template <bool YUV, class W, bool LENS, class Sink>
+    if constexpr (std::is_same_v<G, UnitGrid>)
+        walk_units(dst_rows, dst_cols, [&](int unit, int units_x) __attribute__((always_inline)) {
+            remap_one_unit<YUV, W>(src, src_step, src_rows, src_cols, sink, dst_rows, dst_cols, coord, bg, unit, units_x);
+        });
+    else
+        walk_strips(dst_rows, dst_cols, [&](int strip, int nstrips, int strips_x, int parity) __attribute__((always_inline)) {
+            remap_one_strip<YUV, W>(src, src_step, src_rows, src_cols, sink, dst_rows, dst_cols, coord, bg, strip, nstrips, strips_x, parity);
+        });
+}
+
+template <bool YUV, class W, bool LENS, class G = StripGrid, class Sink>
 __device__ __forceinline__ void remap_homography(const uint8_t* __restrict__ src, int src_step, int src_rows, int src_cols, const Sink& sink, int dst_rows, int dst_cols,
                                                  int off_x, int off_y, const HomographyArgs& H, const LensArgs& L, uint32_t bg)
 {
     with_homography_coord<LENS>(H, off_x, off_y, L, src_rows, src_cols, [&](const auto& coord) __attribute__((always_inline)) {
-        remap_strip<YUV, W>(src, src_step, src_rows, src_cols, sink, dst_rows, dst_cols, coord, bg);
+        remap_strip<YUV, W, G>(src, src_step, src_rows, src_cols, sink, dst_rows, dst_cols, coord, bg);
     });
 }
 
-#define LVK_REMAP_KERNEL(TPARAM, ATTR, NAME, PARAMS, ...)                                                                          \
-    template <TPARAM> __global__ __launch_bounds__(256) LVK_REMAP_ATTR ATTR void NAME PARAMS { using W = EasuExact; __VA_ARGS__ }  \
-    template <TPARAM> __global__ __launch_bounds__(256) LVK_REMAP_ATTR ATTR void NAME##_r1 PARAMS { using W = EasuRegrouped; __VA_ARGS__ }
+#define LVK_REMAP_KERNEL_(TPARAM, ATTR, THREADS, GRID, NAME, PARAMS, ...)                                                                                    \
+    template <TPARAM> __global__ __launch_bounds__(THREADS) LVK_REMAP_ATTR ATTR void NAME PARAMS { using W = EasuExact; using G [[maybe_unused]] = GRID; __VA_ARGS__ }       \
+    template <TPARAM> __global__ __launch_bounds__(THREADS) LVK_REMAP_ATTR ATTR void NAME##_r1 PARAMS { using W = EasuRegrouped; using G [[maybe_unused]] = GRID; __VA_ARGS__ }
+#define LVK_REMAP_KERNEL(TPARAM, ATTR, NAME, PARAMS, ...) LVK_REMAP_KERNEL_(TPARAM, ATTR, 256, StripGrid, NAME, PARAMS, __VA_ARGS__)
 #define LVK_REMAP_KERNEL_CO(TPARAM, NAME, PARAMS, ...)                 \
     LVK_REMAP_KERNEL(TPARAM, , NAME, PARAMS, __VA_ARGS__)              \
     LVK_REMAP_KERNEL(TPARAM, LVK_CO_SCHEDULED, NAME##_co, PARAMS, __VA_ARGS__)
-template <class K> struct RemapForms { K k[2][2][2]; };
+#define LVK_REMAP_KERNEL_UNITS(TPARAM, NAME, PARAMS, ...)                                  \
+    LVK_REMAP_KERNEL(TPARAM, LVK_CO_SCHEDULED, NAME, PARAMS, __VA_ARGS__)                  \
+    LVK_REMAP_KERNEL_(TPARAM, LVK_CO_SCHEDULED LVK_CO_UNIT_VGPRS, CO_UNIT_THREADS, UnitGrid, NAME##_co, PARAMS, __VA_ARGS__)
+template <class K> struct RemapForms { K k[2][2][2]; K units[2][2]; };
 #define LVK_REMAP_FORMS_(K, KCO, F0, F1) \
-    RemapForms<decltype(&K<F0>)>{ { { { K<F0>, K<F1> }, { K##_r1<F0>, K##_r1<F1> } }, { { KCO<F0>, KCO<F1> }, { KCO##_r1<F0>, KCO##_r1<F1> } } } }
+    RemapForms<decltype(&K<F0>)>{ { { { K<F0>, K<F1> }, { K##_r1<F0>, K##_r1<F1> } }, { { KCO<F0>, KCO<F1> }, { KCO##_r1<F0>, KCO##_r1<F1> } } }, {} }
 #define LVK_REMAP_FORMS(K, F0, F1) LVK_REMAP_FORMS_(K, K, F0, F1)
 #define LVK_REMAP_FORMS_CO(K, F0, F1) LVK_REMAP_FORMS_(K, K##_co, F0, F1)
+#define LVK_REMAP_FORMS_UNITS(K, F0, F1) \
+    RemapForms<decltype(&K<F0>)>{ { { { K<F0>, K<F1> }, { K##_r1<F0>, K##_r1<F1> } }, { { K<F0>, K<F1> }, { K##_r1<F0>, K##_r1<F1> } } },  \
+                                  { { K##_co<F0>, K##_co<F1> }, { K##_co_r1<F0>, K##_co_r1<F1> } } }
 
 inline dim3 remap_grid(int dst_rows, int dst_cols)
 {
@@ -530,12 +617,29 @@
     return dim3(full < persistent ? full : persistent);
 }
 
+inline unsigned lvk_co_unit_grid(const lvk_hip_ctx* ctx, const RemapLaunch& o, int dst_rows, int dst_cols)
+{
+    if (o.co_unit_blocks > 0) return (unsigned)((o.co_unit_blocks + NUM_XCD - 1) / NUM_XCD * NUM_XCD);
+    if (o.co_blocks_per_cu != 0) return 0;
+    const int n = ctx->cu_count > 0 ? ctx->cu_count : 256;
+    const long blocks = std::max(NUM_XCD, n / NUM_XCD * NUM_XCD);
+    const long nunits = (long)((dst_cols + UNIT_W - 1) / UNIT_W) * ((dst_rows + UNIT_H - 1) / UNIT_H);
+    return nunits >= blocks * (CO_UNIT_THREADS / 64) ? (unsigned)blocks : 0;
+}
+
 template <class K, class... Args>
-inline void launch_remap(const lvk_hip_ctx* ctx, const RemapForms<K>& forms, bool flag, int dst_rows, int span_cols, const RemapLaunch& o, size_t lds_bytes,
-                         const Args&... args)
-{
+inline int launch_remap(const lvk_hip_ctx* ctx, const RemapForms<K>& forms, bool flag, int dst_rows, int span_cols, const RemapLaunch& o, const Args&... args)
+{
+    const int r1 = o.precision == LVK_REMAP_1LSB ? 1 : 0;
+    const unsigned unit_blocks = (o.co_scheduled && forms.units[r1][flag ? 1 : 0]) ? lvk_co_unit_grid(ctx, o, dst_rows, span_cols) : 0;
+    if (unit_blocks)
+    {
+        hipLaunchKernelGGL(forms.units[r1][flag ? 1 : 0], dim3(unit_blocks), dim3(CO_UNIT_THREADS), 0, o.stream, args...);
+        return LVK_REMAP_GRID_PERSISTENT_UNITS;
+    }
     const dim3 grid = o.co_scheduled ? lvk_co_grid(ctx, o.co_blocks_per_cu, dst_rows, span_cols) : remap_grid(dst_rows, span_cols);
-    hipLaunchKernelGGL(forms.k[o.co_scheduled ? 1 : 0][o.precision == LVK_REMAP_1LSB ? 1 : 0][flag ? 1 : 0], grid, dim3(256), lds_bytes, o.stream, args...);
+    hipLaunchKernelGGL(forms.k[o.co_scheduled ? 1 : 0][r1][flag ? 1 : 0], grid, dim3(256), 0, o.stream, args...);
+    return o.co_scheduled ? LVK_REMAP_GRID_PERSISTENT : LVK_REMAP_GRID_FULL;
 }
 
 inline bool remap_precision_known(int precision) { return precision == LVK_REMAP_EXACT || precision == LVK_REMAP_1LSB; }
diff --git a/livevisionkit_amd/csrc/remap_obs.hip b/livevisionkit_amd/csrc/remap_obs.hip
--- a/livevisionkit_amd/csrc/remap_obs.hip
+++ b/livevisionkit_amd/csrc/remap_obs.hip
@@ -110,15 +110,15 @@
     {
         HomographyArgs H;
         lvkh::mesh2x2_to_homography(mesh, rows, cols, H.h);
-        if (o.lens) launch_remap(ctx, LVK_REMAP_FORMS(k_remap_homography_lens_planes, Sink, Sink), false, rows, cols, o, 0, (const uint8_t*)d_src, src_step, rows, cols, sink, H, *o.lens, pack_bg(bg));
-        else launch_remap(ctx, LVK_REMAP_FORMS(k_remap_homography_planes, Sink, Sink), false, rows, cols, o, 0, (const uint8_t*)d_src, src_step, rows, cols, sink, H, pack_bg(bg));
+        if (o.lens) launch_remap(ctx, LVK_REMAP_FORMS(k_remap_homography_lens_planes, Sink, Sink), false, rows, cols, o, (const uint8_t*)d_src, src_step, rows, cols, sink, H, *o.lens, pack_bg(bg));
+        else launch_remap(ctx, LVK_REMAP_FORMS(k_remap_homography_planes, Sink, Sink), false, rows, cols, o, (const uint8_t*)d_src, src_step, rows, cols, sink, H, pack_bg(bg));
         LVK_HIP_CHECK(ctx, hipGetLastError());
         return LVK_HIP_OK;
     }
     return with_staged_mesh(ctx, o.stream, mesh, mesh_rows, mesh_cols, rows, cols, [&](const StagedMesh& m) {
-        if (o.lens) launch_remap(ctx, LVK_REMAP_FORMS(k_remap_mesh_lens_planes, Sink, Sink), false, rows, cols, o, 0, (const uint8_t*)d_src, src_step, rows, cols, sink,
+        if (o.lens) launch_remap(ctx, LVK_REMAP_FORMS(k_remap_mesh_lens_planes, Sink, Sink), false, rows, cols, o, (const uint8_t*)d_src, src_step, rows, cols, sink,
                                  m.d_mesh, m.mesh_cols, m.mesh_floats, m.xtab, m.ytab, *o.lens, pack_bg(bg));
-        else launch_remap(ctx, LVK_REMAP_FORMS(k_remap_mesh_planes, Sink, Sink), false, rows, cols, o, 0, (const uint8_t*)d_src, src_step, rows, cols, sink,
+        else launch_remap(ctx, LVK_REMAP_FORMS(k_remap_mesh_planes, Sink, Sink), false, rows, cols, o, (const uint8_t*)d_src, src_step, rows, cols, sink,
                           m.d_mesh, m.mesh_cols, m.mesh_floats, m.xtab, m.ytab, pack_bg(bg));
     });
 }
diff --git a/livevisionkit_amd/csrc/remap_px.hip b/livevisionkit_amd/csrc/remap_px.hip
--- a/livevisionkit_amd/csrc/remap_px.hip
+++ b/livevisionkit_amd/csrc/remap_px.hip
@@ -215,7 +215,7 @@
     LVK_HIP_REQUIRE(ctx, H != nullptr && Pix::bg_ok(bg) && planes_ok<Pix>(d_src, src_step, src_rows, src_cols, d_dst, dst_step, dst_rows, dst_cols));
     HomographyArgs args;
     std::memcpy(args.h, H, sizeof(args.h));
-    launch_remap(ctx, LVK_PX_FORMS(k_remap_homography_px, Pix), o.lens != nullptr, dst_rows, px_span(dst_cols), o, 0, (const uint8_t*)d_src, src_step, src_rows, src_cols,
+    launch_remap(ctx, LVK_PX_FORMS(k_remap_homography_px, Pix), o.lens != nullptr, dst_rows, px_span(dst_cols), o, (const uint8_t*)d_src, src_step, src_rows, src_cols,
                  (uint8_t*)d_dst, dst_step, dst_rows, dst_cols, off_x, off_y, args, o.lens ? *o.lens : LensArgs{}, Pix::pack_bg(bg));
     LVK_HIP_CHECK(ctx, hipGetLastError());
     return LVK_HIP_OK;
@@ -227,7 +227,7 @@
 {
     LVK_HIP_REQUIRE(ctx, Pix::bg_ok(bg) && remap_mesh_ok(mesh, mesh_rows, mesh_cols) && planes_ok<Pix>(d_src, src_step, rows, cols, d_dst, dst_step, rows, cols));
     return with_staged_mesh(ctx, o.stream, mesh, mesh_rows, mesh_cols, rows, cols, [&](const StagedMesh& m) {
-        launch_remap(ctx, LVK_PX_FORMS(k_remap_mesh_px, Pix), o.lens != nullptr, rows, px_span(cols), o, 0, (const uint8_t*)d_src, src_step, rows, cols, (uint8_t*)d_dst, dst_step,
+        launch_remap(ctx, LVK_PX_FORMS(k_remap_mesh_px, Pix), o.lens != nullptr, rows, px_span(cols), o, (const uint8_t*)d_src, src_step, rows, cols, (uint8_t*)d_dst, dst_step,
                      m.d_mesh, m.mesh_cols, m.mesh_floats, m.xtab, m.ytab, o.lens ? *o.lens : LensArgs{}, Pix::pack_bg(bg));
     });
 }
diff --git a/livevisionkit_amd/csrc/stab_configure.hip b/livevisionkit_amd/csrc/stab_configure.hip
--- a/livevisionkit_amd/csrc/stab_configure.hip
+++ b/livevisionkit_amd/csrc/stab_configure.hip
@@ -278,6 +278,7 @@
 void lvk_hip_stab_destroy(lvk_hip_stab* st)
 {
     if (!st) return;
+    st->count_free_running(false);
     lvk_device_guard device_guard(st->ctx);
     (void)hipStreamSynchronize(st->ctx->stream);
     st->trace.dump();
diff --git a/livevisionkit_amd/csrc/stab_state.hpp b/livevisionkit_amd/csrc/stab_state.hpp
--- a/livevisionkit_amd/csrc/stab_state.hpp
+++ b/livevisionkit_amd/csrc/stab_state.hpp
@@ -1,4 +1,5 @@
 #pragma once
+#include <atomic>
 #include "lvk_hip_internal.hpp"
 #include "host_logic.hpp"
 
@@ -180,6 +181,15 @@
     bool ingest_on_tracker = false, tracker_ingest_capable = false;
     bool bulk_busy_at_push = false;
     bool caller_runs_free = false;
+    static std::atomic<int>& free_running_on(int device) { static std::atomic<int> n[64]; return n[(unsigned)device % 64u]; }
+    bool counted_free_running = false;
+    void count_free_running(bool now)
+    {
+        if (now == counted_free_running) return;
+        free_running_on(ctx->device).fetch_add(now ? 1 : -1, std::memory_order_relaxed);
+        counted_free_running = now;
+    }
+    bool unit_remap_last = false;
     int assume_caller = [] { const char* e = std::getenv("LVK_HIP_ASSUME_CALLER"); return !e ? 0 : (e[0] == 'f' ? 1 : (e[0] == 's' ? 2 : 0)); }();
     int free_streak = 0, sync_streak = 0;
     std::chrono::steady_clock::time_point last_push_end{};
diff --git a/livevisionkit_amd/csrc/stabilizer.hip b/livevisionkit_amd/csrc/stabilizer.hip
--- a/livevisionkit_amd/csrc/stabilizer.hip
+++ b/livevisionkit_amd/csrc/stabilizer.hip
@@ -125,7 +125,9 @@
     {
         const hipError_t q = hipStreamQuery(remap_stream);
         if (q != hipSuccess) (void)hipGetLastError();
-        ingest_on_tracker = ingest_placement == 1 || (ingest_placement == 0 && ((q == hipErrorNotReady && !host_direct_now) || ingest_wait[0] != nullptr));
+        const bool bulk_has_room = unit_remap_last && free_running_on(ctx->device).load(std::memory_order_relaxed) == 1;
+        ingest_on_tracker = ingest_placement == 1 ||
+                            (ingest_placement == 0 && ((q == hipErrorNotReady && !host_direct_now && !bulk_has_room) || ingest_wait[0] != nullptr));
     }
     const bool build_ahead = chained && ahead_announced.luma != nullptr && pyr_w == cur_w && pyr_h == cur_h;
     if (chained && ((deferred_ingest && tracker_ingest_capable && ingest_on_tracker) || build_ahead))
@@ -329,6 +331,7 @@
         if (grace) st->caller_runs_free = true; else st->free_streak = 0;
     }
     st->sched[st->caller_runs_free ? LVK_SCHED_PUSH_FREE_RUNNING : LVK_SCHED_PUSH_SYNCHRONISED]++;
+    st->count_free_running(st->caller_runs_free);
     { const int lrc = st->ensure_lens(rows, cols); if (lrc != LVK_HIP_OK) return lrc; }
     static const WarpMeshF identity_mesh(2, 2);
     const uint8_t bg[4] = {(uint8_t)st->s.background[0], (uint8_t)st->s.background[1], (uint8_t)st->s.background[2], st->background_alpha};
@@ -362,6 +365,7 @@
             }
         }
         const RemapLaunch how{rs, st->remap_precision, lens_args, persistent, co_blocks_per_cu};
+        bool unit_remap = false;
         if (mesh && o420 && o420->y && o420->vf != 0)
         {
             rc = lvk_launch_warpmesh_apply_obs(ctx, o420->vf, f.d_ptr, f.step, f.rows, f.cols, o420->p, o420->s, mesh->off.data(), mesh->rows, mesh->cols, bg, how);
@@ -369,8 +373,10 @@
         }
         else if (mesh && o420 && o420->y)
         {
+            int grid_taken = LVK_REMAP_GRID_FULL;
             rc = lvk_launch_warpmesh_apply_420(ctx, f.d_ptr, f.step, f.rows, f.cols, o420->y, o420->y_step, o420->u, o420->u_step, o420->v, o420->v_step,
-                                               o420->nv12, mesh->off.data(), mesh->rows, mesh->cols, bg, how);
+                                               o420->nv12, mesh->off.data(), mesh->rows, mesh->cols, bg, how, &grid_taken);
+            unit_remap = rc == LVK_HIP_OK && grid_taken == LVK_REMAP_GRID_PERSISTENT_UNITS;
             o420->used = true;
         }
         else if (mesh && gray_entry) rc = lvk_launch_warpmesh_apply_lens_gray(ctx, f.d_ptr, f.step, f.rows, f.cols, d_out, out_step, mesh->off.data(), mesh->rows, mesh->cols, bg[0], how);
@@ -382,6 +388,7 @@
             hipError_t e = hipMemcpy2DAsync(d_out, out_step, f.d_ptr, f.step, (size_t)f.cols * bpp, f.rows, hipMemcpyDeviceToDevice, ctx->stream);
             if (e != hipSuccess) rc = ctx->fail(LVK_HIP_ERR_RUNTIME, hipGetErrorString(e));
         }
+        if (mesh) st->unit_remap_last = unit_remap;
         st->prof_end(pe, rs);
         st->trace.mark(HostTrace::EMIT_KERNEL);
         if (rc != LVK_HIP_OK) return rc;
```
